# PaddlePaddle/PaddleRec

Hardware: AMD Instinct MI355X
Metric: CTR samples/sec, Criteo DeepFM bs=65536 (train step: fwd+bwd+optimizer) (higher is better)
Workload: dtype f32 (MLP GEMMs: f32 operands as 3 bf16 terms, 6 bf16 MFMAs per product, f32 accumulate); 1 GPU; DeepFM full Criteo: 26 sparse slots x 1000000 rows x dim 16, 13 dense, MLP 400,400,400, batch 65536 per GPU, lazy Adam, uniform ids; global_batch=65536, parallelism=single, table_rows_total=26000000, index_oob_flag=0

## Files before the change

### include/recengine.h

```cpp
#ifndef RECENGINE_H_
#define RECENGINE_H_

#include <stddef.h>
#include <stdint.h>

#ifdef __cplusplus
extern "C" {
#endif

typedef enum {
  REC_OK = 0,
  REC_EINVAL = -1,
  REC_ESHAPE = -2,
  REC_EWORKSPACE = -3,
  REC_EHIP = -4,
  REC_ENCCL = -5
} rec_status;

#define REC_FLAG_INDEX_OOB 1
#define REC_FLAG_EXCHANGE_OVERFLOW 2

const char* rec_last_error(void);
int rec_version(void);

// ... 342 lines not shown

int rec_batchnorm_workspace_bytes(int64_t m, int32_t n, size_t* bytes);
int rec_batchnorm_fwd(int64_t m, int32_t n, const float* X, int64_t ldx, const float* gamma, const float* beta,
                      float* running_mean, float* running_var, float momentum, float eps, int32_t training,
                      float* Y, int64_t ldy, float* save_mean, float* save_invstd, void* workspace,
                      size_t workspace_bytes, void* stream);
int rec_batchnorm_bwd(int64_t m, int32_t n, const float* X, int64_t ldx, const float* dY, int64_t lddy,
                      const float* gamma, const float* save_mean, const float* save_invstd, int32_t relu_mask,
                      float* dX, int64_t lddx, float* dgamma, float* dbeta, void* workspace,
                      size_t workspace_bytes, void* stream);
int rec_dot_interact_fwd(int64_t batch, int32_t F, int32_t D, const float* T, int64_t ldt, float* R, int64_t ldr,
                         void* stream);
int rec_dot_interact_bwd(int64_t batch, int32_t F, int32_t D, const float* T, int64_t ldt, const float* dR,
                         int64_t ldr, float* dT, int64_t lddt, void* stream);
int rec_accuracy_count(int64_t n, const float* pred, const int64_t* label, int64_t* counts, void* stream);

typedef enum {
  REC_EPI_NONE = 0,
  REC_EPI_BIAS = 1,
  REC_EPI_BIAS_RELU = 2,
  REC_EPI_RELU_MASK = 3,
  REC_EPI_CROSS = 4,
  REC_EPI_BIAS_SIGMOID = 5,
  REC_EPI_BIAS_TANH = 6,
  REC_EPI_ADD = 7,
  REC_EPI_DTANH = 10,
  REC_EPI_DSIGMOID = 9,
  REC_EPI_MOE = 8
} rec_epilogue;

typedef struct {
  int64_t m;
  int32_t n, k;
  int32_t lda, ldb, ldc;
  int32_t trans_a, trans_b;
  int32_t epilogue;
  int32_t split_k;
  int32_t num_cus;
} rec_gemm_desc;

typedef struct {
  const float* bias;
  const float* aux0;
  int32_t ld_aux0;
  const float* aux1;
  int32_t ld_aux1;
  const float* row_scale;
  int32_t row_scale_stride;
  float* out2;
  int32_t ld_out2;
  float* b_colsum;
  const void* b_image;
  void* relu_bits;
} rec_gemm_epilogue_args;

int rec_gemm_f32_workspace_bytes(const rec_gemm_desc* desc, size_t* bytes);
int rec_gemm_relu_bits_bytes(const rec_gemm_desc* desc, int32_t* eligible, size_t* bytes);
int rec_gemm_plan_splits(const rec_gemm_desc* desc, int32_t num_cus, int32_t* splits);
int rec_gemm_f32(const rec_gemm_desc* desc, const float* A, const float* B, float* C,
                 const rec_gemm_epilogue_args* args , void* workspace,
                 size_t workspace_bytes, void* stream);
int rec_gemm_f32_pair(const rec_gemm_desc* desc0, const float* A0, const float* B0, float* C0,
                      const rec_gemm_epilogue_args* args0 , const rec_gemm_desc* desc1, const float* A1,
                      const float* B1, float* C1, const rec_gemm_epilogue_args* args1 , void* workspace,
                      size_t workspace_bytes, void* stream);
typedef enum {
  REC_GEMM_ROUTE_SKINNY_ROWS = 0,
  REC_GEMM_ROUTE_SKINNY_DW = 1,
  REC_GEMM_ROUTE_X3_DW = 2,
  REC_GEMM_ROUTE_X3 = 3,
  REC_GEMM_ROUTE_PANEL = 4,
  REC_GEMM_ROUTE_GLDS = 5,
  REC_GEMM_ROUTE_DIRECT = 6,
  REC_GEMM_ROUTE_TILED = 7
} rec_gemm_route_family;
enum {
  REC_GEMM_ROUTE_FAST = 1,
  REC_GEMM_ROUTE_PIPE = 2,
  REC_GEMM_ROUTE_VEC = 4,
  REC_GEMM_ROUTE_KS4 = 8,
  REC_GEMM_ROUTE_FOLD = 16,
  REC_GEMM_ROUTE_VEC_A = 32,
  REC_GEMM_ROUTE_PAIR = 64
};
typedef struct {
  int32_t family;
  int32_t cfg;
  int32_t splits;
  int32_t flags;
} rec_gemm_route;
int rec_gemm_last_route(rec_gemm_route* out);
typedef struct {
  const float* B;
  int32_t ldb, k, n, trans_b;
  void* image;
} rec_gemm_b_image;
int rec_gemm_b_image_bytes(int32_t k, int32_t n, int32_t* eligible, size_t* bytes);
int rec_gemm_b_images(int32_t count, const rec_gemm_b_image* items, void* stream);

int rec_colsum_workspace_bytes(int64_t m, int32_t n, size_t* bytes);
int rec_colsum(int64_t m, int32_t n, int32_t ld, const float* G, float* out, void* workspace,
               size_t workspace_bytes, void* stream);

typedef struct {
  int64_t batch;
  int32_t d;
  int32_t ld_x0, ld_xl, ld_out, ld_u;
} rec_crossnet_v2_desc;
int rec_crossnet_v2_layer_workspace_bytes(const rec_crossnet_v2_desc* desc, size_t* fwd_bytes, size_t* bwd_bytes);
int rec_crossnet_v2_layer_fwd(const rec_crossnet_v2_desc* desc, const float* X0, const float* Xl, const float* W,
                              const float* bias, float* Xnext, float* U_saved, void* workspace,
                              size_t workspace_bytes, void* stream);
int rec_crossnet_v2_layer_bwd(const rec_crossnet_v2_desc* desc, const float* X0, const float* Xl, const float* W,
                              const float* U_saved, const float* dXnext, int32_t ld_dxnext, float* dX0_acc,
                              int32_t ld_acc, int32_t accumulate_dx0, int32_t fold_dx0, float* dXl,
                              int32_t ld_dxl, float* dW, float* db, void* workspace, size_t workspace_bytes,
                              void* stream);

typedef struct {
  int64_t batch;
  int32_t d, rank, experts;
  int32_t ld_x0, ld_xl, ld_out;
} rec_crossnet_mix_desc;
int rec_crossnet_mix_layer_workspace_bytes(const rec_crossnet_mix_desc* desc, size_t* fwd_bytes, size_t* bwd_bytes);
int rec_crossnet_mix_layer_fwd(const rec_crossnet_mix_desc* desc, const float* X0, const float* Xl, const float* U,
                               const float* V, const float* C, const float* bias, const float* gate_w,
                               const float* gate_b, float* Xnext, float* t1, float* t2, float* prob,
                               void* workspace, size_t workspace_bytes, void* stream);
int rec_crossnet_mix_layer_bwd(const rec_crossnet_mix_desc* desc, const float* X0, const float* Xl, const float* U,
                               const float* V, const float* C, const float* bias, const float* gate_w,
                               const float* t1, const float* t2, const float* prob, const float* dXnext,
                               int32_t ld_dxnext, float* dX0_acc, int32_t ld_acc, int32_t accumulate_dx0,
                               int32_t fold_dx0, float* dXl, int32_t ld_dxl, float* gU, float* gV, float* gC,
                               float* gbias, float* g_gate_w, float* g_gate_b, int32_t accumulate_gate,
                               void* workspace, size_t workspace_bytes, void* stream);

// ... 497 lines not shown
```

### paddlerec_amd/_lib.py

```python
import ctypes as C
import os
import re

_HERE = os.path.dirname(os.path.abspath(__file__))
LIB_PATH = os.path.join(_HERE, "librecengine.so")
HEADER_PATH = os.path.join(os.path.dirname(_HERE), "include", "recengine.h")


class RecError(RuntimeError):
    pass


_SCALARS = {"int64_t": C.c_int64, "int32_t": C.c_int32, "uint64_t": C.c_uint64, "uint32_t": C.c_uint32,
            "float": C.c_float, "size_t": C.c_size_t, "int": C.c_int}
_POINTEES = ("void", "char", "uint8_t")
_DIRECTIVE = re.compile(r"#\s*(?:ifn?def\s+\w+|endif|include\s*<\w+\.h>|define\s+RECENGINE_H_)")
_DEFINE = re.compile(r"#\s*define\s+(REC_\w+)\s+(\S.*)")
_DECL = re.compile(r"\s*(?:(typedef\s+)?(enum|struct)\s*\{([^{}]*)\}\s*(\w*)\s*;|([^;{}]+);)")
_PROTO = re.compile(r"(const\s+)?(\w+)\s*(\*?)\s*(rec_\w+)\s*\((.*)\)", re.S)
_PARAM = re.compile(r"(?:const\s+)?(\w+)\s*((?:\*\s*(?:const\s*)?)*)(\w+)")
_FIELD = re.compile(r"(?:const\s+)?(\w+)\b(.*)", re.S)
_DECLARATOR = re.compile(r"(\*?)\s*(\w+)\s*(?:\[\s*(\w+)\s*\])?")


# ... 67 lines not shown
                argtypes.append(pointee(base, decl) if stars else by_value(base, decl))
        sigs[name] = (C.c_char_p if star else by_value(ret, decl), argtypes)

    pos = 0
    while body[pos:].strip():
        m = _DECL.match(body, pos)
        if not m:
            raise RecError("recengine.h: cannot place declaration %r" % body[pos:].strip()[:80])
        pos = m.end()
        typedef, kind, members, name, other = m.groups()
        if kind == "enum":
            for item in filter(None, (s.strip() for s in members.split(","))):
                e = re.fullmatch(r"(REC_\w+)\s*=\s*(.+)", item, re.S)
                if not e:
                    raise RecError("recengine.h: enumerator %r has no explicit value" % item)
                consts[e.group(1)] = _int(e.group(2), consts, item)
        elif kind == "struct":
            if not typedef or not name or name in structs:
                raise RecError("recengine.h: cannot place declaration 'struct { ... } %s'" % name)
            structs[name] = type(struct_names.get(name, name), (C.Structure,),
                                 {"_fields_": fields_of(members, name), "__doc__": name + " (include/recengine.h)."})
        else:
            prototype(" ".join(other.split()))
    return consts, structs, sigs


def _read_header():
    try:
        with open(HEADER_PATH) as f:
            return f.read()
    except OSError as e:
        raise RecError("cannot read the engine's header %s: %s" % (HEADER_PATH, e)) from None


_STRUCT_NAMES = dict(
    rec_deepfm_desc="DeepFMDesc", rec_ffm_desc="FFMDesc", rec_fatffm_desc="FatFFMDesc", rec_fefm_desc="FEFMDesc",
    rec_dcn_cross_desc="DcnCrossDesc", rec_deepfm_net="DeepFMNet", rec_din_net="DinNet", rec_dcn_v2_net="DcnV2Net",
    rec_adam_hyper="AdamHyper", rec_adagrad_hyper="AdagradHyper", rec_grad_layout="GradLayout",
    rec_small_sgd_job="SmallSgdJob", rec_cin_view="CinView", rec_ps_accessor="PsAccessor", rec_lazy_init="LazyInit",
    rec_ps_layout="PsLayout", rec_grad_src="GradSrc", rec_multislot_desc="MultislotDesc", rec_din_desc="DinDesc",
    rec_crossnet_v2_desc="CrossV2Desc", rec_crossnet_mix_desc="CrossMixDesc", rec_gemm_desc="GemmDesc",
    rec_gemm_epilogue_args="GemmEpilogueArgs", rec_gemm_route="GemmRoute", rec_mtl_mix_desc="MtlMixDesc",
    rec_esm_head_desc="EsmHeadDesc", rec_aitm_head_desc="AitmHeadDesc", rec_ids_group_plan_t="IdsGroupPlan",
    rec_gemm_b_image="GemmBImage")

CONSTANTS, STRUCTS, SIGNATURES = parse_header(_read_header(), _STRUCT_NAMES)
globals().update(CONSTANTS)
globals().update((_STRUCT_NAMES[c_name], cls) for c_name, cls in STRUCTS.items() if c_name in _STRUCT_NAMES)

STRUCTS["rec_deepfm_net"].MAX_LINEAR = CONSTANTS["REC_DEEPFM_MAX_LINEAR"]
DCN_MAX_LAYERS = CONSTANTS["REC_DCN_MAX_LAYERS"]
EPI = {name[len("REC_EPI_"):].lower(): value for name, value in CONSTANTS.items() if name.startswith("REC_EPI_")}
GEMM_ROUTE_FAMILIES = ("skinny_rows", "skinny_dw", "x3_dw", "x3", "panel", "glds", "direct", "tiled")
GEMM_ROUTE_FLAGS = dict(fast=1, pipe=2, vec=4, ks4=8, fold=16, vec_a=32, pair=64)
GEMM_CFGS = ("128x80", "256x80", "256x128", "128x128", "80x80", "64x80", "128x80_o4", "144x80")

_lib = None


def lib():
    global _lib
    if _lib is None:
        if not os.path.exists(LIB_PATH):
            raise RecError(
                "librecengine.so not found at %s — run `python -m paddlerec_amd.build` "
                "(there is no CPU fallback)" % LIB_PATH)
        import torch
        h = C.CDLL(LIB_PATH)
        for name, (res, args) in SIGNATURES.items():
            fn = getattr(h, name)
            fn.restype, fn.argtypes = res, args
        _lib = h
    return _lib


def check(rc, what=""):
    if rc != 0:
        msg = lib().rec_last_error().decode("utf-8", "replace")
        raise RecError("%s failed (rc=%d): %s" % (what or "recengine call", rc, msg))
```

### paddlerec_amd/csrc/deepfm_step.hip

```cpp
#include <stdlib.h>

#include <map>
#include <mutex>
#include <tuple>

#include "rec_common.h"
#include "tail_roles.h"

using namespace rec;

namespace {

struct Carve {
  char* base;
  size_t off = 0;
  explicit Carve(void* p) : base((char*)p) {}
  template <class T>
  T* take(size_t count) {
    T* p = base ? (T*)(base + off) : nullptr;
    off += align_up(count * sizeof(T), 256);
    return p;
  }
  void* bytes(size_t n) { return take<char>(n); }
};
// ... 155 lines not shown
        size_t ib = 0;
        if (rec_gemm_b_image_bytes(in, w, &ok, &ib) == REC_OK && ok) bf->img_f[i] = c.bytes(ib);
        if (rec_gemm_b_image_bytes(w, in, &ok, &ib) == REC_OK && ok) bf->img_t[i] = c.bytes(ib);
      }
      in = w;
    }
  }
  static const bool bits_env = [] { const char* v = getenv("REC_RELU_BITS"); return !(v && *v == '0'); }();
  for (int i = 0; i < s.n; ++i) {
    bf->relu_bits[i] = nullptr;
    if (i == 0 || !bits_env) continue;
    const int wi = net->widths[i - 1], kin = i == 1 ? s.in0 : net->widths[i - 2];
    rec_gemm_desc df{B, wi, kin, kin, wi, wi, 0, 0, REC_EPI_BIAS_RELU, 0, 0};
    rec_gemm_desc db{B, wi, net->widths[i], net->widths[i], net->widths[i], wi, 0, 1, REC_EPI_RELU_MASK, 0, 0};
    int32_t okf = 0, okb = 0;
    size_t nf = 0, nb = 0;
    if (rec_gemm_relu_bits_bytes(&df, &okf, &nf) == REC_OK && rec_gemm_relu_bits_bytes(&db, &okb, &nb) == REC_OK && okf && okb &&
        nf == nb)
      bf->relu_bits[i] = c.bytes(nf);
  }
  size_t cw = 0;
  if (int rc = call_workspace(net, s, B, &cw)) return rc;
  bf->ws = c.bytes(cw);
  bf->ws_bytes = cw;
  bf->ws_head = nullptr;
  bf->ws_head_bytes = 0;
  if (s.small && s.ctr_head) {
    size_t hb = 0;
    if (int rc = rec_ctr_head_workspace_bytes(B, net->widths[s.n - 2], &hb)) return rc;
    bf->ws_head = c.bytes(hb);
    bf->ws_head_bytes = hb;
  }
  *total = c.off;
  return REC_OK;
}

int gemm(int64_t m, int n, int k, bool ta, bool tb, int epi, const float* A, const float* Bm, float* C,
         const float* bias, const float* aux0, int ld0, float* b_colsum, int split_k, const Buffers& bf, void* st,
         const void* b_image = nullptr, int num_cus = 0, void* relu_bits = nullptr) {
  rec_gemm_desc d{};
  d.num_cus = num_cus;
  d.m = m; d.n = n; d.k = k;
  d.lda = ta ? (int)m : k;
  d.ldb = tb ? k : n;
  d.ldc = n;
  d.trans_a = ta; d.trans_b = tb; d.epilogue = epi; d.split_k = split_k;
  rec_gemm_epilogue_args x{};
  x.bias = bias; x.aux0 = aux0; x.ld_aux0 = ld0; x.b_colsum = b_colsum; x.b_image = b_image; x.relu_bits = relu_bits;
  return rec_gemm_f32(&d, A, Bm, C, &x, bf.ws, bf.ws_bytes, st);
}

int linear_backward(int64_t B, int in, int w, const float* X, const float* G, const float* W, float* dW, float* db,
                    float* dX, const float* mask, const Buffers& bf, void* st, const void* b_image_t,
                    void* mask_bits = nullptr) {
  rec_gemm_desc d0{}, d1{};
  d0.m = in; d0.n = w; d0.k = (int)B; d0.lda = in; d0.ldb = w; d0.ldc = w; d0.trans_a = 1; d0.epilogue = REC_EPI_NONE;
  d1.m = B; d1.n = in; d1.k = w; d1.lda = w; d1.ldb = w; d1.ldc = in; d1.trans_b = 1;
  d1.epilogue = mask ? REC_EPI_RELU_MASK : REC_EPI_NONE;
  rec_gemm_epilogue_args x0{}, x1{};
  x0.b_colsum = db;
  x1.aux0 = mask; x1.ld_aux0 = mask ? in : 0; x1.b_image = b_image_t; x1.relu_bits = mask ? mask_bits : nullptr;
  return rec_gemm_f32_pair(&d0, X, G, dW, &x0, &d1, G, W, dX, &x1, bf.ws, bf.ws_bytes, st);
}

}

extern "C" int rec_deepfm_train_step_workspace_bytes(const rec_deepfm_net* net, int64_t batch, size_t* bytes) {
  REC_REQUIRE(bytes, REC_EINVAL, "bytes is NULL");
  Shape s;
  if (int rc = shape_of(net, batch, &s)) return rc;
  Buffers bf;
  return carve(net, s, batch, nullptr, &bf, bytes);
}

#define REC_TRY(call)            \
  do {                           \
    if (int rc_ = (call)) return rc_; \
  } while (0)

int rec::step_events(void* stream, void* side_stream, hipEvent_t** out) {
  struct Set { hipEvent_t ev[kStepEvents]; };
  static std::mutex mu;
  static std::map<std::tuple<int, void*, void*>, Set> cache;
  int dev = 0;
  REC_REQUIRE(hipGetDevice(&dev) == hipSuccess, REC_EHIP, "hipGetDevice failed");
  std::lock_guard<std::mutex> lock(mu);
  auto key = std::make_tuple(dev, stream, side_stream);
  auto it = cache.find(key);
  if (it == cache.end()) {
    Set st{};
    for (auto& e : st.ev)
      REC_REQUIRE(hipEventCreateWithFlags(&e, hipEventDisableTiming) == hipSuccess, REC_EHIP, "hipEventCreate failed");
    it = cache.emplace(key, st).first;
  }
  *out = it->second.ev;
  return REC_OK;
}

extern "C" int rec_deepfm_train_step(const rec_deepfm_net* net, int64_t batch, const int64_t* ids, const float* dense,
                                     const int64_t* label, const rec_adam_hyper* hyper, int64_t* auc_pos,
                                     int64_t* auc_neg, int32_t num_thresholds, float* loss_out, float* pred_out,
                                     int32_t* status, void* workspace, size_t workspace_bytes, void* stream,
                                     void* side_stream) {
  Shape s;
  if (int rc = shape_of(net, batch, &s)) return rc;
  REC_REQUIRE(ids && label && hyper && loss_out && pred_out && (dense || s.Dn == 0), REC_EINVAL,
              "null pointer argument");
  REC_REQUIRE(net->rec && net->mv && net->flat_param && net->flat_grad && net->flat_m && net->flat_v, REC_EINVAL,
              "net: null parameter pointer");
  REC_REQUIRE(!(s.compact || s.pad) || net->w0_folded, REC_EINVAL,
              "net: w0_folded is needed with 0 < dense_dim <= dim and with a padded layer0_width");
  REC_REQUIRE((auc_pos == nullptr) == (auc_neg == nullptr), REC_EINVAL, "auc_pos / auc_neg: both or neither");
  Buffers bf;
  size_t need = 0;
// ... 41 lines not shown
  float* gw0 = net->gw[0];
  if (s.compact) {
    if (!fold_rode)
      REC_TRY(rec_dense_fold_fwd_full(S, Dn, D, net->widths[0], net->dense_w, net->w[0], net->w0_folded, stream));
    w0 = net->w0_folded;
    gw0 = bf.dw0p;
  }
  const bool pad_copy = s.pad && net->w0_folded != net->w[0];
  if (pad_copy) {
    REC_TRY(rec_copy_async(net->w0_folded, net->w[0], (size_t)s.in0_real * net->widths[0] * f4, stream));
    w0 = net->w0_folded;
    gw0 = bf.dw0p;
  }
  const int n_fwd = s.ctr_head ? n - 1 : n;
  {
    rec_gemm_b_image items[2 * REC_DEEPFM_MAX_LINEAR];
    int cnt = 0, in = s.in0;
    for (int i = 0; i < n; ++i) {
      const int w = net->widths[i];
      const float* wi = i == 0 ? w0 : net->w[i];
      if (bf.img_f[i]) items[cnt++] = rec_gemm_b_image{wi, w, in, w, 0, bf.img_f[i]};
      if (bf.img_t[i]) items[cnt++] = rec_gemm_b_image{wi, w, w, in, 1, bf.img_t[i]};
      in = w;
    }
    if (cnt) REC_TRY(rec_gemm_b_images(cnt, items, stream));
  }
  {
    int in = s.in0;
    for (int i = 0; i < n_fwd; ++i) {
      const bool last = i == n - 1;
      float* out = last ? bf.y_dnn : bf.act[i + 1];
      REC_TRY(gemm(B, net->widths[i], in, false, false, last ? REC_EPI_BIAS : REC_EPI_BIAS_RELU, bf.act[i],
                   i == 0 ? w0 : net->w[i], out, net->b[i], nullptr, 0, nullptr, 0, bf, stream, bf.img_f[i], 0,
                   last ? nullptr : bf.relu_bits[i + 1]));
      in = net->widths[i];
    }
  }
  const float* g = bf.dz;
  int gi = 0;
  int n_run = n;
  const float* P0 = net->flat_param;
  const float* G0 = net->flat_grad;
  auto flat_pair = [&](const float* pp, const float* gg, int64_t cnt) {
    return pp && gg && pp >= P0 && pp + cnt <= P0 + net->flat_numel && pp - P0 == gg - G0;
  };
  const bool pad_copy_ = s.pad && net->w0_folded != net->w[0];
  bool tail = s.small && s.ctr_head && !pad_copy_ && small_tail_eligible(nlook, D, net->slot_offset, S) &&
              flat_pair(net->w[n - 1], net->gw[n - 1], net->widths[n - 2]) && flat_pair(net->b[n - 1], net->gb[n - 1], 1) &&
              flat_pair(net->w[0], net->gw[0], (int64_t)s.in0_full * net->widths[0]) &&
              (Dn == 0 || (flat_pair(net->dense_w, net->g_dense_w, (int64_t)Dn * D) &&
                           flat_pair(net->dense_w_one, net->g_dense_w_one, Dn)));
  int head_nblk = 0;
  float head_inv = 0.f;
  if (s.ctr_head) {
    const int nh = net->widths[n - 2];
    if (tail)
      REC_TRY(ctr_head_fwd_bwd_partial(B, nh, 0, bf.act[n - 1], nh, net->w[n - 1], net->b[n - 1], bf.y1, bf.y2, label, 1e-4f,
                                       0.f, 0.f, 1, nullptr, pred_out, bf.dz, bf.g[gi], nh, bf.ws_head, bf.ws_head_bytes,
                                       stream, &head_nblk, &head_inv));
    else
    REC_TRY(rec_ctr_head_fwd_bwd(B, nh, 0, bf.act[n - 1], nh, net->w[n - 1], net->b[n - 1], bf.y1, bf.y2, label, 1e-4f,
                                 0.f, 0.f, 1, nullptr, pred_out, bf.dz, loss_out, bf.g[gi], nh, net->gw[n - 1],
                                 net->gb[n - 1], bf.ws, bf.ws_bytes, stream));
    g = bf.g[gi];
    gi ^= 1;
    n_run = n - 1;
  } else {
    REC_TRY(rec_sigmoid_logloss(B, 0, bf.y1, bf.y2, bf.y_dnn, label, 1e-4f, 0.f, 0.f, pred_out, bf.dz, loss_out, bf.ws,
                                bf.ws_bytes, stream));
  }
  if (auc_pos) REC_TRY(rec_auc_histogram(B, pred_out, label, num_thresholds, auc_pos, auc_neg, stream));
  if (!s.ctr_head && s.head) {
    const int nh = net->widths[n - 2];
    REC_TRY(rec_mlp_head_bwd(B, nh, bf.act[n - 1], nh, bf.dz, net->w[n - 1], 1, bf.g[gi], nh, net->gw[n - 1],
                             net->gb[n - 1], bf.ws, bf.ws_bytes, stream));
    g = bf.g[gi];
    gi ^= 1;
    n_run = n - 1;
  }
  const float* g0 = nullptr;
  float* d_flat = nullptr;
  bool dw0_done = false;
  for (int i = n_run - 1; i >= 0; --i) {
    const int in = i == 0 ? s.in0 : net->widths[i - 1], w = net->widths[i];
    if (i == 0) {
      g0 = g;
      d_flat = bf.g[gi];
      if (s.small) {
        dw0_done = true;
        REC_TRY(linear_backward(B, in, w, bf.feat, g, w0, gw0, net->gb[0], d_flat, nullptr, bf, stream, bf.img_t[0]));
        break;
      }
      REC_TRY(gemm(B, in, w, false, true, REC_EPI_NONE, g, w0, d_flat, nullptr, nullptr, 0, nullptr, 0, bf, stream,
                   bf.img_t[0]));
      break;
    }
    REC_TRY(linear_backward(B, in, w, bf.act[i], g, net->w[i], net->gw[i], net->gb[i], bf.g[gi], bf.act[i], bf, stream,
                            bf.img_t[i], bf.relu_bits[i]));
    g = bf.g[gi];
    gi ^= 1;
  }
  rec_deepfm_desc bd{B, S, Dn, D, D, 1, -1, 1, s.compact ? 1 : 0, s.pad ? (int64_t)s.in0 : 0};
  int fm_nblk = 0;
  if (tail)
    REC_TRY(deepfm_fm_bwd_partial(&bd, dense, bf.feat, bf.sum_emb, d_flat, bf.dz, bf.dz, net->dense_w, bf.row_grad, bf.ws,
                                  bf.ws_bytes, stream, &fm_nblk));
  else
  REC_TRY(rec_deepfm_fm_bwd(&bd, dense, bf.feat, bf.sum_emb, d_flat, bf.dz, bf.dz, net->dense_w, bf.row_grad,
                            net->g_dense_w, net->g_dense_w_one, bf.ws, bf.ws_bytes, stream));
  rec_grad_layout gl{1, 0, 0, nullptr, nullptr, 0}, gl1{S, 0, 0, nullptr, nullptr, 0};
  if (tail) {
    TailRoles t{};
    const int nh = net->widths[n - 2], NO = net->widths[0];
    t.head_blocks = (nh + 2 + 15) / 16;
    t.head_nblk = head_nblk; t.head_n2 = nh + 2; t.head_partial = (const float*)bf.ws_head; t.head_invB = head_inv;
    t.head_dw = net->gw[n - 1]; t.head_db = net->gb[n - 1]; t.loss = loss_out;
    t.head_w_off = net->w[n - 1] - P0; t.head_b_off = net->b[n - 1] - P0;
    t.n_skip = 0;
    auto skip = [&](int64_t lo, int64_t cnt) { t.skip_lo[t.n_skip] = lo; t.skip_hi[t.n_skip] = lo + cnt; ++t.n_skip; };
    skip(t.head_w_off, nh);
    skip(t.head_b_off, 1);
    t.fm_blocks = Dn * D + Dn;
    t.fm_nblk = fm_nblk; t.fm_split = Dn * D; t.fm_partial = (const float*)bf.ws;
    t.ddw = net->g_dense_w; t.ddw1 = net->g_dense_w_one;
    if (Dn > 0) {
      t.dw_off = net->dense_w - P0; t.dw1_off = net->dense_w_one - P0;
      skip(t.dw_off, (int64_t)Dn * D);
      skip(t.dw1_off, Dn);
    }
    t.w0_off = net->w[0] - P0;
    t.f = FoldedLayer0{S, Dn, D, NO, nullptr, nullptr, nullptr, nullptr};
    t.w0_blocks = 0;
    if (s.compact) {
      t.f.dW0f = gw0; t.f.dW0 = net->gw[0]; t.f.W0 = net->w[0]; t.f.dense_w = net->dense_w;
      skip(t.w0_off, (int64_t)s.in0_full * NO);
      const int64_t we = (int64_t)S * D * NO;
      t.w0_blocks = (int)((we + 4 * 1024 - 1) / (4 * 1024));
    }
    t.flat_numel = net->flat_numel; t.flat_grad = net->flat_grad;
    t.adam.p = net->flat_param; t.adam.m = net->flat_m; t.adam.v = net->flat_v;
    t.rest_blocks = (int)((net->flat_numel + 4 * 1024 - 1) / (4 * 1024));
    if (t.rest_blocks > 256) t.rest_blocks = 256;
    REC_TRY(sparse_adam_record_small_tail(nlook, S, D, net->rec_stride, net->mv_stride, net->v_offset, net->table_rows,
                                          net->padding_idx, ids, net->slot_offset, bf.row_grad, &gl, bf.dz, &gl1, net->rec,
                                          net->mv, hyper, status, t, stream));
    return REC_OK;
  }
  if (s.small) {
    REC_TRY(rec_sparse_adam_record_small(nlook, S, D, net->rec_stride, net->mv_stride, net->v_offset, net->table_rows,
                                         net->padding_idx, ids, net->slot_offset, bf.row_grad, &gl, bf.dz, &gl1,
                                         nullptr, net->rec, net->mv, hyper, status, bf.small_scratch, stream));
// ... 26 lines not shown
```

### paddlerec_amd/csrc/gemm_bf16x3.h

```cpp
#pragma once

#include <atomic>

#include "gemm_epi.h"
#include "gemm_glds.h"

namespace rec {

typedef __bf16 bf16x8_t __attribute__((ext_vector_type(8)));
typedef unsigned u32x4_t __attribute__((ext_vector_type(4)));

constexpr int kX3NT = 13;
constexpr int kX3NP = 2 * kX3NT * 16;
constexpr int kX3BM = 128;
constexpr int kX3MT = 4;
constexpr int kX3Stage = 3 * kX3NP * 64;
template <int NT>
struct X3Geo {
  static constexpr int NP = NT * 16;
  static constexpr int Plane = NP * 64;
  static constexpr int Stage = 3 * Plane;
  static constexpr int Pieces = Stage / 1024;
};
struct X3Cols { int nt, ncb; };
inline X3Cols x3_cols(int N) {
  const int tiles = (N + 15) / 16;
  X3Cols best{0, 0};
  int best_pad = 1 << 30;
  const int cand[3] = {13, 8, 7};
  for (int c = 0; c < 3; ++c) {
    const int ncb = (tiles + 2 * cand[c] - 1) / (2 * cand[c]);
    const int pad = ncb * 2 * cand[c] - tiles;
    if (pad < best_pad) { best_pad = pad; best = X3Cols{cand[c], ncb}; }
  }
  if (best_pad * 100 > tiles * 15) best.nt = 0;
  return best;
}
inline size_t x3_image_bytes(int K, int N) {
  const X3Cols c = x3_cols(N);
  return (size_t)c.ncb * ((K + 31) / 32) * 3 * (2 * c.nt * 16) * 64;
}

__device__ __forceinline__ int x3_swz(int i) { return (4 - (i >> 2)) & 3; }

typedef __bf16 bf16x2_t __attribute__((ext_vector_type(2)));
typedef float f32x2_t __attribute__((ext_vector_type(2)));
__device__ __forceinline__ unsigned x3_cvt_pk(float lo, float hi) {
  return __builtin_bit_cast(unsigned, __builtin_convertvector(f32x2_t{lo, hi}, bf16x2_t));
}
__device__ __forceinline__ void x3_split_pair(float xe, float xo, unsigned& p0, unsigned& p1, unsigned& p2) {
  p0 = x3_cvt_pk(xe, xo);
  const float re = xe - __uint_as_float(p0 << 16), ro = xo - __uint_as_float(p0 & 0xffff0000u);
  p1 = x3_cvt_pk(re, ro);
  const float se = re - __uint_as_float(p1 << 16), so = ro - __uint_as_float(p1 & 0xffff0000u);
  p2 = x3_cvt_pk(se, so);
}

__device__ __forceinline__ void x3_split_one(const float* __restrict__ W, int64_t ldw, int K, int N, int trans,
                                             char* __restrict__ img, int nkt, int np, int ncb, int64_t tid) {
  if (tid >= (int64_t)ncb * nkt * np * 4) return;
  const int c = (int)(tid & 3), nl = (int)((tid >> 2) % np);
  const int kt = (int)(((tid >> 2) / np) % nkt), cb = (int)((tid >> 2) / np / nkt);
  const int n = cb * np + nl;
  float x[8];
#pragma unroll
  for (int j = 0; j < 8; ++j) {
    const int k = kt * 32 + c * 8 + j;
    x[j] = (n < N && k < K) ? (trans ? W[(int64_t)n * ldw + k] : W[(int64_t)k * ldw + n]) : 0.f;
  }
  u32x4_t p0, p1, p2;
#pragma unroll
  for (int d = 0; d < 4; ++d) {
    unsigned a, b, e;
    x3_split_pair(x[2 * d], x[2 * d + 1], a, b, e);
    p0[d] = a; p1[d] = b; p2[d] = e;
  }
  const size_t plane = (size_t)np * 64;
  char* dst = img + ((size_t)cb * nkt + kt) * 3 * plane + (size_t)nl * 64 + ((c ^ x3_swz(nl & 15)) * 16);
  *reinterpret_cast<u32x4_t*>(dst) = p0;
  *reinterpret_cast<u32x4_t*>(dst + plane) = p1;
  *reinterpret_cast<u32x4_t*>(dst + 2 * plane) = p2;
}
__global__ __launch_bounds__(kBlock) void x3_split_kernel(const float* __restrict__ W, int64_t ldw, int K, int N, int trans,
                                                          char* __restrict__ img, int nkt, int np, int ncb) {
  x3_split_one(W, ldw, K, N, trans, img, nkt, np, ncb, (int64_t)blockIdx.x * kBlock + threadIdx.x);
}
constexpr int kX3BatchMax = 8;
struct X3SplitBatch {
  const float* W[kX3BatchMax];
  char* img[kX3BatchMax];
  int64_t ldw[kX3BatchMax];
  int K[kX3BatchMax], N[kX3BatchMax], trans[kX3BatchMax], nkt[kX3BatchMax], np[kX3BatchMax], ncb[kX3BatchMax];
  unsigned first[kX3BatchMax + 1];
  int count;
};
__global__ __launch_bounds__(kBlock) void x3_split_batch_kernel(const X3SplitBatch b) {
  int i = 0;
#pragma unroll
  for (int j = 1; j < kX3BatchMax; ++j)
    if (j < b.count && blockIdx.x >= b.first[j]) i = j;
  x3_split_one(b.W[i], b.ldw[i], b.K[i], b.N[i], b.trans[i], b.img[i], b.nkt[i], b.np[i], b.ncb[i],
               (int64_t)(blockIdx.x - b.first[i]) * kBlock + threadIdx.x);
}

template <int T, int PLANE>
__device__ __forceinline__ void x3_read_frags(u32x4_t (&bf)[3], unsigned sb, unsigned sb2) {
  asm volatile("ds_read_b128 %0, %1 offset:%2" : "=v"(bf[0]) : "v"(sb), "n"(T * 1024));
  asm volatile("ds_read_b128 %0, %1 offset:%2" : "=v"(bf[1]) : "v"(sb), "n"(T * 1024 + PLANE));
  asm volatile("ds_read_b128 %0, %1 offset:%2" : "=v"(bf[2]) : "v"(sb2), "n"(T * 1024));
}
template <int PLANE>
__device__ __forceinline__ void x3_read_frags_t(u32x4_t (&bf)[3], unsigned sb, unsigned sb2, int t) {
  switch (t) {
    case 0: x3_read_frags<0, PLANE>(bf, sb, sb2); break;
    case 1: x3_read_frags<1, PLANE>(bf, sb, sb2); break;
    case 2: x3_read_frags<2, PLANE>(bf, sb, sb2); break;
    case 3: x3_read_frags<3, PLANE>(bf, sb, sb2); break;
    case 4: x3_read_frags<4, PLANE>(bf, sb, sb2); break;
    case 5: x3_read_frags<5, PLANE>(bf, sb, sb2); break;
    case 6: x3_read_frags<6, PLANE>(bf, sb, sb2); break;
    case 7: x3_read_frags<7, PLANE>(bf, sb, sb2); break;
    case 8: x3_read_frags<8, PLANE>(bf, sb, sb2); break;
    case 9: x3_read_frags<9, PLANE>(bf, sb, sb2); break;
    case 10: x3_read_frags<10, PLANE>(bf, sb, sb2); break;
    case 11: x3_read_frags<11, PLANE>(bf, sb, sb2); break;
    default: x3_read_frags<12, PLANE>(bf, sb, sb2); break;
  }
}

#ifndef REC_X3_LAB
#define REC_X3_LAB 0
#endif
#ifndef REC_X3_TG
#define REC_X3_TG 2
#endif
template <int TG>
__device__ __forceinline__ void x3_wait_group(u32x4_t (&f)[TG][3], int left) {
#define REC_X3_TIE(U) if constexpr (TG > U) asm volatile("" : "+v"(f[U][0]), "+v"(f[U][1]), "+v"(f[U][2]));
  switch (left) {
    case 0: asm volatile("s_waitcnt lgkmcnt(0)" ::: "memory"); break;
    case 3: asm volatile("s_waitcnt lgkmcnt(3)" ::: "memory"); break;
    case 6: asm volatile("s_waitcnt lgkmcnt(6)" ::: "memory"); break;
    case 9: asm volatile("s_waitcnt lgkmcnt(9)" ::: "memory"); break;
    default: asm volatile("s_waitcnt lgkmcnt(0)" ::: "memory"); break;
  }
  REC_X3_TIE(0) REC_X3_TIE(1) REC_X3_TIE(2) REC_X3_TIE(3)
#undef REC_X3_TIE
}

#ifndef REC_X3_DW_PIPE_STORES
#define REC_X3_DW_PIPE_STORES 1
#endif
#ifndef REC_X3_DW_VALU_PER_MFMA
#define REC_X3_DW_VALU_PER_MFMA 2
#endif
#ifndef REC_X3_PRODUCTS
#define REC_X3_PRODUCTS 6
#endif

template <int NT, int EPI, int WM, int WN>
__global__ __launch_bounds__(WM * WN * 64, WN == 1 ? 2 : 1) void gemm_bf16x3_kernel(
    int64_t M, int N, int K, const float* __restrict__ A, int64_t lda, const char* __restrict__ Bimg_all,
    float* __restrict__ C, int64_t ldc, EpiArgs epi, int ncb) {
  using Geo = X3Geo<NT>;
  constexpr int MT = kX3BM / 16 / WM;
  constexpr int NW = WM * WN;
  constexpr int BStage = WN * Geo::Stage;
  extern __shared__ __attribute__((aligned(1024))) char x3_smem[];
  const int lane = threadIdx.x % kWave;
  const int wave = __builtin_amdgcn_readfirstlane(threadIdx.x / kWave);
  const int li = lane & 15, g = lane >> 4;
  const int wm = wave % WM, wn = wave / WM;
  const int nkt = (K + 31) / 32;
  int64_t row_tile;
  int cb0;
  if constexpr (WN == 1) {
    const int xcd = blockIdx.x & 7, j = blockIdx.x >> 3;
    cb0 = j % ncb;
    row_tile = (int64_t)(j / ncb) * 8 + xcd;
    if (row_tile * kX3BM >= M) return;
  } else {
    row_tile = blockIdx.x;
    cb0 = blockIdx.y * WN;
  }
  const int64_t m0 = row_tile * kX3BM + wm * (MT * 16);
  const char* Bimg = Bimg_all + (size_t)cb0 * nkt * Geo::Stage;

  const float* ap[MT];
#pragma unroll
  for (int a = 0; a < MT; ++a) {
    int64_t r = m0 + a * 16 + li;
    r = r < M ? r : M - 1;
    ap[a] = A + r * lda + g * 8;
  }
  float4 araw[MT][2];
  auto load_a = [&](int kt) {
#if REC_X3_LAB == 2
    if (kt > 0) return;
#endif
    const int koff = kt * 32 + g * 8 < K ? kt * 32 : 0;
#pragma unroll
    for (int a = 0; a < MT; ++a) {
      araw[a][0] = *reinterpret_cast<const float4*>(ap[a] + koff);
      araw[a][1] = *reinterpret_cast<const float4*>(ap[a] + koff + 4);
    }
  };
  auto issue_b = [&](int kt, int stage) {
#if REC_X3_LAB == 3
    if (kt > 0) return;
#endif
    const char* src = Bimg + (size_t)kt * Geo::Stage + lane * 16;
    const char* dst = x3_smem + stage * BStage;
#pragma unroll
    for (int j = 0; j < (WN * Geo::Pieces + NW - 1) / NW; ++j) {
      const int piece = wave + NW * j;
      if (piece < WN * Geo::Pieces) {
        const int w = WN == 1 ? 0 : piece / Geo::Pieces, q = piece - w * Geo::Pieces;
        __builtin_amdgcn_global_load_lds((glb_void_t*)(src + (size_t)w * nkt * Geo::Stage + q * 1024),
                                         (lds_void_t*)(dst + w * Geo::Stage + q * 1024), 16, 0, 0);
      }
    }
  };

  f32x4_t acc[MT][NT];
#pragma unroll
  for (int a = 0; a < MT; ++a)
#pragma unroll
    for (int t = 0; t < NT; ++t) acc[a][t] = f32x4_t{0.f, 0.f, 0.f, 0.f};

  const unsigned lds_base = (unsigned)(uintptr_t)x3_smem + wn * Geo::Stage + li * 64 + ((g ^ x3_swz(li)) * 16);

  issue_b(0, 0);
  load_a(0);
  wait_vmcnt<0>();
  __builtin_amdgcn_s_barrier();

  for (int kt = 0; kt < nkt; ++kt) {
    const int stage = kt & 1;
    u32x4_t af[MT][3];
    if (kt == nkt - 1 && (K & 31) != 0 && kt * 32 + g * 8 >= K) {
#pragma unroll
      for (int a = 0; a < MT; ++a) araw[a][0] = araw[a][1] = make_float4(0.f, 0.f, 0.f, 0.f);
    }
#pragma unroll
    for (int a = 0; a < MT; ++a) {
      const float x[8] = {araw[a][0].x, araw[a][0].y, araw[a][0].z, araw[a][0].w,
                          araw[a][1].x, araw[a][1].y, araw[a][1].z, araw[a][1].w};
#pragma unroll
      for (int d = 0; d < 4; ++d) {
#if REC_X3_LAB == 4
        af[a][0][d] = __float_as_uint(x[2 * d]); af[a][1][d] = __float_as_uint(x[2 * d + 1]); af[a][2][d] = __float_as_uint(x[2 * d]) ^ 1u;
#else
        unsigned p0, p1, p2;
        x3_split_pair(x[2 * d], x[2 * d + 1], p0, p1, p2);
        af[a][0][d] = p0; af[a][1][d] = p1; af[a][2][d] = p2;
#endif
      }
    }
    if (kt + 1 < nkt) {
      issue_b(kt + 1, stage ^ 1);
      load_a(kt + 1);
    }
    __builtin_amdgcn_sched_barrier(0);
#if REC_X3_LAB == 3
    const unsigned sb = lds_base;
#else
    const unsigned sb = lds_base + stage * BStage;
#endif
    constexpr int TG = REC_X3_TG, NG = (NT + TG - 1) / TG;
    u32x4_t bf[2][TG][3];
    auto read_group = [&](int gi, int slot) {
#pragma unroll
      for (int u = 0; u < TG; ++u)
        if (gi * TG + u < NT) x3_read_frags_t<Geo::Plane>(bf[slot][u], sb, sb + 2 * Geo::Plane, gi * TG + u);
    };
    read_group(0, 0);
#pragma unroll
    for (int gi = 0; gi < NG; ++gi) {
      const int slot = gi & 1;
      const int n_cur = NT - gi * TG < TG ? NT - gi * TG : TG;
      int left = 0;
      if (gi + 1 < NG) {
        read_group(gi + 1, slot ^ 1);
        left = 3 * (NT - (gi + 1) * TG < TG ? NT - (gi + 1) * TG : TG);
      }
      x3_wait_group<TG>(bf[slot], left);
#define REC_X3_MFMA(PB, PA)                                                                                          \
  _Pragma("unroll") for (int u = 0; u < TG; ++u) if (u < n_cur) {                                                    \
    _Pragma("unroll") for (int a = 0; a < MT; ++a) acc[a][gi * TG + u] = __builtin_amdgcn_mfma_f32_16x16x32_bf16(    \
        __builtin_bit_cast(bf16x8_t, bf[slot][u][PB]), __builtin_bit_cast(bf16x8_t, af[a][PA]), acc[a][gi * TG + u], 0, 0, 0); \
  }
#if REC_X3_PRODUCTS >= 6
      REC_X3_MFMA(2, 0)
      REC_X3_MFMA(1, 1)
      REC_X3_MFMA(0, 2)
#endif
#if REC_X3_PRODUCTS >= 3
      REC_X3_MFMA(1, 0)
      REC_X3_MFMA(0, 1)
#endif
      REC_X3_MFMA(0, 0)
#undef REC_X3_MFMA
      __builtin_amdgcn_sched_barrier(0);
    }
    if (kt + 1 < nkt) {
      wait_vmcnt<0>();
      __builtin_amdgcn_s_barrier();
// ... 10 lines not shown
    unsigned long long* bits_at = epi.relu_bits ? epi.relu_bits + ((ic * ncb + (cb0 + wn)) * 4 + g) : nullptr;
    unsigned long long mbits = 0ull;
    if constexpr (EPI == REC_EPI_RELU_MASK) {
      if (bits_at) mbits = *bits_at;
    }
#pragma unroll
    for (int t = 0; t < NT; ++t) {
      const int j = n_base + t * 16;
      const int jc = j < N ? j : 0;
#pragma unroll
      for (int c = 0; c < 4; ++c) bj[t][c] = load_bias<EPI>(jc + c, epi);
      if constexpr (EPI == REC_EPI_ADD) {
        x0[t] = epi.aux0 ? *reinterpret_cast<const f32x4_t*>(epi.aux0 + ic * epi.ld0 + jc) : f32x4_t{0.f, 0.f, 0.f, 0.f};
      } else if constexpr (EPI == REC_EPI_RELU_MASK) {
        if (bits_at) {
#pragma unroll
          for (int c = 0; c < 4; ++c) x0[t][c] = ((mbits >> (4 * t + c)) & 1ull) ? 1.f : 0.f;
        } else {
          x0[t] = *reinterpret_cast<const f32x4_t*>(epi.aux0 + ic * epi.ld0 + jc);
        }
      } else if constexpr (EpiUses<EPI>::aux0) {
        x0[t] = *reinterpret_cast<const f32x4_t*>(epi.aux0 + ic * epi.ld0 + jc);
      } else {
        x0[t] = f32x4_t{0.f, 0.f, 0.f, 0.f};
      }
      if constexpr (EpiUses<EPI>::aux1) x1[t] = *reinterpret_cast<const f32x4_t*>(epi.aux1 + ic * epi.ld1 + jc);
    }
#pragma unroll
    for (int t = 0; t < NT; ++t) {
      const int j = n_base + t * 16;
      f32x4_t v, u;
#pragma unroll
      for (int c = 0; c < 4; ++c) {
        const float xx1 = EpiUses<EPI>::aux1 ? x1[EpiUses<EPI>::aux1 ? t : 0][c] : 0.f;
        v[c] = apply_epi<EPI>(acc[a][t][c], x0[t][c], xx1, bj[t][c], ic, epi);
        u[c] = acc[a][t][c] + bj[t][c];
        if constexpr (EPI == REC_EPI_BIAS_RELU) mbits |= (unsigned long long)(v[c] > 0.f ? 1 : 0) << (4 * t + c);
      }
#if REC_X3_LAB == 1
      if (row_ok && j < N && v[0] == 1.2345678e33f) {
#else
      if (row_ok && j < N) {
#endif
        *reinterpret_cast<f32x4_t*>(C + i * ldc + j) = v;
        if constexpr (EPI == REC_EPI_CROSS) {
          if (epi.out2) *reinterpret_cast<f32x4_t*>(epi.out2 + i * epi.ld2 + j) = u;
        }
      }
    }
    if constexpr (EPI == REC_EPI_BIAS_RELU) {
      if (bits_at && row_ok) *bits_at = mbits;
    }
  }
}

constexpr int kX3DwCols = 208;
constexpr int kX3DwPlane = kX3DwCols * 64;
constexpr int kX3DwOperand = 3 * kX3DwPlane;
constexpr int kX3DwWT = 7;

__device__ __forceinline__ int x3_dw_q(int i, int a) { return (i >> 2) + 4 * (((i & 3) + a) & 3); }

template <int T>
__device__ __forceinline__ void x3_dw_read(u32x4_t (&f)[3], unsigned base) {
  asm volatile("ds_read_b128 %0, %1 offset:%2" : "=v"(f[0]) : "v"(base), "n"(T * 256));
  asm volatile("ds_read_b128 %0, %1 offset:%2" : "=v"(f[1]) : "v"(base), "n"(T * 256 + kX3DwPlane));
  asm volatile("ds_read_b128 %0, %1 offset:%2" : "=v"(f[2]) : "v"(base), "n"(T * 256 + 2 * kX3DwPlane));
}

__device__ __forceinline__ void x3_dw_read_u(u32x4_t (&f)[3], unsigned base, int u) {
  switch (u) {
    case 0: x3_dw_read<0>(f, base); break;
    case 1: x3_dw_read<1>(f, base); break;
    case 2: x3_dw_read<2>(f, base); break;
    case 3: x3_dw_read<3>(f, base); break;
    case 4: x3_dw_read<4>(f, base); break;
    case 5: x3_dw_read<5>(f, base); break;
    default: x3_dw_read<6>(f, base); break;
  }
}

__device__ __forceinline__ void x3_dw_wait_frags(u32x4_t (&f)[3], int left) {
#define REC_X3_WAIT_CASE(N) case N: asm volatile("s_waitcnt lgkmcnt(" #N ")" : "+v"(f[0]), "+v"(f[1]), "+v"(f[2])); break;
  switch (left) {
    REC_X3_WAIT_CASE(0) REC_X3_WAIT_CASE(1) REC_X3_WAIT_CASE(2) REC_X3_WAIT_CASE(3) REC_X3_WAIT_CASE(4) REC_X3_WAIT_CASE(5)
    REC_X3_WAIT_CASE(6) REC_X3_WAIT_CASE(7) REC_X3_WAIT_CASE(8) REC_X3_WAIT_CASE(9) REC_X3_WAIT_CASE(10) REC_X3_WAIT_CASE(11)
    REC_X3_WAIT_CASE(12) REC_X3_WAIT_CASE(13) REC_X3_WAIT_CASE(14) REC_X3_WAIT_CASE(15)
    default: asm volatile("s_waitcnt lgkmcnt(0)" : "+v"(f[0]), "+v"(f[1]), "+v"(f[2])); break;
  }
#undef REC_X3_WAIT_CASE
}

struct X3DwArgs {
  const float* X; int64_t ldx;
  const float* G; int64_t ldg;
  int64_t rows;
  int kin, nout;
  int kb_tiles, nb_tiles;
  int kblocks, nblocks;
  int slices, steps_per_slice;
  float* P; int64_t ldp;
  float* cpart;
};

template <int PW, bool PIPE>
__global__ __launch_bounds__(256) void gemm_bf16x3_dw_kernel(X3DwArgs w) {
  extern __shared__ __attribute__((aligned(1024))) char x3_smem[];
  const int tid = threadIdx.x;
  const int lane = tid % kWave;
  const int wave = __builtin_amdgcn_readfirstlane(tid / kWave);
  const int li = lane & 15, g = lane >> 4;
  const int wk = wave & 1, wn = wave >> 1;
  const int nob = w.kblocks * w.nblocks;
  const int xcd = blockIdx.x & 7, j = blockIdx.x >> 3;
  const int ob = j % nob, slice = (j / nob) * 8 + xcd;
  const int kb = ob / w.nblocks, nb = ob % w.nblocks;
  const int k_tile0 = kb * w.kb_tiles, n_tile0 = nb * w.nb_tiles;
  const int kt_blk = min(w.kb_tiles, (w.kin + 15) / 16 - k_tile0);
  const int nt_blk = min(w.nb_tiles, (w.nout + 15) / 16 - n_tile0);
  const int k_split = (kt_blk + 1) / 2, n_split = (nt_blk + 1) / 2;
  const int my_k0 = wk ? k_split : 0, my_p = __builtin_amdgcn_readfirstlane(wk ? kt_blk - k_split : k_split);
  const int my_n0 = wn ? n_split : 0, my_q = __builtin_amdgcn_readfirstlane(wn ? nt_blk - n_split : n_split);
  const int64_t row0 = (int64_t)slice * w.steps_per_slice * 32;
  int nsteps = (int)min((int64_t)w.steps_per_slice, (w.rows - row0) / 32);
  if (nsteps < 0) nsteps = 0;

  const bool stager = tid < 4 * (kX3DwCols / 4);
  const int mg = stager ? tid / (kX3DwCols / 4) : 0, cg = tid % (kX3DwCols / 4);
  const int xc = k_tile0 * 16 + cg * 4, gc = n_tile0 * 16 + cg * 4;
  const bool x_ok = stager && cg * 4 < kt_blk * 16 && xc < w.kin;
  const bool g_ok = stager && cg * 4 < nt_blk * 16 && gc < w.nout;
  const float* xp = w.X + (row0 + mg * 8) * w.ldx + (x_ok ? xc : 0);
  const float* gp = w.G + (row0 + mg * 8) * w.ldg + (g_ok ? gc : 0);
  float4 xr[8], gr[8];
  auto load_patches = [&](int kt) {
#ifdef REC_X3_DW_NO_LOADS
    if (kt > 0) return;
#endif
#pragma unroll
    for (int r = 0; r < 8; ++r) {
      xr[r] = *reinterpret_cast<const float4*>(xp + ((int64_t)kt * 32 + r) * w.ldx);
      gr[r] = *reinterpret_cast<const float4*>(gp + ((int64_t)kt * 32 + r) * w.ldg);
    }
  };
  unsigned wr_off[4];
#pragma unroll
  for (int e = 0; e < 4; ++e) {
    const int a = cg >> 2, i = 4 * (cg & 3) + e;
    wr_off[e] = (unsigned)((mg * kX3DwCols + 16 * a + x3_dw_q(i, a)) * 16);
  }
  float4 csum = make_float4(0.f, 0.f, 0.f, 0.f);
  const unsigned w_stage = stager ? (unsigned)kX3Stage : 0u, w_oper = stager ? (unsigned)kX3DwOperand : 0u,
                 w_plane = stager ? (unsigned)kX3DwPlane : 0u;
  char* const w_base = stager ? x3_smem : x3_smem + 2 * kX3Stage + tid * 16;
  if (!stager) { wr_off[0] = wr_off[1] = wr_off[2] = wr_off[3] = 0u; }
  auto convert_compute = [&](int e, u32x4_t (&ch)[6]) {
    float xv[8], gv[8];
#pragma unroll
    for (int r = 0; r < 8; ++r) {
      xv[r] = e == 0 ? xr[r].x : e == 1 ? xr[r].y : e == 2 ? xr[r].z : xr[r].w;
      gv[r] = e == 0 ? gr[r].x : e == 1 ? gr[r].y : e == 2 ? gr[r].z : gr[r].w;
    }
    asm volatile("" : "+v"(xv[0]), "+v"(xv[1]), "+v"(xv[2]), "+v"(xv[3]), "+v"(xv[4]), "+v"(xv[5]), "+v"(xv[6]), "+v"(xv[7]),
                      "+v"(gv[0]), "+v"(gv[1]), "+v"(gv[2]), "+v"(gv[3]), "+v"(gv[4]), "+v"(gv[5]), "+v"(gv[6]), "+v"(gv[7]));
#pragma unroll
    for (int d = 0; d < 4; ++d) {
      unsigned a, b, c;
#ifdef REC_X3_DW_NOCVT
      a = __float_as_uint(xv[2 * d]); b = __float_as_uint(xv[2 * d + 1]); c = a ^ b;
#else
      x3_split_pair(x_ok ? xv[2 * d] : 0.f, x_ok ? xv[2 * d + 1] : 0.f, a, b, c);
#endif
      ch[0][d] = a; ch[1][d] = b; ch[2][d] = c;
    }
    float cs = 0.f;
#pragma unroll
    for (int d = 0; d < 4; ++d) {
      const float u0 = g_ok ? gv[2 * d] : 0.f, u1 = g_ok ? gv[2 * d + 1] : 0.f;
      cs += u0 + u1;
      unsigned a, b, c;
#ifdef REC_X3_DW_NOCVT
      a = __float_as_uint(u0); b = __float_as_uint(u1); c = a ^ b;
#else
      x3_split_pair(u0, u1, a, b, c);
#endif
      ch[3][d] = a; ch[4][d] = b; ch[5][d] = c;
    }
    if (e == 0) csum.x += cs; else if (e == 1) csum.y += cs; else if (e == 2) csum.z += cs; else csum.w += cs;
  };
  auto convert_write = [&](int stage, int e, const u32x4_t (&ch)[6]) {
    char* sx = w_base + stage * w_stage + wr_off[e];
    char* sg = sx + w_oper;
#ifdef REC_X3_DW_NOWRITE
    *reinterpret_cast<u32x4_t*>(sx) = ch[0] ^ ch[1] ^ ch[2];
    *reinterpret_cast<u32x4_t*>(sg) = ch[3] ^ ch[4] ^ ch[5];
#else
    *reinterpret_cast<u32x4_t*>(sx) = ch[0];
    *reinterpret_cast<u32x4_t*>(sx + w_plane) = ch[1];
    *reinterpret_cast<u32x4_t*>(sx + 2 * w_plane) = ch[2];
    *reinterpret_cast<u32x4_t*>(sg) = ch[3];
    *reinterpret_cast<u32x4_t*>(sg + w_plane) = ch[4];
    *reinterpret_cast<u32x4_t*>(sg + 2 * w_plane) = ch[5];
#endif
  };
  auto convert_part = [&](int stage, int e) {
    u32x4_t ch[6];
    convert_compute(e, ch);
    convert_write(stage, e, ch);
  };
  auto convert_store = [&](int stage) {
#pragma unroll
    for (int e = 0; e < 4; ++e) convert_part(stage, e);
  };

  f32x4_t acc[PW][kX3DwWT];
#pragma unroll
  for (int a = 0; a < PW; ++a)
// ... 28 lines not shown
#pragma unroll
    for (int u = 0; u < PW; ++u) x3_dw_read_u(af[u], xb[u & 3] + so, u);
    x3_dw_read_u(bf[1], gb[1] + so, 1);
#pragma unroll
    for (int a = 0; a < PW; ++a) {
      x3_dw_wait_frags(af[a], 3 * (PW - 1 - a) + 3);
      const u32x4_t* b0 = bf[0];
#define REC_X3_DW_MFMA0(PB, PA)                                                                                \
  acc[a][0] = __builtin_amdgcn_mfma_f32_16x16x32_bf16(__builtin_bit_cast(bf16x8_t, b0[PB]),                      \
                                                      __builtin_bit_cast(bf16x8_t, af[a][PA]), acc[a][0], 0, 0, 0);
#if REC_X3_PRODUCTS >= 6
      REC_X3_DW_MFMA0(2, 0) REC_X3_DW_MFMA0(1, 1) REC_X3_DW_MFMA0(0, 2)
#endif
#if REC_X3_PRODUCTS >= 3
      REC_X3_DW_MFMA0(1, 0) REC_X3_DW_MFMA0(0, 1)
#endif
      REC_X3_DW_MFMA0(0, 0)
#undef REC_X3_DW_MFMA0
      __builtin_amdgcn_sched_barrier(0);
    }
    __builtin_amdgcn_sched_barrier(0);
#pragma unroll
    for (int t = 1; t < kX3DwWT; ++t) {
      if (t + 1 < kX3DwWT) {
        x3_dw_read_u(bf[(t + 1) & 1], gb[(t + 1) & 3] + so, t + 1);
        asm volatile("s_waitcnt lgkmcnt(3)" : "+v"(bf[t & 1][0]), "+v"(bf[t & 1][1]), "+v"(bf[t & 1][2]));
      } else {
        asm volatile("s_waitcnt lgkmcnt(0)" : "+v"(bf[t & 1][0]), "+v"(bf[t & 1][1]), "+v"(bf[t & 1][2]));
      }
      const u32x4_t* b = bf[t & 1];
#define REC_X3_DW_MFMA(PB, PA)                                                                                 \
  _Pragma("unroll") for (int a = 0; a < PW; ++a) acc[a][t] = __builtin_amdgcn_mfma_f32_16x16x32_bf16(            \
      __builtin_bit_cast(bf16x8_t, b[PB]), __builtin_bit_cast(bf16x8_t, af[a][PA]), acc[a][t], 0, 0, 0);
#if REC_X3_PRODUCTS >= 6
      REC_X3_DW_MFMA(2, 0) REC_X3_DW_MFMA(1, 1) REC_X3_DW_MFMA(0, 2)
#endif
#if REC_X3_PRODUCTS >= 3
      REC_X3_DW_MFMA(1, 0) REC_X3_DW_MFMA(0, 1)
#endif
      REC_X3_DW_MFMA(0, 0)
#undef REC_X3_DW_MFMA
#ifndef REC_X3_DW_SERIAL_CONVERT
      if constexpr (PIPE) {
      if (MORE && t >= kX3DwWT - 5) {
        const bool wr = t >= kX3DwWT - 4, cv = t <= kX3DwWT - 2;
        if (wr) convert_write(stage ^ 1, t - (kX3DwWT - 4), pend);
        if (cv) convert_compute(t - (kX3DwWT - 5), pend);
#pragma unroll
        for (int i = 0; i < 6 * PW; ++i) {
          __builtin_amdgcn_sched_group_barrier(0x008, 1, 0);
          if (cv) __builtin_amdgcn_sched_group_barrier(0x002, REC_X3_DW_VALU_PER_MFMA, 0);
          if (wr && i % PW == PW / 2) __builtin_amdgcn_sched_group_barrier(0x200, 1, 0);
        }
        if (cv) __builtin_amdgcn_sched_group_barrier(0x002, 32, 0);
      }
      } else if (MORE && t >= kX3DwWT - 4) {
        convert_part(stage ^ 1, t - (kX3DwWT - 4));
#pragma unroll
        for (int i = 0; i < 6 * PW; ++i) {
          __builtin_amdgcn_sched_group_barrier(0x008, 1, 0);
          __builtin_amdgcn_sched_group_barrier(0x002, REC_X3_DW_VALU_PER_MFMA, 0);
        }
        __builtin_amdgcn_sched_group_barrier(0x002, 32, 0);
        __builtin_amdgcn_sched_group_barrier(0x200, 6, 0);
      }
#endif
      __builtin_amdgcn_sched_barrier(0);
    }
#ifdef REC_X3_DW_SERIAL_CONVERT
    if (MORE) convert_store(stage ^ 1);
#endif
    __syncthreads();
  };
  for (int kt = 0; kt + 1 < nsteps; ++kt) step(kt, std::true_type{});
  if (nsteps > 0) step(nsteps - 1, std::false_type{});

  float* P = w.P + (int64_t)slice * w.kin * w.ldp;
#pragma unroll
  for (int a = 0; a < PW; ++a) {
    if (a >= my_p) continue;
    const int ki = (k_tile0 + my_k0 + a) * 16 + li;
#pragma unroll
    for (int t = 0; t < kX3DwWT; ++t) {
      if (t >= my_q) continue;
      const int nj = (n_tile0 + my_n0 + t) * 16 + g * 4;
      if (ki < w.kin && nj < w.nout) *reinterpret_cast<f32x4_t*>(P + (int64_t)ki * w.ldp + nj) = acc[a][t];
    }
  }
  if (w.cpart && kb == 0) {
    float4* red = reinterpret_cast<float4*>(x3_smem);
    if (stager) red[(tid / (kX3DwCols / 4)) * (kX3DwCols / 4) + cg] = csum;
    __syncthreads();
    if (tid < kX3DwCols / 4 && tid * 4 < nt_blk * 16 && n_tile0 * 16 + tid * 4 < w.nout) {
      const float4 s0 = red[tid], s1 = red[kX3DwCols / 4 + tid], s2 = red[2 * (kX3DwCols / 4) + tid],
                   s3 = red[3 * (kX3DwCols / 4) + tid];
      float4 o;
      o.x = (s0.x + s1.x) + (s2.x + s3.x); o.y = (s0.y + s1.y) + (s2.y + s3.y);
      o.z = (s0.z + s1.z) + (s2.z + s3.z); o.w = (s0.w + s1.w) + (s2.w + s3.w);
      *reinterpret_cast<float4*>(w.cpart + (int64_t)slice * w.nout + n_tile0 * 16 + tid * 4) = o;
    }
  }
}

template <int PW>
struct X3Dw8Acc { f32x4_t v[PW][kX3DwWT]; };

struct X3Dw8Ctx {
  const float* src; int64_t ld; bool ok;
  char* base; unsigned wr_off[4];
  unsigned xb[4], gb[4];
  float4 raw[8];
  float4 csum;
  float* P; int64_t ldp; int kin, nout, k_tile0, n_tile0, my_k0, my_n0, my_p, my_q, li, g;
  __device__ __forceinline__ void load_patch(int kt) {
#pragma unroll
    for (int r = 0; r < 8; ++r) raw[r] = *reinterpret_cast<const float4*>(src + ((int64_t)kt * 32 + r) * ld);
  }
  __device__ __forceinline__ void convert(int e, u32x4_t (&ch)[3]) {
    float v[8];
#pragma unroll
    for (int r = 0; r < 8; ++r) v[r] = e == 0 ? raw[r].x : e == 1 ? raw[r].y : e == 2 ? raw[r].z : raw[r].w;
    asm volatile("" : "+v"(v[0]), "+v"(v[1]), "+v"(v[2]), "+v"(v[3]), "+v"(v[4]), "+v"(v[5]), "+v"(v[6]), "+v"(v[7]));
    float cs = 0.f;
#pragma unroll
    for (int d = 0; d < 4; ++d) {
      const float u0 = ok ? v[2 * d] : 0.f, u1 = ok ? v[2 * d + 1] : 0.f;
      cs += u0 + u1;
      unsigned a, b, cc;
      x3_split_pair(u0, u1, a, b, cc);
      ch[0][d] = a; ch[1][d] = b; ch[2][d] = cc;
    }
    if (e == 0) csum.x += cs; else if (e == 1) csum.y += cs; else if (e == 2) csum.z += cs; else csum.w += cs;
  }
  __device__ __forceinline__ void write(int stage, int e, const u32x4_t (&ch)[3]) {
    char* p = base + stage * kX3Stage + wr_off[e];
    *reinterpret_cast<u32x4_t*>(p) = ch[0];
    *reinterpret_cast<u32x4_t*>(p + kX3DwPlane) = ch[1];
    *reinterpret_cast<u32x4_t*>(p + 2 * kX3DwPlane) = ch[2];
  }
  template <int NP>
  __device__ __forceinline__ void store(const f32x4_t (&acc)[NP][kX3DwWT]) {
#pragma unroll
    for (int a = 0; a < NP; ++a) {
      if (a >= my_p) continue;
      const int ki = (k_tile0 + my_k0 + a) * 16 + li;
#pragma unroll
      for (int t = 0; t < kX3DwWT; ++t) {
        if (t >= my_q) continue;
        const int nj = (n_tile0 + my_n0 + t) * 16 + g * 4;
        if (ki < kin && nj < nout) *reinterpret_cast<f32x4_t*>(P + (int64_t)ki * ldp + nj) = acc[a][t];
      }
    }
  }
};

template <int PW>
__device__ __forceinline__ void x3_dw8_run(X3Dw8Ctx& c, int nsteps) {
  X3Dw8Acc<PW> acc;
#pragma unroll
  for (int a = 0; a < PW; ++a)
#pragma unroll
    for (int t = 0; t < kX3DwWT; ++t) acc.v[a][t] = f32x4_t{0.f, 0.f, 0.f, 0.f};
  auto step = [&](int kt, auto more_c) {
    constexpr bool MORE = decltype(more_c)::value;
    const int stage = kt & 1;
    if (MORE) c.load_patch(kt + 1);
    __builtin_amdgcn_sched_barrier(0);
    const unsigned so = stage * kX3Stage;
    u32x4_t af[PW][3];
    u32x4_t bf[2][3];
    u32x4_t pend[3];
    x3_dw_read_u(bf[0], c.gb[0] + so, 0);
#pragma unroll
    for (int u = 0; u < PW; ++u) x3_dw_read_u(af[u], c.xb[u & 3] + so, u);
    x3_dw_read_u(bf[1], c.gb[1] + so, 1);
#pragma unroll
    for (int a = 0; a < PW; ++a) {
      x3_dw_wait_frags(af[a], 3 * (PW - 1 - a) + 3);
      const u32x4_t* b0 = bf[0];
#define REC_X3_DW8_MFMA0(PB, PA)                                                                               \
  acc.v[a][0] = __builtin_amdgcn_mfma_f32_16x16x32_bf16(__builtin_bit_cast(bf16x8_t, b0[PB]),                  \
                                                        __builtin_bit_cast(bf16x8_t, af[a][PA]), acc.v[a][0], 0, 0, 0);
#if REC_X3_PRODUCTS >= 6
      REC_X3_DW8_MFMA0(2, 0) REC_X3_DW8_MFMA0(1, 1) REC_X3_DW8_MFMA0(0, 2)
#endif
#if REC_X3_PRODUCTS >= 3
      REC_X3_DW8_MFMA0(1, 0) REC_X3_DW8_MFMA0(0, 1)
#endif
      REC_X3_DW8_MFMA0(0, 0)
#undef REC_X3_DW8_MFMA0
      __builtin_amdgcn_sched_barrier(0);
    }
    __builtin_amdgcn_sched_barrier(0);
#pragma unroll
    for (int t = 1; t < kX3DwWT; ++t) {
      if (t + 1 < kX3DwWT) {
        x3_dw_read_u(bf[(t + 1) & 1], c.gb[(t + 1) & 3] + so, t + 1);
        asm volatile("s_waitcnt lgkmcnt(3)" : "+v"(bf[t & 1][0]), "+v"(bf[t & 1][1]), "+v"(bf[t & 1][2]));
      } else {
        asm volatile("s_waitcnt lgkmcnt(0)" : "+v"(bf[t & 1][0]), "+v"(bf[t & 1][1]), "+v"(bf[t & 1][2]));
      }
      const u32x4_t* b = bf[t & 1];
#define REC_X3_DW8_MFMA(PB, PA)                                                                                \
  _Pragma("unroll") for (int a = 0; a < PW; ++a) acc.v[a][t] = __builtin_amdgcn_mfma_f32_16x16x32_bf16(        \
      __builtin_bit_cast(bf16x8_t, b[PB]), __builtin_bit_cast(bf16x8_t, af[a][PA]), acc.v[a][t], 0, 0, 0);
#if REC_X3_PRODUCTS >= 6
      REC_X3_DW8_MFMA(2, 0) REC_X3_DW8_MFMA(1, 1) REC_X3_DW8_MFMA(0, 2)
#endif
#if REC_X3_PRODUCTS >= 3
      REC_X3_DW8_MFMA(1, 0) REC_X3_DW8_MFMA(0, 1)
#endif
      REC_X3_DW8_MFMA(0, 0)
#undef REC_X3_DW8_MFMA
      if (MORE && t >= kX3DwWT - 5) {
        const bool wr = t >= kX3DwWT - 4, cv = t <= kX3DwWT - 2;
        if (wr) c.write(stage ^ 1, t - (kX3DwWT - 4), pend);
        if (cv) c.convert(t - (kX3DwWT - 5), pend);
#pragma unroll
        for (int i = 0; i < 6 * PW; ++i) {
          __builtin_amdgcn_sched_group_barrier(0x008, 1, 0);
          if (cv) __builtin_amdgcn_sched_group_barrier(0x002, REC_X3_DW_VALU_PER_MFMA, 0);
          if (wr && i % (2 * PW) == PW) __builtin_amdgcn_sched_group_barrier(0x200, 1, 0);
        }
        if (cv) __builtin_amdgcn_sched_group_barrier(0x002, 32, 0);
      }
      __builtin_amdgcn_sched_barrier(0);
    }
    __syncthreads();
  };
  for (int kt = 0; kt + 1 < nsteps; ++kt) step(kt, std::true_type{});
  if (nsteps > 0) step(nsteps - 1, std::false_type{});
  c.store(acc.v);
}

template <int PW>
__global__ __launch_bounds__(512) void gemm_bf16x3_dw_kernel_w8(X3DwArgs w) {
  static_assert(PW >= 2 && PW <= 4, "four X tiles at most fit the 256-register budget");
  extern __shared__ __attribute__((aligned(1024))) char x3_smem[];
  const int tid = threadIdx.x;
  const int lane = tid % kWave;
  const int wave = __builtin_amdgcn_readfirstlane(tid / kWave);
  const int li = lane & 15, g = lane >> 4;
  const int wk = wave < 4 ? wave : 7 - wave, wn = wave >> 2;
  const int nob = w.kblocks * w.nblocks;
  const int xcd = blockIdx.x & 7, j = blockIdx.x >> 3;
  const int ob = j % nob, slice = (j / nob) * 8 + xcd;
  const int kb = ob / w.nblocks, nb = ob % w.nblocks;
  const int k_tile0 = kb * w.kb_tiles, n_tile0 = nb * w.nb_tiles;
  const int kt_blk = min(w.kb_tiles, (w.kin + 15) / 16 - k_tile0);
  const int nt_blk = min(w.nb_tiles, (w.nout + 15) / 16 - n_tile0);
  const int n_split = (nt_blk + 1) / 2;
  const int kq = kt_blk >> 2, kr = kt_blk & 3;
  const int my_k0 = wk * kq + min(wk, kr), my_p = __builtin_amdgcn_readfirstlane(kq + (wk < kr ? 1 : 0));
  const int my_n0 = wn ? n_split : 0, my_q = __builtin_amdgcn_readfirstlane(wn ? nt_blk - n_split : n_split);
  const int64_t row0 = (int64_t)slice * w.steps_per_slice * 32;
  int nsteps = (int)min((int64_t)w.steps_per_slice, (w.rows - row0) / 32);
  if (nsteps < 0) nsteps = 0;

  const int op = wave >> 2, s = tid & 255;
  const bool stager = s < 4 * (kX3DwCols / 4);
  const int sp = stager ? s : s - 4 * (kX3DwCols / 4);
  const int mg = sp / (kX3DwCols / 4), cg = sp % (kX3DwCols / 4);
  const int col = (op ? n_tile0 : k_tile0) * 16 + cg * 4;
  const bool ok = cg * 4 < (op ? nt_blk : kt_blk) * 16 && col < (op ? w.nout : w.kin);
  const int64_t ld = op ? w.ldg : w.ldx;
  const float* src = (op ? w.G : w.X) + (row0 + mg * 8) * ld + (ok ? col : 0);

  X3Dw8Ctx c;
  c.src = src; c.ld = ld; c.ok = ok;
  c.base = x3_smem + op * kX3DwOperand;
#pragma unroll
  for (int e = 0; e < 4; ++e) {
    const int a = cg >> 2, i = 4 * (cg & 3) + e;
    c.wr_off[e] = (unsigned)((mg * kX3DwCols + 16 * a + x3_dw_q(i, a)) * 16);
  }
  c.csum = make_float4(0.f, 0.f, 0.f, 0.f);
  const unsigned lds0 = (unsigned)(uintptr_t)x3_smem;
#pragma unroll
  for (int u = 0; u < 4; ++u) {
    const int ax = my_k0 + u, an = my_n0 + u;
    c.xb[u] = lds0 + (unsigned)((g * kX3DwCols + 16 * my_k0 + x3_dw_q(li, ax)) * 16);
    c.gb[u] = lds0 + kX3DwOperand + (unsigned)((g * kX3DwCols + 16 * my_n0 + x3_dw_q(li, an)) * 16);
  }
  c.P = w.P + (int64_t)slice * w.kin * w.ldp; c.ldp = w.ldp; c.kin = w.kin; c.nout = w.nout; c.k_tile0 = k_tile0; c.n_tile0 = n_tile0; c.my_k0 = my_k0; c.my_n0 = my_n0;
  c.my_p = my_p; c.my_q = my_q; c.li = li; c.g = g;

  if (nsteps > 0) {
    c.load_patch(0);
#pragma unroll
    for (int e = 0; e < 4; ++e) {
      u32x4_t ch[3];
      c.convert(e, ch);
      c.write(0, e, ch);
    }
  }
  __syncthreads();
  if (my_p == PW) x3_dw8_run<PW>(c, nsteps);
  else x3_dw8_run<PW - 1>(c, nsteps);

  if (w.cpart && kb == 0) {
    float4* red = reinterpret_cast<float4*>(x3_smem);
    if (op == 1 && stager) red[mg * (kX3DwCols / 4) + cg] = c.csum;
    __syncthreads();
    if (tid < kX3DwCols / 4 && tid * 4 < nt_blk * 16 && n_tile0 * 16 + tid * 4 < w.nout) {
      const float4 s0 = red[tid], s1 = red[kX3DwCols / 4 + tid], s2 = red[2 * (kX3DwCols / 4) + tid],
                   s3 = red[3 * (kX3DwCols / 4) + tid];
      float4 o;
      o.x = (s0.x + s1.x) + (s2.x + s3.x); o.y = (s0.y + s1.y) + (s2.y + s3.y);
      o.z = (s0.z + s1.z) + (s2.z + s3.z); o.w = (s0.w + s1.w) + (s2.w + s3.w);
      *reinterpret_cast<float4*>(w.cpart + (int64_t)slice * w.nout + n_tile0 * 16 + tid * 4) = o;
    }
  }
}

inline int x3_launch_split(const float* W, int64_t ldw, int K, int N, int trans, char* img, hipStream_t st) {
  const X3Cols c = x3_cols(N);
  const int nkt = (K + 31) / 32, np = c.nt * 16, ncb = 2 * c.ncb;
  const int64_t thr = (int64_t)ncb * nkt * np * 4;
  hipLaunchKernelGGL(x3_split_kernel, dim3((unsigned)((thr + kBlock - 1) / kBlock)), dim3(kBlock), 0, st, W, ldw, K, N,
                     trans, img, nkt, np, ncb);
  return check_launch("x3_split_kernel");
}

inline size_t x3_relu_bits_bytes(int64_t M, int N) { return (size_t)M * (2 * x3_cols(N).ncb) * 4 * sizeof(unsigned long long); }

inline bool x3_shape_ok(int64_t M, int N, int K, int64_t lda, int64_t ldc, const void* A, const void* C) {
  return M > 0 && N > 0 && x3_cols(N).nt > 0 && N % 4 == 0 && K > 0 && K % 8 == 0 && lda % 4 == 0 && ldc % 4 == 0 &&
         ((uintptr_t)A % 16) == 0 && ((uintptr_t)C % 16) == 0;
}

template <int NT, int EPI, int WM, int WN>
inline int x3_launch_gemm_wm(int64_t M, int N, int K, const float* A, int64_t lda, const char* img, float* C, int64_t ldc,
                             const EpiArgs& e, int ncb, hipStream_t st) {
  static std::atomic<bool> attr_set{false};
  constexpr int lds = 2 * WN * X3Geo<NT>::Stage;
  if (!attr_set.load(std::memory_order_acquire)) {
    if (hipFuncSetAttribute(reinterpret_cast<const void*>(&gemm_bf16x3_kernel<NT, EPI, WM, WN>),
                            hipFuncAttributeMaxDynamicSharedMemorySize, lds) != hipSuccess) {
      (void)hipGetLastError();
      set_error("gemm_bf16x3: %d B of dynamic LDS refused", lds);
      return REC_EHIP;
    }
    attr_set.store(true, std::memory_order_release);
  }
  const int64_t row_tiles = (M + kX3BM - 1) / kX3BM;
  if constexpr (WN == 1) {
    const int64_t grid = (row_tiles + 7) / 8 * 8 * ncb;
    if (grid >= (1ll << 31)) { set_error("gemm_bf16x3: too many workgroups"); return REC_ESHAPE; }
    hipLaunchKernelGGL((gemm_bf16x3_kernel<NT, EPI, WM, WN>), dim3((unsigned)grid), dim3(WM * WN * 64), lds, st, M, N, K, A,
                       lda, img, C, ldc, e, ncb);
  } else {
    hipLaunchKernelGGL((gemm_bf16x3_kernel<NT, EPI, WM, WN>), dim3((unsigned)row_tiles, (unsigned)(ncb / WN)),
                       dim3(WM * WN * 64), lds, st, M, N, K, A, lda, img, C, ldc, e, ncb);
  }
  return check_launch("gemm_bf16x3_kernel");
}

#ifndef REC_X3_WM
#define REC_X3_WM 4
#endif
inline int x3_wn_default() {
  static const int v = [] { const char* e = getenv("REC_X3_WN"); return e && *e == '2' ? 2 : 1; }();
  return v;
}
template <int NT, int EPI>
inline int x3_launch_gemm_cfg(int64_t M, int N, int K, const float* A, int64_t lda, const char* img, float* C, int64_t ldc,
                              const EpiArgs& e, int ncb, hipStream_t st) {
  if constexpr (EpiUses<EPI>::aux1) {
    return x3_launch_gemm_wm<NT, EPI, 2, 2>(M, N, K, A, lda, img, C, ldc, e, ncb, st);
  } else {
    if (REC_X3_WM == 4 && x3_wn_default() == 1)
      return x3_launch_gemm_wm<NT, EPI, 4, 1>(M, N, K, A, lda, img, C, ldc, e, ncb, st);
    return x3_launch_gemm_wm<NT, EPI, REC_X3_WM, 2>(M, N, K, A, lda, img, C, ldc, e, ncb, st);
  }
}

template <int EPI>
inline int x3_launch_gemm_epi(int64_t M, int N, int K, const float* A, int64_t lda, const char* img, float* C, int64_t ldc,
                              const EpiArgs& e, hipStream_t st) {
  const X3Cols c = x3_cols(N);
  switch (c.nt) {
    case 13: return x3_launch_gemm_cfg<13, EPI>(M, N, K, A, lda, img, C, ldc, e, 2 * c.ncb, st);
    case 8: return x3_launch_gemm_cfg<8, EPI>(M, N, K, A, lda, img, C, ldc, e, 2 * c.ncb, st);
    case 7: return x3_launch_gemm_cfg<7, EPI>(M, N, K, A, lda, img, C, ldc, e, 2 * c.ncb, st);
    default: set_error("gemm_bf16x3: no column blocking for N = %d", N); return REC_ESHAPE;
  }
}

inline bool x3_epilogue_ok(int epi) { return epi >= REC_EPI_NONE && epi <= REC_EPI_DTANH; }

inline int x3_launch_gemm(int epi, int64_t M, int N, int K, const float* A, int64_t lda, const char* img, float* C,
                          int64_t ldc, const EpiArgs& e, hipStream_t st) {
  switch (epi) {
    case REC_EPI_NONE: return x3_launch_gemm_epi<REC_EPI_NONE>(M, N, K, A, lda, img, C, ldc, e, st);
    case REC_EPI_BIAS: return x3_launch_gemm_epi<REC_EPI_BIAS>(M, N, K, A, lda, img, C, ldc, e, st);
    case REC_EPI_BIAS_RELU: return x3_launch_gemm_epi<REC_EPI_BIAS_RELU>(M, N, K, A, lda, img, C, ldc, e, st);
    case REC_EPI_RELU_MASK: return x3_launch_gemm_epi<REC_EPI_RELU_MASK>(M, N, K, A, lda, img, C, ldc, e, st);
    case REC_EPI_CROSS: return x3_launch_gemm_epi<REC_EPI_CROSS>(M, N, K, A, lda, img, C, ldc, e, st);
    case REC_EPI_BIAS_SIGMOID: return x3_launch_gemm_epi<REC_EPI_BIAS_SIGMOID>(M, N, K, A, lda, img, C, ldc, e, st);
    case REC_EPI_BIAS_TANH: return x3_launch_gemm_epi<REC_EPI_BIAS_TANH>(M, N, K, A, lda, img, C, ldc, e, st);
    case REC_EPI_ADD: return x3_launch_gemm_epi<REC_EPI_ADD>(M, N, K, A, lda, img, C, ldc, e, st);
    case REC_EPI_MOE: return x3_launch_gemm_epi<REC_EPI_MOE>(M, N, K, A, lda, img, C, ldc, e, st);
    case REC_EPI_DSIGMOID: return x3_launch_gemm_epi<REC_EPI_DSIGMOID>(M, N, K, A, lda, img, C, ldc, e, st);
    case REC_EPI_DTANH: return x3_launch_gemm_epi<REC_EPI_DTANH>(M, N, K, A, lda, img, C, ldc, e, st);
    default: set_error("gemm_bf16x3: epilogue %d not built", epi); return REC_EINVAL;
  }
}

struct X3DwPlan { int kb_tiles, nb_tiles, kblocks, nblocks, slices, steps_per_slice; };
inline bool x3_dw_plan(int kin, int nout, int64_t rows, int cus, X3DwPlan* p) {
  if (kin % 4 || nout % 4 || rows % 32 || kin < 16 || nout < 16) return false;
  const int kt = (kin + 15) / 16, nt = (nout + 15) / 16;
  p->kblocks = (kt + 12) / 13; p->nblocks = (nt + 12) / 13;
  p->kb_tiles = (kt + p->kblocks - 1) / p->kblocks; p->nb_tiles = (nt + p->nblocks - 1) / p->nblocks;
  const int nob = p->kblocks * p->nblocks;
  int slices = cus / nob;
  slices -= slices % 8;
  if (slices < 8) return false;
  const int64_t steps = rows / 32;
  p->steps_per_slice = (int)((steps + slices - 1) / slices);
  if (p->steps_per_slice < 4) return false;
  p->slices = (int)((steps + p->steps_per_slice - 1) / p->steps_per_slice);
  p->slices = (p->slices + 7) / 8 * 8;
  return true;
}
#ifndef REC_X3_DW_FORM_DEFAULT
#define REC_X3_DW_FORM_DEFAULT 1
#endif
template <typename K>
inline bool x3_dw_lds_attr(K kernel, int lds) {
  return hipFuncSetAttribute(reinterpret_cast<const void*>(kernel), hipFuncAttributeMaxDynamicSharedMemorySize, lds) == hipSuccess;
}
inline int x3_launch_dw(const X3DwPlan& pl, int kin, int nout, int64_t rows, const float* X, int64_t ldx, const float* G,
                        int64_t ldg, float* P, int64_t ldp, float* cpart, hipStream_t st, int form = -1) {
  static std::atomic<bool> attr_set{false};
  constexpr int lds = 2 * kX3Stage + 4096;
  if (!attr_set.load(std::memory_order_acquire)) {
    if (!x3_dw_lds_attr(&gemm_bf16x3_dw_kernel<7, true>, lds) || !x3_dw_lds_attr(&gemm_bf16x3_dw_kernel<5, true>, lds) ||
        !x3_dw_lds_attr(&gemm_bf16x3_dw_kernel<7, false>, lds) || !x3_dw_lds_attr(&gemm_bf16x3_dw_kernel<5, false>, lds) ||
        !x3_dw_lds_attr(&gemm_bf16x3_dw_kernel_w8<4>, lds) || !x3_dw_lds_attr(&gemm_bf16x3_dw_kernel_w8<3>, lds)) {
      (void)hipGetLastError();
      set_error("gemm_bf16x3_dw: %d B of dynamic LDS refused", lds);
      return REC_EHIP;
    }
    attr_set.store(true, std::memory_order_release);
  }
  X3DwArgs w{X, ldx, G, ldg, rows, kin, nout, pl.kb_tiles, pl.nb_tiles, pl.kblocks, pl.nblocks, pl.slices,
             pl.steps_per_slice, P, ldp, cpart};
  const unsigned grid = (unsigned)(pl.slices * pl.kblocks * pl.nblocks);
  static const int env_form = [] {
    const char* v = getenv("REC_X3_DW_FORM");
    return v && *v ? (*v != '0' ? 1 : 0) : REC_X3_DW_FORM_DEFAULT;
  }();
  if ((form < 0 ? env_form : form) != 0) {
    if ((pl.kb_tiles + 3) / 4 >= 4) hipLaunchKernelGGL((gemm_bf16x3_dw_kernel_w8<4>), dim3(grid), dim3(512), lds, st, w);
    else hipLaunchKernelGGL((gemm_bf16x3_dw_kernel_w8<3>), dim3(grid), dim3(512), lds, st, w);
    return check_launch("gemm_bf16x3_dw_kernel_w8");
  }
  static const bool pipe = [] { const char* v = getenv("REC_X3_DW_PIPE"); return v && *v ? *v != '0' : REC_X3_DW_PIPE_STORES != 0; }();
  const bool p5 = (pl.kb_tiles + 1) / 2 <= 5;
  if (p5 && pipe) hipLaunchKernelGGL((gemm_bf16x3_dw_kernel<5, true>), dim3(grid), dim3(256), lds, st, w);
  else if (p5) hipLaunchKernelGGL((gemm_bf16x3_dw_kernel<5, false>), dim3(grid), dim3(256), lds, st, w);
  else if (pipe) hipLaunchKernelGGL((gemm_bf16x3_dw_kernel<7, true>), dim3(grid), dim3(256), lds, st, w);
  else hipLaunchKernelGGL((gemm_bf16x3_dw_kernel<7, false>), dim3(grid), dim3(256), lds, st, w);
  return check_launch("gemm_bf16x3_dw_kernel");
}

}
```

### paddlerec_amd/csrc/gemm_epi.h

```cpp
#pragma once

#include "rec_common.h"

namespace rec {

typedef float f32x4_t __attribute__((ext_vector_type(4)));

constexpr int kBK = 16;

inline thread_local rec_gemm_route g_gemm_route = {-1, -1, 0, 0};
inline void set_route(int family, int cfg = -1, int splits = 1, int flags = 0) {
  g_gemm_route = rec_gemm_route{family, cfg, splits, flags};
}

template <int R, int C, bool MEMT, int NTHR>
struct TileLoader {
  static constexpr int INNER = MEMT ? R : C, OUTER = MEMT ? C : R;
  static constexpr int kVecs = R * C / 4;
  static constexpr int kPerThread = (kVecs + NTHR - 1) / NTHR;
  float4 stage[kPerThread];

  template <int MODE>
  __device__ __forceinline__ void load(const float* __restrict__ p, int64_t ld, int64_t r0, int64_t c0,
                                       int64_t rmax, int64_t cmax, bool vec_ok, int tid) {
// ... 9 lines not shown
        if (MODE == 0) {
          x = *reinterpret_cast<const float4*>(p + go * ld + gi);
        } else if (MODE == 1) {
          const bool ok = go < omax && gi + 3 < imax;
          const int64_t go_c = go < omax ? go : omax - 1;
          const int64_t gi_c = gi + 3 < imax ? gi : 0;
          const float4 t = *reinterpret_cast<const float4*>(p + go_c * ld + gi_c);
          x.x = ok ? t.x : 0.f; x.y = ok ? t.y : 0.f; x.z = ok ? t.z : 0.f; x.w = ok ? t.w : 0.f;
        } else if (go < omax) {
          const float* q = p + go * ld + gi;
          if (vec_ok && gi + 3 < imax) {
            x = *reinterpret_cast<const float4*>(q);
          } else {
            if (gi + 0 < imax) x.x = q[0];
            if (gi + 1 < imax) x.y = q[1];
            if (gi + 2 < imax) x.z = q[2];
            if (gi + 3 < imax) x.w = q[3];
          }
        }
      }
      stage[it] = x;
    }
  }

  template <bool TRANSPOSE>
  __device__ __forceinline__ void store(float* __restrict__ lds, int tid) const {
#pragma unroll
    for (int it = 0; it < kPerThread; ++it) {
      const int v = tid + it * NTHR;
      if (kVecs % NTHR == 0 || v < kVecs) {
        const int o = v / (INNER / 4), i4 = (v % (INNER / 4)) * 4;
        if (!TRANSPOSE) {
          *reinterpret_cast<float4*>(lds + o * (INNER + 4) + i4) = stage[it];
        } else {
          lds[(i4 + 0) * (OUTER + 4) + o] = stage[it].x;
          lds[(i4 + 1) * (OUTER + 4) + o] = stage[it].y;
          lds[(i4 + 2) * (OUTER + 4) + o] = stage[it].z;
          lds[(i4 + 3) * (OUTER + 4) + o] = stage[it].w;
        }
      }
    }
  }
};

struct EpiArgs {
  const float* bias;
  const float* aux0;
  const float* aux1;
  const float* row_scale;
  float* out2;
  int ld0, ld1, rs_stride, ld2;
  int nt_store;
  unsigned long long* relu_bits;
};

template <int EPI>
struct EpiUses {
  static constexpr bool aux0 = EPI == REC_EPI_RELU_MASK || EPI == REC_EPI_CROSS || EPI == REC_EPI_DTANH ||
                               EPI == REC_EPI_DSIGMOID || EPI == REC_EPI_MOE || EPI == REC_EPI_ADD;
  static constexpr bool aux1 = EPI == REC_EPI_CROSS || EPI == REC_EPI_MOE || EPI == REC_EPI_ADD;
};
template <int EPI>
__device__ __forceinline__ float load_aux0(int64_t i, int j, const EpiArgs& e) {
  if (EPI == REC_EPI_ADD) return e.aux0 ? e.aux0[i * e.ld0 + j] : 0.f;
  return EpiUses<EPI>::aux0 ? e.aux0[i * e.ld0 + j] : 0.f;
}
template <int EPI>
__device__ __forceinline__ float load_aux1(int64_t i, int j, const EpiArgs& e) {
  return EpiUses<EPI>::aux1 ? e.aux1[i * e.ld1 + j] : 0.f;
}

template <int EPI>
__device__ __forceinline__ float load_bias(int j, const EpiArgs& e) {
  if (EPI == REC_EPI_BIAS || EPI == REC_EPI_BIAS_RELU || EPI == REC_EPI_CROSS || EPI == REC_EPI_MOE ||
      EPI == REC_EPI_BIAS_SIGMOID)
    return e.bias[j];
  if (EPI == REC_EPI_BIAS_TANH || EPI == REC_EPI_ADD) return e.bias ? e.bias[j] : 0.f;
  return 0.f;
}
template <int EPI>
__device__ __forceinline__ float apply_epi(float acc, float x0, float x1, float bj, int64_t i, const EpiArgs& e) {
  if (EPI == REC_EPI_NONE) return acc;
  if (EPI == REC_EPI_BIAS) return acc + bj;
  if (EPI == REC_EPI_BIAS_RELU) return fmaxf(acc + bj, 0.f);
  if (EPI == REC_EPI_RELU_MASK) return x0 > 0.f ? acc : 0.f;
  if (EPI == REC_EPI_CROSS) return x1 + x0 * (acc + bj);
  if (EPI == REC_EPI_DTANH) return acc * (1.f - x0 * x0);
  if (EPI == REC_EPI_DSIGMOID) return acc * x0 * (1.f - x0);
  if (EPI == REC_EPI_MOE) return x1 + x0 * (e.row_scale[i * e.rs_stride] * (acc + bj));
  if (EPI == REC_EPI_BIAS_SIGMOID) return 1.f / (1.f + expf(-(acc + bj)));
  if (EPI == REC_EPI_BIAS_TANH) return tanhf(acc + bj);
  if (EPI == REC_EPI_ADD) return acc + bj + x1 + x0;
  return acc;
}
template <int EPI>
__device__ __forceinline__ float apply_epi(float acc, int64_t i, int j, const EpiArgs& e) {
  return apply_epi<EPI>(acc, load_aux0<EPI>(i, j, e), load_aux1<EPI>(i, j, e), load_bias<EPI>(j, e), i, e);
}

}
```

### paddlerec_amd/csrc/gemm_f32.hip

```cpp
#include <stdlib.h>

#include "rec_common.h"

#include "gemm_epi.h"
#include "gemm_direct.h"
#include "gemm_glds.h"
#include "gemm_panel.h"
#include "gemm_pipe.h"
#include "gemm_bf16x3.h"
namespace rec {

template <int BM, int BN, int WAVES_M, int WAVES_N, int OCC, bool TA, bool TB, int EPI>
__global__ __launch_bounds__(WAVES_M* WAVES_N* kWave, (OCC * WAVES_M * WAVES_N + 3) / 4) void gemm_f32_kernel(
    int64_t M, int N, int K, const float* __restrict__ A, int64_t lda, const float* __restrict__ B,
    int64_t ldb, float* __restrict__ C, int64_t ldc, EpiArgs epi, int tiles_n, int64_t tiles_total,
    int k_chunk, bool vec_a, bool vec_b, bool fast, float* __restrict__ partial,
    float* __restrict__ colsum_partial, int splits_in_x) {
  constexpr int NTHR = WAVES_M * WAVES_N * kWave;
  constexpr int WTM = BM / WAVES_M, WTN = BN / WAVES_N;
  constexpr int MT = WTM / 16, NT = WTN / 16;
  static_assert(WTM % 16 == 0 && WTN % 16 == 0, "wave tile must be a multiple of the 16x16 MFMA tile");
  constexpr int LDA_S = TA ? BM + 4 : kBK + 4, LDB_S = BN + 4;
  constexpr int A_ELEMS = TA ? kBK * LDA_S : BM * LDA_S, B_ELEMS = kBK * LDB_S;
  extern __shared__ __attribute__((aligned(16))) float gemm_smem[];
// ... 700 lines not shown
static bool x3_call_ok(const rec_gemm_desc* d, const float* A, const float* C, const EpiArgs& e) {
  if (!x3_eligible(d)) return false;
  if (!x3_shape_ok(d->m, d->n, d->k, d->lda, d->ldc, A, C)) return false;
  if (e.aux0 && (e.ld0 % 4 || ((uintptr_t)e.aux0) % 16)) return false;
  if (e.aux1 && (e.ld1 % 4 || ((uintptr_t)e.aux1) % 16)) return false;
  if (e.out2 && (e.ld2 % 4 || ((uintptr_t)e.out2) % 16)) return false;
  return true;
}
static bool launch_x3(const rec_gemm_desc* d, const float* A, const float* B, float* C, const EpiArgs& e,
                      const void* b_image, void* workspace, size_t workspace_bytes, hipStream_t st) {
  if (!x3_call_ok(d, A, C, e)) return false;
  if (b_image && ((uintptr_t)b_image) % 16 == 0)
    return x3_launch_gemm(d->epilogue, d->m, d->n, d->k, A, d->lda, (const char*)b_image, C, d->ldc, e, st) == REC_OK;
  if (!workspace || ((uintptr_t)workspace) % 16 || workspace_bytes < x3_image_bytes(d->k, d->n)) return false;
  char* img = (char*)workspace;
  if (x3_launch_split(B, d->ldb, d->k, d->n, d->trans_b ? 1 : 0, img, st) != REC_OK) return false;
  return x3_launch_gemm(d->epilogue, d->m, d->n, d->k, A, d->lda, img, C, d->ldc, e, st) == REC_OK;
}

template <int EPI>
static void launch_reduce(const rec_gemm_desc* d, const GemmPlan& p, const float* partial, float* C,
                          const EpiArgs& e, hipStream_t st, const float* cpart = nullptr, float* colsum_out = nullptr) {
  int64_t grid = (d->m * d->n + kBlock - 1) / kBlock;
  if (grid > kNumCU * 8) grid = kNumCU * 8;
  const int cblocks = cpart && colsum_out ? (d->n + kBlock - 1) / kBlock : 0;
  hipLaunchKernelGGL(splitk_reduce_kernel<EPI>, dim3((unsigned)(grid + cblocks)), dim3(kBlock), 0, st, d->m,
                     d->n, (int64_t)d->ldc, p.splits, partial, C, e, cpart, colsum_out, cblocks);
}

static bool x3_dw_eligible(const rec_gemm_desc* d, X3DwPlan* pl) {
  const char* v = getenv("REC_GEMM_BF16X3");
  const bool forced = !(v && *v == '1');
  const char* vd = getenv("REC_GEMM_BF16X3_DW");
  if (vd && *vd == '0') return false;
  if (!x3_enabled() || !d->trans_a || d->trans_b || (d->split_k != 0 && !forced && d->num_cus <= 0) ||
      d->epilogue != REC_EPI_NONE)
    return false;
  if (d->k < 8192 || d->m < 336 || d->m > 448 || d->n < 336 || d->n > 416) return false;
  if (d->lda % 4 || d->ldb % 4 || d->ldc % 4) return false;
  const int cus = d->num_cus > 0 && d->num_cus < device_cus() ? d->num_cus : device_cus();
  return x3_dw_plan((int)d->m, d->n, d->k, cus, pl);
}
static size_t x3_dw_bytes(const rec_gemm_desc* d, const X3DwPlan& pl) {
  return align_up((size_t)pl.slices * d->m * d->ldc * sizeof(float), 256) + align_up((size_t)pl.slices * d->n * sizeof(float), 256);
}
static bool launch_x3_dw(const rec_gemm_desc* d, const float* A, const float* B, float* C, const EpiArgs& e, float* b_colsum,
                         void* workspace, size_t workspace_bytes, hipStream_t st) {
  X3DwPlan pl;
  if (!x3_dw_eligible(d, &pl)) return false;
  if (((uintptr_t)A) % 16 || ((uintptr_t)B) % 16 || ((uintptr_t)C) % 16) return false;
  if (!workspace || ((uintptr_t)workspace) % 16 || workspace_bytes < x3_dw_bytes(d, pl)) return false;
  float* partial = (float*)workspace;
  float* cpart = (float*)((char*)workspace + align_up((size_t)pl.slices * d->m * d->ldc * sizeof(float), 256));
  if (x3_launch_dw(pl, (int)d->m, d->n, d->k, A, d->lda, B, d->ldb, partial, d->ldc, b_colsum ? cpart : nullptr, st) != REC_OK)
    return false;
  GemmPlan sp{};
  sp.splits = pl.slices;
  launch_reduce<REC_EPI_NONE>(d, sp, partial, C, e, st, b_colsum ? cpart : nullptr, b_colsum);
  set_route(REC_GEMM_ROUTE_X3_DW, -1, pl.slices);
  return true;
}

}

using namespace rec;

static size_t plain_workspace_bytes(const rec_gemm_desc* desc) {
  if (skinny_dw(desc)) {
    const size_t z = (size_t)((desc->k + kSkinnyKC - 1) / kSkinnyKC);
    return align_up(z * desc->m * desc->ldc * sizeof(float), 256) + align_up(z * desc->n * sizeof(float), 256);
  }
  const GemmPlan p = plan_gemm(desc);
  return (p.splits > 1 ? align_up((size_t)p.splits * desc->m * desc->ldc * sizeof(float), 256) : 0) +
         align_up((size_t)p.splits * desc->n * sizeof(float), 256);
}

static bool relu_bits_ok(const rec_gemm_desc* d) {
  return (d->epilogue == REC_EPI_BIAS_RELU || d->epilogue == REC_EPI_RELU_MASK) && x3_eligible(d) && d->lda % 4 == 0 &&
         d->ldc % 4 == 0;
}
extern "C" int rec_gemm_relu_bits_bytes(const rec_gemm_desc* desc, int32_t* eligible, size_t* bytes) {
  if (int rc = check_gemm(desc)) return rc;
  REC_REQUIRE(bytes, REC_EINVAL, "bytes is NULL");
  const bool ok = relu_bits_ok(desc);
  if (eligible) *eligible = ok ? 1 : 0;
  *bytes = ok ? align_up(x3_relu_bits_bytes(desc->m, desc->n), 256) : 0;
  return REC_OK;
}

extern "C" int rec_gemm_f32_workspace_bytes(const rec_gemm_desc* desc, size_t* bytes) {
  if (int rc = check_gemm(desc)) return rc;
  REC_REQUIRE(bytes, REC_EINVAL, "bytes is NULL");
  if (skinny_dw(desc)) {
    const size_t z = (size_t)((desc->k + kSkinnyKC - 1) / kSkinnyKC);
    *bytes = align_up(z * desc->m * desc->ldc * sizeof(float), 256) + align_up(z * desc->n * sizeof(float), 256);
    return REC_OK;
  }
  const GemmPlan p = plan_gemm(desc);
  *bytes = (p.splits > 1 ? align_up((size_t)p.splits * desc->m * desc->ldc * sizeof(float), 256) : 0) +
           align_up((size_t)p.splits * desc->n * sizeof(float), 256);
  if (x3_eligible(desc) && *bytes < x3_image_bytes(desc->k, desc->n)) *bytes = align_up(x3_image_bytes(desc->k, desc->n), 256);
  X3DwPlan dwp;
  if (x3_dw_eligible(desc, &dwp) && *bytes < x3_dw_bytes(desc, dwp)) *bytes = x3_dw_bytes(desc, dwp);
  return REC_OK;
}

extern "C" int rec_gemm_b_image_bytes(int32_t k, int32_t n, int32_t* eligible, size_t* bytes) {
  REC_REQUIRE(k > 0 && n > 0 && bytes, REC_EINVAL, "bad arguments");
  const bool ok = n % 4 == 0 && k % 8 == 0 && k >= 64 && x3_cols(n).nt > 0;
  if (eligible) *eligible = ok ? 1 : 0;
  *bytes = ok ? align_up(x3_image_bytes(k, n), 256) : 0;
  return REC_OK;
}

extern "C" int rec_gemm_b_images(int32_t count, const rec_gemm_b_image* items, void* stream) {
  REC_REQUIRE(count >= 0 && (count == 0 || items), REC_EINVAL, "bad arguments");
  for (int32_t at = 0; at < count; at += kX3BatchMax) {
    X3SplitBatch b{};
    b.count = count - at < kX3BatchMax ? count - at : kX3BatchMax;
    int64_t blocks = 0;
    for (int i = 0; i < b.count; ++i) {
      const rec_gemm_b_image& it = items[at + i];
      REC_REQUIRE(it.B && it.image && ((uintptr_t)it.image) % 16 == 0, REC_EINVAL, "item %d: null / unaligned pointer", at + i);
      REC_REQUIRE(it.k > 0 && it.n > 0 && it.n % 4 == 0 && it.k % 8 == 0 && it.k >= 64 && x3_cols(it.n).nt > 0, REC_ESHAPE,
                  "item %d: k %d x n %d has no image form (rec_gemm_b_image_bytes)", at + i, it.k, it.n);
      REC_REQUIRE(it.ldb >= (it.trans_b ? it.k : it.n), REC_EINVAL, "item %d: ldb too small", at + i);
      const X3Cols c = x3_cols(it.n);
      b.W[i] = it.B; b.img[i] = (char*)it.image; b.ldw[i] = it.ldb; b.K[i] = it.k; b.N[i] = it.n;
      b.trans[i] = it.trans_b ? 1 : 0;
      b.nkt[i] = (it.k + 31) / 32; b.np[i] = c.nt * 16; b.ncb[i] = 2 * c.ncb;
      b.first[i] = (unsigned)blocks;
      blocks += ((int64_t)b.ncb[i] * b.nkt[i] * b.np[i] * 4 + kBlock - 1) / kBlock;
    }
    b.first[b.count] = (unsigned)blocks;
    REC_REQUIRE(blocks < (1ll << 31), REC_ESHAPE, "too many blocks");
    hipLaunchKernelGGL(x3_split_batch_kernel, dim3((unsigned)blocks), dim3(kBlock), 0, (hipStream_t)stream, b);
    if (int rc = check_launch("rec_gemm_b_images")) return rc;
  }
  return REC_OK;
}

extern "C" int rec_gemm_last_route(rec_gemm_route* out) {
  REC_REQUIRE(out, REC_EINVAL, "out is NULL");
  *out = g_gemm_route;
  return REC_OK;
}

extern "C" int rec_gemm_plan_splits(const rec_gemm_desc* desc, int32_t num_cus, int32_t* splits) {
  if (int rc = check_gemm(desc)) return rc;
  REC_REQUIRE(splits && num_cus <= kNumCU, REC_EINVAL, "bad arguments");
  rec_gemm_desc d = *desc;
  d.split_k = 0;
  *splits = plan_gemm(&d, num_cus > 0 ? num_cus : kNumCU).splits;
  return REC_OK;
}

extern "C" int rec_gemm_f32_pair(const rec_gemm_desc* desc0, const float* A0, const float* B0, float* C0,
                                 const rec_gemm_epilogue_args* x0, const rec_gemm_desc* desc1, const float* A1,
                                 const float* B1, float* C1, const rec_gemm_epilogue_args* x1, void* workspace,
                                 size_t workspace_bytes, void* stream) {
  if (int rc = check_gemm(desc0)) return rc;
  if (int rc = check_gemm(desc1)) return rc;
  {
    size_t q0 = 0, q1 = 0;
    rec_gemm_f32_workspace_bytes(desc0, &q0);
    rec_gemm_f32_workspace_bytes(desc1, &q1);
    const size_t owed = q0 > q1 ? q0 : q1;
    REC_REQUIRE(owed == 0 || (workspace && workspace_bytes >= owed), REC_EWORKSPACE, "workspace %zu < %zu", workspace_bytes,
                owed);
  }
  static const rec_gemm_epilogue_args kNoArgs = {};
  const rec_gemm_epilogue_args* y0 = x0 ? x0 : &kNoArgs;
  const rec_gemm_epilogue_args* y1 = x1 ? x1 : &kNoArgs;
  const bool shape = desc0->m > 0 && desc1->m > 0 && A0 && B0 && C0 && A1 && B1 && C1 && desc0->trans_a &&
                     desc0->epilogue == REC_EPI_NONE && !desc1->trans_a &&
                     (desc1->epilogue == REC_EPI_NONE ||
                      ((desc1->epilogue == REC_EPI_RELU_MASK || desc1->epilogue == REC_EPI_DSIGMOID) && y1->aux0 &&
                       y1->ld_aux0 >= desc1->n)) &&
                     !y1->b_colsum;
  if (shape) {
    EpiArgs e0{}, e1{};
    e1.aux0 = y1->aux0;
    e1.ld0 = y1->ld_aux0;
    if (launch_direct_pair(desc0, A0, B0, C0, e0, y0->b_colsum, desc1, A1, B1, C1, e1, (hipStream_t)stream))
      return check_launch("rec_gemm_f32_pair");
  }
  if (int rc = rec_gemm_f32(desc0, A0, B0, C0, x0, workspace, workspace_bytes, stream)) return rc;
  return rec_gemm_f32(desc1, A1, B1, C1, x1, workspace, workspace_bytes, stream);
}

extern "C" int rec_gemm_f32(const rec_gemm_desc* desc, const float* A, const float* B, float* C,
                            const rec_gemm_epilogue_args* x, void* workspace,
                            size_t workspace_bytes, void* stream) {
  if (int rc = check_gemm(desc)) return rc;
  if (desc->m == 0) return REC_OK;
  REC_REQUIRE(A && B && C, REC_EINVAL, "null pointer argument");
  static const rec_gemm_epilogue_args kNoArgs = {};
  if (!x) x = &kNoArgs;
  const int epi = desc->epilogue;
  const float* bias = x->bias;
  const float *aux0 = x->aux0, *aux1 = x->aux1;
  const int ld_aux0 = x->ld_aux0, ld_aux1 = x->ld_aux1;
  float* b_colsum = x->b_colsum;
  REC_REQUIRE(!b_colsum || desc->trans_a, REC_EINVAL,
              "b_colsum (the bias gradient) is produced by the trans_a form dW = X^T dY only");
  REC_REQUIRE(!(epi == REC_EPI_BIAS || epi == REC_EPI_BIAS_RELU || epi == REC_EPI_CROSS ||
                epi == REC_EPI_BIAS_SIGMOID || epi == REC_EPI_MOE) || bias, REC_EINVAL,
              "epilogue needs bias");
  unsigned long long* relu_bits = (unsigned long long*)x->relu_bits;
  REC_REQUIRE(!relu_bits || ((epi == REC_EPI_BIAS_RELU || epi == REC_EPI_RELU_MASK) && relu_bits_ok(desc) &&
                             ((uintptr_t)relu_bits) % 8 == 0), REC_EINVAL,
              "relu_bits: only a BIAS_RELU / RELU_MASK call that takes the bf16 x 3 forward / dX kernel "
              "(rec_gemm_relu_bits_bytes says which)");
  REC_REQUIRE(!(epi == REC_EPI_RELU_MASK || epi == REC_EPI_CROSS || epi == REC_EPI_MOE ||
                epi == REC_EPI_DSIGMOID || epi == REC_EPI_DTANH) || (epi == REC_EPI_RELU_MASK && relu_bits) ||
                  (aux0 && ld_aux0 >= desc->n), REC_EINVAL, "epilogue needs aux0");
  REC_REQUIRE(!(epi == REC_EPI_CROSS || epi == REC_EPI_ADD || epi == REC_EPI_MOE) ||
                  (aux1 && ld_aux1 >= desc->n), REC_EINVAL, "epilogue needs aux1");
  REC_REQUIRE(epi != REC_EPI_ADD || !aux0 || ld_aux0 >= desc->n, REC_EINVAL, "bad ld_aux0");
  REC_REQUIRE(epi != REC_EPI_MOE || (x->row_scale && x->row_scale_stride >= 1), REC_EINVAL,
              "epilogue needs row_scale");
  hipStream_t st = (hipStream_t)stream;
  static const int nt_env = [] { const char* v = getenv("REC_GEMM_NT_STORE"); return v && *v ? atoi(v) : 0; }();
  const int nt_store = nt_env == 2 || (nt_env == 1 && epi == REC_EPI_RELU_MASK) ? 1 : 0;
  EpiArgs e{bias, aux0, aux1, x->row_scale, x->out2, ld_aux0, ld_aux1, x->row_scale_stride, x->ld_out2, nt_store, relu_bits};
  REC_REQUIRE(!x->out2 || x->ld_out2 >= desc->n, REC_EINVAL, "bad ld_out2");
  if (skinny_rows(desc) && !b_colsum) {
    const bool vec_a = desc->lda % 4 == 0 && ((uintptr_t)A) % 16 == 0 && desc->k % 4 == 0;
    int64_t grid = (desc->m + kBlock / kWave - 1) / (kBlock / kWave);
    if (grid > kNumCU * 8) grid = kNumCU * 8;
    const size_t shmem = (size_t)desc->n * desc->k * sizeof(float);
#define REC_GEMV_CASE(E)                                                                                   \
  case E:                                                                                                  \
    hipLaunchKernelGGL(gemv_rows_kernel<E>, dim3((unsigned)grid), dim3(kBlock), shmem, st, desc->m, desc->n, \
                       desc->k, A, (int64_t)desc->lda, B, (int64_t)desc->ldb, desc->trans_b != 0, C,       \
                       (int64_t)desc->ldc, e, vec_a);                                                      \
    break;
    switch (epi) {
      REC_GEMV_CASE(REC_EPI_NONE) REC_GEMV_CASE(REC_EPI_BIAS) REC_GEMV_CASE(REC_EPI_BIAS_RELU)
      REC_GEMV_CASE(REC_EPI_RELU_MASK) REC_GEMV_CASE(REC_EPI_CROSS) REC_GEMV_CASE(REC_EPI_BIAS_SIGMOID)
      REC_GEMV_CASE(REC_EPI_BIAS_TANH) REC_GEMV_CASE(REC_EPI_ADD) REC_GEMV_CASE(REC_EPI_MOE)
      REC_GEMV_CASE(REC_EPI_DSIGMOID) REC_GEMV_CASE(REC_EPI_DTANH)
    }
#undef REC_GEMV_CASE
    set_route(REC_GEMM_ROUTE_SKINNY_ROWS, -1, 1, vec_a ? REC_GEMM_ROUTE_VEC_A : 0);
    return check_launch("rec_gemm_f32 (skinny rows)");
  }
  if (skinny_dw(desc) && epi == REC_EPI_NONE) {
    const size_t need = plain_workspace_bytes(desc);
    REC_REQUIRE(workspace && workspace_bytes >= need, REC_EWORKSPACE, "workspace %zu < %zu", workspace_bytes, need);
    const int z = (int)((desc->k + kSkinnyKC - 1) / kSkinnyKC);
    float* part = (float*)workspace;
    float* cpart2 = (float*)((char*)workspace + align_up((size_t)z * desc->m * desc->ldc * sizeof(float), 256));
    hipLaunchKernelGGL(desc->m <= kBlock / 2 ? skinny_dw_narrow_kernel : skinny_dw_kernel, dim3(z), dim3(kBlock), 0, st,
                       (int)desc->m, desc->n, (int64_t)desc->k, A, (int64_t)desc->lda, B, (int64_t)desc->ldb,
                       (int64_t)desc->ldc, part, b_colsum ? cpart2 : nullptr);
    GemmPlan sp;
    sp.splits = z;
    launch_reduce<REC_EPI_NONE>(desc, sp, part, C, e, st);
    if (b_colsum)
      hipLaunchKernelGGL(colsum_reduce_kernel, dim3((desc->n + kBlock - 1) / kBlock), dim3(kBlock), 0, st,
                         desc->n, z, (const float*)cpart2, b_colsum);
    set_route(REC_GEMM_ROUTE_SKINNY_DW, -1, z);
    return check_launch("rec_gemm_f32 (skinny dW)");
  }
  {
    X3DwPlan pl;
    size_t owed = 0;
    if ((x3_dw_eligible(desc, &pl) && ((uintptr_t)A) % 16 == 0 && ((uintptr_t)B) % 16 == 0 && ((uintptr_t)C) % 16 == 0) ||
        (!b_colsum && x3_call_ok(desc, A, C, e) && !(x->b_image && ((uintptr_t)x->b_image) % 16 == 0)))
      rec_gemm_f32_workspace_bytes(desc, &owed);
    REC_REQUIRE(owed == 0 || (workspace && workspace_bytes >= owed), REC_EWORKSPACE, "workspace %zu < %zu", workspace_bytes,
                owed);
  }
  if (launch_x3_dw(desc, A, B, C, e, b_colsum, workspace, workspace_bytes, st)) return check_launch("rec_gemm_f32 (bf16x3 dW)");
  if (!b_colsum && launch_x3(desc, A, B, C, e, x->b_image, workspace, workspace_bytes, st)) {
    set_route(REC_GEMM_ROUTE_X3);
    return check_launch("rec_gemm_f32 (bf16x3)");
  }
  REC_REQUIRE(!relu_bits, REC_EINVAL, "relu_bits: the call did not take the bf16 x 3 kernel (alignment / workspace)");
  if (!b_colsum && launch_panel(desc, A, B, C, e, st, device_cus())) {
    set_route(REC_GEMM_ROUTE_PANEL);
    return check_launch("rec_gemm_f32 (panel)");
  }
  if (!b_colsum && launch_glds(desc, A, B, C, e, st)) {
    set_route(REC_GEMM_ROUTE_GLDS);
    return check_launch("rec_gemm_f32 (glds)");
  }
  if (launch_direct(desc, A, B, C, e, b_colsum, st)) return check_launch("rec_gemm_f32 (direct)");
  const GemmPlan p = plan_gemm(desc);
  REC_REQUIRE(p.tiles_total < (1ll << 31), REC_ESHAPE, "too many tiles");
  float* partial = nullptr;
  float* cpart = nullptr;
  if (p.splits > 1 || b_colsum) {
    const size_t need = plain_workspace_bytes(desc);
    REC_REQUIRE(workspace && workspace_bytes >= need, REC_EWORKSPACE, "workspace %zu < %zu",
                workspace_bytes, need);
    size_t off = 0;
    if (p.splits > 1) {
      partial = (float*)workspace;
      off = align_up((size_t)p.splits * desc->m * desc->ldc * sizeof(float), 256);
    }
    if (b_colsum) cpart = p.splits == 1 ? b_colsum : (float*)((char*)workspace + off);
  }
  static const bool skip_reduce = [] { const char* v = getenv("REC_GEMM_SKIP_REDUCE"); return v && *v == '1'; }();
#define REC_EPI_CASE(E)                                                   \
  case E:                                                                 \
    if (partial) {                                                        \
      launch_epi<REC_EPI_NONE>(desc, p, A, B, C, e, partial, cpart, st);  \
      if (!skip_reduce) launch_reduce<E>(desc, p, partial, C, e, st, cpart, b_colsum); \
    } else {                                                              \
      launch_epi<E>(desc, p, A, B, C, e, nullptr, cpart, st);             \
    }                                                                     \
    break;
  switch (epi) {
    REC_EPI_CASE(REC_EPI_NONE)
    REC_EPI_CASE(REC_EPI_BIAS)
    REC_EPI_CASE(REC_EPI_BIAS_RELU)
    REC_EPI_CASE(REC_EPI_RELU_MASK)
    REC_EPI_CASE(REC_EPI_CROSS)
    REC_EPI_CASE(REC_EPI_BIAS_SIGMOID)
    REC_EPI_CASE(REC_EPI_BIAS_TANH)
    REC_EPI_CASE(REC_EPI_ADD)
    REC_EPI_CASE(REC_EPI_MOE)
    REC_EPI_CASE(REC_EPI_DSIGMOID)
    REC_EPI_CASE(REC_EPI_DTANH)
  }
#undef REC_EPI_CASE
  if (b_colsum && !partial && cpart != b_colsum && !skip_reduce)
    hipLaunchKernelGGL(colsum_reduce_kernel, dim3((desc->n + kBlock - 1) / kBlock), dim3(kBlock), 0,
                       st, desc->n, p.splits, (const float*)cpart, b_colsum);
  return check_launch("rec_gemm_f32");
}
// ... 59 lines not shown
```

### paddlerec_amd/csrc/head_ops.hip

```cpp
#include <stdarg.h>
#include <string.h>

#include <string>

#include "rec_common.h"
#include "tail_roles.h"

namespace rec {

static thread_local char g_err[512] = "";

void set_error(const char* fmt, ...) {
  va_list ap;
  va_start(ap, fmt);
  vsnprintf(g_err, sizeof(g_err), fmt, ap);
  va_end(ap);
}

constexpr int kLossBlocks = 1024;

__global__ __launch_bounds__(kBlock) void sigmoid_logloss_kernel(
    int64_t B, float invB, const float* __restrict__ y1, const float* __restrict__ y2,
    const float* __restrict__ y3, const int64_t* __restrict__ label, float eps, float clip_lo,
    float clip_hi, float* __restrict__ pred, float* __restrict__ dz, float* __restrict__ partial) {
// ... 36 lines not shown
    if ((int)threadIdx.x < o) red[threadIdx.x] += red[threadIdx.x + o];
    __syncthreads();
  }
  if (threadIdx.x == 0) out[0] = red[0] * invB;
}

__global__ __launch_bounds__(kBlock) void bce_logits_kernel(int64_t B, float invB,
                                                            const float* __restrict__ z,
                                                            const float* __restrict__ label,
                                                            float* __restrict__ pred, float* __restrict__ dz,
                                                            float* __restrict__ partial, float* __restrict__ loss_one) {
  __shared__ float red[kBlock / kWave];
  float local = 0.f;
  for (int64_t i = (int64_t)blockIdx.x * kBlock + threadIdx.x; i < B; i += (int64_t)gridDim.x * kBlock) {
    const float zi = z[i], t = label[i];
    local += fmaxf(zi, 0.f) - zi * t + log1pf(expf(-fabsf(zi)));
    const float p = 1.f / (1.f + expf(-zi));
    if (pred) pred[i] = p;
    if (dz) dz[i] = (p - t) * invB;
  }
#pragma unroll
  for (int o = kWave / 2; o > 0; o >>= 1) local += __shfl_xor(local, o, kWave);
  if (threadIdx.x % kWave == 0) red[threadIdx.x / kWave] = local;
  __syncthreads();
  if (threadIdx.x == 0) {
    float t = 0.f;
    for (int w = 0; w < kBlock / kWave; ++w) t += red[w];
    partial[blockIdx.x] = t;
    if (loss_one) loss_one[0] = (0.f + t) * invB;
  }
}

__global__ __launch_bounds__(kBlock) void auc_hist_kernel(
    int64_t B, const float* __restrict__ pred, const int64_t* __restrict__ label, int T,
    unsigned long long* __restrict__ pos, unsigned long long* __restrict__ neg) {
  extern __shared__ int sh[];
  const int nb = T + 1;
  for (int i = threadIdx.x; i < 2 * nb; i += kBlock) sh[i] = 0;
  __syncthreads();
  for (int64_t i = (int64_t)blockIdx.x * kBlock + threadIdx.x; i < B;
       i += (int64_t)gridDim.x * kBlock) {
    int bucket = (int)(pred[i] * (float)T);
    bucket = bucket < 0 ? 0 : (bucket > T ? T : bucket);
    atomicAdd(&sh[(label[i] != 0 ? 0 : nb) + bucket], 1);
  }
  __syncthreads();
  for (int i = threadIdx.x; i < nb; i += kBlock) {
    if (sh[i]) atomicAdd(&pos[i], (unsigned long long)sh[i]);
    if (sh[nb + i]) atomicAdd(&neg[i], (unsigned long long)sh[nb + i]);
  }
}

constexpr int kCtrHeadMaxBlocks = kNumCU * 4;
__global__ __launch_bounds__(kBlock) void ctr_head_kernel(
    int64_t B, int N, float invB, const float* __restrict__ act, int64_t ld_act, const float* __restrict__ w,
    const float* __restrict__ bias, const float* __restrict__ y1, const float* __restrict__ y2,
    const int64_t* __restrict__ label, float eps, float clip_lo, float clip_hi, int relu, float* __restrict__ y_out,
    float* __restrict__ pred, float* __restrict__ dz_out, float* __restrict__ dx, int64_t ld_dx,
    float* __restrict__ partial) {
  extern __shared__ float ctr_red[];
  constexpr int W = kBlock / kWave;
  const int lane = threadIdx.x % kWave, wave = threadIdx.x / kWave;
  const int c0 = lane * 4, c1 = 256 + lane * 4;
  const bool ok0 = c0 < N, ok1 = c1 < N;
  float w0[4] = {0.f, 0.f, 0.f, 0.f}, w1[4] = {0.f, 0.f, 0.f, 0.f};
  if (ok0) vload<4>(w0, w + c0);
  if (ok1) vload<4>(w1, w + c1);
  const float b0 = bias ? bias[0] : 0.f;
  const bool clipped = clip_lo < clip_hi;
  float g0[4] = {0.f, 0.f, 0.f, 0.f}, g1[4] = {0.f, 0.f, 0.f, 0.f}, gb = 0.f, cost_sum = 0.f;
  const int64_t nw = (int64_t)gridDim.x * W;
  for (int64_t r = (int64_t)blockIdx.x * W + wave; r < B; r += 2 * nw) {
    const int64_t rr[2] = {r, r + nw};
    float a0[2][4], a1[2][4];
#pragma unroll
    for (int u = 0; u < 2; ++u) {
#pragma unroll
      for (int v = 0; v < 4; ++v) a0[u][v] = a1[u][v] = 0.f;
      if (rr[u] < B) {
        if (ok0) vload_nt<4>(a0[u], act + rr[u] * ld_act + c0);
        if (ok1) vload_nt<4>(a1[u], act + rr[u] * ld_act + c1);
      }
    }
#pragma unroll
    for (int u = 0; u < 2; ++u) {
      if (rr[u] >= B) continue;
      const int64_t i = rr[u];
      float acc = 0.f;
      acc += a0[u][0] * w0[0] + a0[u][1] * w0[1] + a0[u][2] * w0[2] + a0[u][3] * w0[3];
      acc += a1[u][0] * w1[0] + a1[u][1] * w1[1] + a1[u][2] * w1[2] + a1[u][3] * w1[3];
#pragma unroll
      for (int o = kWave / 2; o > 0; o >>= 1) acc += __shfl_xor(acc, o, kWave);
      const float y = acc + b0;
      float z = y1 ? y1[i] : 0.f;
      if (y2) z += y2[i];
      z = y1 ? z + y : y;
      const float open = (!clipped || (z > clip_lo && z < clip_hi)) ? 1.f : 0.f;
      if (clipped) z = fminf(fmaxf(z, clip_lo), clip_hi);
      const float p = 1.f / (1.f + expf(-z));
      const float t = (float)label[i];
      cost_sum += -t * logf(p + eps) - (1.f - t) * logf(1.f - p + eps);
      const float dz = (-t / (p + eps) + (1.f - t) / (1.f - p + eps)) * invB * (p * (1.f - p)) * open;
      gb += dz;
      if (lane == 0) {
        if (y_out) y_out[i] = y;
        pred[i] = p;
        dz_out[i] = dz;
      }
      float o0[4], o1[4];
#pragma unroll
      for (int v = 0; v < 4; ++v) {
        g0[v] += a0[u][v] * dz;
        g1[v] += a1[u][v] * dz;
        o0[v] = (!relu || a0[u][v] > 0.f) ? dz * w0[v] : 0.f;
        o1[v] = (!relu || a1[u][v] > 0.f) ? dz * w1[v] : 0.f;
      }
      if (ok0) vstore<4>(dx + i * ld_dx + c0, o0);
      if (ok1) vstore<4>(dx + i * ld_dx + c1, o1);
    }
  }
  float* mine = ctr_red + wave * (N + 2);
  if (ok0) { mine[c0] = g0[0]; mine[c0 + 1] = g0[1]; mine[c0 + 2] = g0[2]; mine[c0 + 3] = g0[3]; }
  if (ok1) { mine[c1] = g1[0]; mine[c1 + 1] = g1[1]; mine[c1 + 2] = g1[2]; mine[c1 + 3] = g1[3]; }
  if (lane == 0) { mine[N] = gb; mine[N + 1] = cost_sum; }
  __syncthreads();
  float* prow = partial + (int64_t)blockIdx.x * (N + 2);
  for (int j = threadIdx.x; j < N + 2; j += kBlock) {
    float s = ctr_red[j];
#pragma unroll
    for (int q = 1; q < W; ++q) s += ctr_red[q * (N + 2) + j];
    prow[j] = s;
  }
}

__global__ __launch_bounds__(kBlock) void ctr_head_fold_kernel(int nblk, int n2, const float* __restrict__ partial,
                                                               float invB, float* __restrict__ dw,
                                                               float* __restrict__ db, float* __restrict__ loss) {
  ctr_head_fold_role<false>(blockIdx.x, threadIdx.x, nblk, n2, partial, invB, dw, db, loss, DenseAdam{}, 0, 0);
}

__device__ __forceinline__ uint64_t splitmix64(uint64_t x) {
  x += 0x9E3779B97F4A7C15ull;
  x = (x ^ (x >> 30)) * 0xBF58476D1CE4E5B9ull;
  x = (x ^ (x >> 27)) * 0x94D049BB133111EBull;
  return x ^ (x >> 31);
}

__global__ void fill_uniform_kernel(int64_t n, float* __restrict__ buf, float lo, float hi,
                                    uint64_t seed) {
  for (int64_t i = (int64_t)blockIdx.x * blockDim.x + threadIdx.x; i < n;
       i += (int64_t)gridDim.x * blockDim.x) {
    const uint64_t r = splitmix64(seed ^ splitmix64((uint64_t)i));
    const float u = (float)(r >> 40) * (1.0f / 16777216.0f);
    buf[i] = lo + (hi - lo) * u;
  }
}

}

using namespace rec;

extern "C" const char* rec_last_error(void) { return rec::g_err; }
extern "C" int rec_version(void) { return 100; }

extern "C" int rec_logloss_workspace_bytes(int64_t batch, size_t* bytes) {
  REC_REQUIRE(bytes && batch >= 0, REC_EINVAL, "bad arguments");
  *bytes = kLossBlocks * sizeof(float);
  return REC_OK;
}

extern "C" int rec_sigmoid_logloss(int64_t batch, int64_t mean_over, const float* y1,
                                   const float* y2, const float* y_dnn, const int64_t* label,
                                   float eps, float clip_lo, float clip_hi,
                                   float* pred, float* dz, float* loss_out, void* workspace,
                                   size_t workspace_bytes, void* stream) {
  REC_REQUIRE(batch > 0 && mean_over >= 0 && y1 && label && loss_out, REC_EINVAL,
              "bad arguments");
  const float inv = 1.f / (float)(mean_over > 0 ? mean_over : batch);
  REC_REQUIRE(workspace && workspace_bytes >= kLossBlocks * sizeof(float), REC_EWORKSPACE,
              "workspace too small");
  int64_t grid = (batch + kBlock - 1) / kBlock;
  if (grid > kLossBlocks) grid = kLossBlocks;
  hipStream_t st = (hipStream_t)stream;
  hipLaunchKernelGGL(sigmoid_logloss_kernel, dim3((unsigned)grid), dim3(kBlock), 0, st, batch, inv,
                     y1, y2, y_dnn, label, eps, clip_lo, clip_hi, pred, dz, (float*)workspace);
  hipLaunchKernelGGL(fold_loss_kernel, dim3(1), dim3(kBlock), 0, st, (const float*)workspace,
                     (int)grid, inv, loss_out);
  return check_launch("rec_sigmoid_logloss");
}

static int64_t ctr_head_grid(int64_t batch) {
  const int per = (kBlock / kWave) * (batch <= 4096 ? 2 : 4);
  int64_t grid = (batch + per - 1) / per;
  if (grid > kCtrHeadMaxBlocks) grid = kCtrHeadMaxBlocks;
  return grid < 1 ? 1 : grid;
}

extern "C" int rec_ctr_head_workspace_bytes(int64_t batch, int32_t n, size_t* bytes) {
  REC_REQUIRE(bytes && batch >= 0 && n > 0, REC_EINVAL, "bad arguments");
  *bytes = align_up((size_t)ctr_head_grid(batch) * (n + 2) * sizeof(float), 256);
  return REC_OK;
}

static int ctr_head_impl(int64_t batch, int32_t n, int64_t mean_over, const float* act, int64_t ld_act, const float* w,
                         const float* bias, const float* y1, const float* y2, const int64_t* label, float eps,
                         float clip_lo, float clip_hi, int32_t relu, float* y_dnn, float* pred, float* dz,
                         float* loss_out, float* dx, int64_t ld_dx, float* dw, float* db, void* workspace,
                         size_t workspace_bytes, void* stream, bool fold, int* nblk, float* invB) {
  REC_REQUIRE(batch > 0 && mean_over >= 0, REC_EINVAL, "bad batch");
  REC_REQUIRE(n > 0 && n % 4 == 0 && n <= 512, REC_ESHAPE, "rec_ctr_head_fwd_bwd: n must be a multiple of 4 and <= 512");
  REC_REQUIRE(act && w && label && pred && dz && dx && (!fold || (loss_out && dw && db)), REC_EINVAL,
              "null pointer argument");
  REC_REQUIRE(!y2 || y1, REC_EINVAL, "y2 without y1");
  REC_REQUIRE(ld_act >= n && ld_dx >= n && ld_act % 4 == 0 && ld_dx % 4 == 0 && ((uintptr_t)act) % 16 == 0 &&
                  ((uintptr_t)dx) % 16 == 0 && ((uintptr_t)w) % 16 == 0, REC_ESHAPE,
              "rec_ctr_head_fwd_bwd: act / dx / w must be 16-byte aligned with row strides that are multiples of 4");
  size_t need = 0;
  rec_ctr_head_workspace_bytes(batch, n, &need);
  REC_REQUIRE(workspace && workspace_bytes >= need, REC_EWORKSPACE, "workspace %zu < %zu", workspace_bytes, need);
  const float inv = 1.f / (float)(mean_over > 0 ? mean_over : batch);
  const int64_t grid = ctr_head_grid(batch);
  hipStream_t st = (hipStream_t)stream;
  const size_t shmem = (size_t)(kBlock / kWave) * (n + 2) * sizeof(float);
  hipLaunchKernelGGL(ctr_head_kernel, dim3((unsigned)grid), dim3(kBlock), shmem, st, batch, n, inv, act, ld_act, w, bias, y1,
                     y2, label, eps, clip_lo, clip_hi, relu, y_dnn, pred, dz, dx, ld_dx, (float*)workspace);
  if (fold)
    hipLaunchKernelGGL(ctr_head_fold_kernel, dim3((unsigned)((n + 2 + 15) / 16)), dim3(kBlock), 0, st, (int)grid,
                       n + 2, (const float*)workspace, inv, dw, db, loss_out);
  if (nblk) *nblk = (int)grid;
  if (invB) *invB = inv;
  return check_launch("rec_ctr_head_fwd_bwd");
}

extern "C" int rec_ctr_head_fwd_bwd(int64_t batch, int32_t n, int64_t mean_over, const float* act, int64_t ld_act,
                                    const float* w, const float* bias, const float* y1, const float* y2,
                                    const int64_t* label, float eps, float clip_lo, float clip_hi, int32_t relu,
                                    float* y_dnn, float* pred, float* dz, float* loss_out, float* dx, int64_t ld_dx,
                                    float* dw, float* db, void* workspace, size_t workspace_bytes, void* stream) {
  return ctr_head_impl(batch, n, mean_over, act, ld_act, w, bias, y1, y2, label, eps, clip_lo, clip_hi, relu, y_dnn, pred,
                       dz, loss_out, dx, ld_dx, dw, db, workspace, workspace_bytes, stream, true, nullptr, nullptr);
}

int rec::ctr_head_fwd_bwd_partial(int64_t batch, int32_t n, int64_t mean_over, const float* act, int64_t ld_act,
                                  const float* w, const float* bias, const float* y1, const float* y2,
                                  const int64_t* label, float eps, float clip_lo, float clip_hi, int32_t relu,
                                  float* y_dnn, float* pred, float* dz, float* dx, int64_t ld_dx, void* workspace,
                                  size_t workspace_bytes, void* stream, int* nblk, float* invB) {
  return ctr_head_impl(batch, n, mean_over, act, ld_act, w, bias, y1, y2, label, eps, clip_lo, clip_hi, relu, y_dnn, pred,
                       dz, nullptr, dx, ld_dx, nullptr, nullptr, workspace, workspace_bytes, stream, false, nblk, invB);
}

extern "C" int rec_bce_with_logits(int64_t batch, int64_t mean_over, const float* logit,
                                   const float* label, float* pred, float* dz, float* loss_out,
                                   void* workspace, size_t workspace_bytes, void* stream) {
  REC_REQUIRE(batch > 0 && mean_over >= 0 && logit && label && loss_out, REC_EINVAL, "bad arguments");
  REC_REQUIRE(workspace && workspace_bytes >= kLossBlocks * sizeof(float), REC_EWORKSPACE,
              "workspace too small");
  const float inv = 1.f / (float)(mean_over > 0 ? mean_over : batch);
  int64_t grid = (batch + kBlock - 1) / kBlock;
  if (grid > kLossBlocks) grid = kLossBlocks;
  hipStream_t st = (hipStream_t)stream;
  hipLaunchKernelGGL(bce_logits_kernel, dim3((unsigned)grid), dim3(kBlock), 0, st, batch, inv, logit, label,
                     pred, dz, (float*)workspace, grid == 1 ? loss_out : (float*)nullptr);
  if (grid > 1)
    hipLaunchKernelGGL(fold_loss_kernel, dim3(1), dim3(kBlock), 0, st, (const float*)workspace, (int)grid, inv,
                       loss_out);
  return check_launch("rec_bce_with_logits");
}

extern "C" int rec_auc_histogram(int64_t batch, const float* pred, const int64_t* label,
                                 int32_t num_thresholds, int64_t* stat_pos, int64_t* stat_neg,
                                 void* stream) {
  REC_REQUIRE(batch >= 0 && num_thresholds > 0 && num_thresholds < 16000, REC_EINVAL,
              "bad arguments");
  if (batch == 0) return REC_OK;
  REC_REQUIRE(pred && label && stat_pos && stat_neg, REC_EINVAL, "null pointer argument");
  int64_t grid = (batch + kBlock * 16 - 1) / (kBlock * 16);
  if (grid > kNumCU * 2) grid = kNumCU * 2;
// ... 180 lines not shown
```

### paddlerec_amd/deepfm.py

```python
import math
import os
import time

import torch

from . import ops
from .slot_net import (NUM_THRESHOLDS, SlotDygraphModel, SlotLayerBase, _OnSide, _round_up,
                       auc_metrics, slot_feeds)


class _FlatParams:
    ALIGN = 64

    def __init__(self, shapes, device, reserve=None):
        self.names = [n for n, _ in shapes]
        self.shapes = dict(shapes)
        self.offsets, o = {}, 0
        for n, s in shapes:
            self.offsets[n] = o
            o += -(-max(math.prod(s), (reserve or {}).get(n, 0)) // self.ALIGN) * self.ALIGN
        self.data = torch.zeros(max(o, 1), dtype=torch.float32, device=device)
        self.grad = torch.zeros_like(self.data)
        self.m = torch.zeros_like(self.data)
        self.v = torch.zeros_like(self.data)
# ... 382 lines not shown
        sorted_rg = slot_sort and self.lazy_mode and os.environ.get("REC_DEEPFM_SORTED_GRAD", "0") == "1"
        gspec = os.environ.get("REC_DEEPFM_GROUP_CUS", "")
        gside = side
        pipe = (self.pipelined and side is not None and self.lazy_mode and not small and allreduce is None
                and B >= 16384 and os.environ.get("REC_DEEPFM_DEFER_ALL", "0") != "1")
        if pipe:
            if self._gside is None:
                self._gside = self.k.concurrent_stream(self.device, index=1)
            gside = self._gside
        elif self._side_pending:
            self.sync()
        if gspec and side is not None and hasattr(self.k, "cu_stride_stream"):
            if "," in gspec:
                gside = self.k.cu_range_stream(self.device, 0, int(gspec.split(",")[1]))
            else:
                gside = self.k.cu_stride_stream(self.device, 0, int(gspec))

        def issue_group():
            if small:
                return
            if self.step_count > 3 and os.environ.get("REC_DEEPFM_SKIP_GROUP", "0") == "1":
                return
            with _OnSide(gside, cur):
                if slot_sort:
                    self.k.ids_group_slots(ids, self.slot_rows, self.fm.padding_idx, self.ws_group, self.status, groups,
                                           want_rank=sorted_rg)
                else:
                    self.k.ids_group(ids, self.sparse_feature_number, self.fm.padding_idx, self.ws_group,
                                     self.fm.slot_offset, self.status, groups)
        if group_at == "pre":
            issue_group()
        if self._adam_done is not None and "adam" in os.environ.get("REC_PIPE_SKIP", ""):
            self._adam_done = None
        if self._adam_done is not None:
            cur.wait_event(self._adam_done)
            self._adam_done = None
        if os.environ.get("REC_PIPE_JOIN", "early") == "early":
            self.sync()
        with self._timed("fm_fwd"):
            y1, y2, feat, sum_emb, _ = self._fm_fwd(ids, dense_inputs)
        self.sync()
        if group_at == "fwd":
            issue_group()
        mlp_w, mlp_dw = self._mlp_weights(use_images)
        img_f, img_t = self._image_lists() if use_images else (None, None)
        nl = self.n_linear
        ikw_f = lambda n_: dict(images=img_f[:n_]) if img_f is not None else {}
        ikw_t = lambda n_: dict(images_t=img_t[:n_]) if img_t is not None else {}
        fused_head = self.n_linear > 1 and hasattr(self.k, "ctr_head") and self.k.ctr_head_ok(mlp_w[-1], mlp_dw[-1])
        with self._timed("mlp_fwd"):
            if fused_head:
                h, acts = self.k.mlp_forward(feat.view(B, -1), mlp_w[:-1], self.mlp_b[:-1], self.ws_mlp, relu_last=True,
                                             **ikw_f(nl - 1))
                pred, dz, loss, g_head = self.k.ctr_head(h, mlp_w[-1], self.mlp_b[-1], y1, y2, label, self.ws,
                                                         mlp_dw[-1], self.mlp_db[-1])
            else:
                y_dnn, acts = self.k.mlp_forward(feat.view(B, -1), mlp_w, self.mlp_b, self.ws_mlp, **ikw_f(nl))
        if not fused_head:
            pred, dz, loss = self.k.sigmoid_logloss(y1, y2, y_dnn, label, self.ws)
        if group_at == "bwd":
            issue_group()
        if auc_stats is not None:
            self.k.auc_histogram(pred, label, auc_stats[0], auc_stats[1], NUM_THRESHOLDS)
        defer_all = os.environ.get("REC_DEEPFM_DEFER_ALL", "0") == "1"
        kw = dict(defer_all=True) if defer_all else dict(defer_first=True) if not small else {}
        if overlap and not defer_all and not small and B >= 16384:
            kw.update(defer_split=int(os.environ.get("REC_DW0_SPLIT", "16")))
            kw.update(defer_cus=int(os.environ.get("REC_DW0_CUS", "192")))
        if on_gpu and not defer_all and not self._recording and os.environ.get("REC_MLP_DW_STREAM", "0") == "1":
            if getattr(self, "_dw_stream", None) is None:
                self._dw_stream, self._ws_dw = self.k.concurrent_stream(self.device), self.k.Workspace(self.device)
            kw.update(dw_stream=self._dw_stream, dw_ws=self._ws_dw)
        with self._timed("mlp_bwd"):
            if fused_head:
                res = self.k.mlp_backward(g_head, acts, mlp_w[:-1], mlp_dw[:-1], self.mlp_db[:-1], self.ws_mlp, **kw,
                                          **ikw_t(nl - 1))
            else:
                res = self.k.mlp_backward(dz, acts, mlp_w, mlp_dw, self.mlp_db, self.ws_mlp, **kw, **ikw_t(nl))
            d_flat, finish_dw0 = res if kw else (res, (lambda: None))
        if group_at == "tail":
            issue_group()
        if sorted_rg and side is not None:
            cur.wait_stream(gside)
        with self._timed("fm_bwd"):
            row_grad, _, _ = self.k.deepfm_fm_bwd(
                dense_inputs, feat, sum_emb, d_flat if self.padded else d_flat.view(B, self.fp, -1), dz, dz, S, self.ws,
                out=(self._buf("_rg", (B * S, self.sparse_feature_dim)),
                     self.dense.g["fm.dense_w"].view(self.dense_feature_dim, -1),
                     self.dense.g["fm.dense_w_one"]),
                dense_w=self.dense.p["fm.dense_w"], compact=self.compact,
                **(dict(row_rank=groups.rank) if sorted_rg else {}),
                **(dict(feat_ld=self.ld0) if self.padded else {}))
        t = self.step_count
        st = self.sparse_state
        skw = dict(grad_sorted=True) if sorted_rg else {}
        swap = (side is not None and allreduce is None and not small
                and os.environ.get("REC_DEEPFM_TAIL_SWAP", "0") == "1")
        if not sorted_rg and side is not None and (gside is not side or swap):
            cur.wait_stream(gside)

        def tail_sparse():
            with self._timed("sparse_adam"):
                upd = self.k.sparse_adam_rows if self.lazy_mode else self.k.adam_rows_all
                if small:
                    D = self.sparse_feature_dim
                    self.k.sparse_adam_record_small(ids, self.fm.slot_offset, self.fm.padding_idx, row_grad, dz, S,
                                                    self.fm.rec, st["mv"], D, t, lr, v_offset=_round_up(D, 4),
                                                    status=self.status)
                    return
                pp = self._pp = self.k.segment_partials(groups, row_grad, row_grad.shape[1],
                                                        out=getattr(self, "_pp", None), **skw)
                pp1 = self._pp1 = self.k.segment_partials(groups, dz, 1, grad_div=S, out=getattr(self, "_pp1", None))
                if self.lazy_mode:
                    D = self.sparse_feature_dim
                    self.k.sparse_adam_record(groups, row_grad, dz, S, self.fm.rec, st["mv"], D, t, lr,
                                              v_offset=_round_up(D, 4), partials=pp, partials1=pp1, **skw)
                elif hasattr(self.k, "adam_record_all") and os.environ.get("REC_NONLAZY_RECORD", "1") != "0":
                    D = self.sparse_feature_dim
                    self.k.adam_record_all(groups, row_grad, dz, S, self.fm.rec, st["mv"], D, t, lr,
                                           v_offset=_round_up(D, 4), partials=pp, partials1=pp1)
                else:
                    upd(groups, row_grad, 1, self.fm.embedding, st["m"], st["v"], t, lr, partials=pp)
                    upd(groups, dz, S, self.fm.embedding_one, st["m1"], st["v1"], t, lr, partials=pp1)

        def tail_dense():
            with self._timed("mlp_bwd_dw0"):
                finish_dw0()
                self._fold_backward()
            if allreduce is not None:
# ... 113 lines not shown
```

### paddlerec_amd/ops.py

```python
import collections
import ctypes as C
import os

import torch

from . import _lib
from ._lib import (EPI, AdagradHyper, AdamHyper, AitmHeadDesc, CinView, DcnCrossDesc, DeepFMDesc, DinDesc, EsmHeadDesc, FatFFMDesc, FEFMDesc, FFMDesc, GemmBImage, GemmDesc, GemmEpilogueArgs, GradLayout,
                   GradSrc, LazyInit, MtlMixDesc, MultislotDesc, PsAccessor, PsLayout, RecError, check)

_recorder = None


def lib():
    h = _lib.lib()
    return h if _recorder is None else _recorder.proxy(h)


_raw_stream = getattr(torch._C, "_cuda_getCurrentRawStream", None)
_raw_device = getattr(torch._C, "_cuda_getDevice", None)


def _stream():
    if _raw_stream is not None and _raw_device is not None:
        return C.c_void_p(_raw_stream(_raw_device()))
# ... 2958 lines not shown
    if route is None:
        route = ShardRoute(n, num_shards, dev)
    if status is None:
        status = new_status(dev)
    nbytes = C.c_size_t(0)
    check(lib().rec_shard_route_workspace_bytes(n, num_shards, C.byref(nbytes)))
    w = ws.get(nbytes.value)
    check(lib().rec_shard_route(n, S, num_rows, -1 if padding_idx is None else padding_idx,
                                num_shards, _p(ids), _p(slot_offset), _p(route.send_local_row),
                                _p(route.send_pos), _p(route.send_sample), _p(route.slot_of_pos),
                                _p(route.send_counts), _p(status), _p(w), C.c_size_t(w.numel()),
                                _stream()), "rec_shard_route")
    return route, status


def _chk_mat(t, name):
    if not t.is_cuda:
        raise RecError("%s must be a device tensor (no CPU fallback)" % name)
    if t.dtype != torch.float32 or t.dim() != 2:
        raise RecError("%s must be a 2-D float32 tensor" % name)
    if t.shape[1] > 1 and t.stride(1) != 1:
        raise RecError("%s must have unit column stride" % name)
    return t.stride(0) if t.shape[0] > 1 else max(t.shape[1], 1)


_gemm_ws_cache = {}


class GemmImages:

    def __init__(self, specs, device):
        self.specs, self.images = list(specs), []
        for B, trans_b in self.specs:
            n, k = (B.shape if trans_b else B.shape[::-1])
            ok, nb = C.c_int32(0), C.c_size_t(0)
            check(lib().rec_gemm_b_image_bytes(int(k), int(n), C.byref(ok), C.byref(nb)), "rec_gemm_b_image_bytes")
            self.images.append(torch.empty(nb.value, dtype=torch.uint8, device=device) if ok.value else None)
        live = [(B, t, img) for (B, t), img in zip(self.specs, self.images) if img is not None]
        self._items = (GemmBImage * max(1, len(live)))()
        self._n = len(live)
        for it, (B, t, img) in zip(self._items, live):
            n, k = (B.shape if t else B.shape[::-1])
            it.B, it.ldb, it.k, it.n, it.trans_b, it.image = B.data_ptr(), _chk_mat(B, "B"), int(k), int(n), int(t), img.data_ptr()

    def refresh(self):
        if self._n:
            check(lib().rec_gemm_b_images(self._n, self._items, _stream()), "rec_gemm_b_images")

    def get(self, i):
        return self.images[i]


def gemm(A, B, ws, trans_a=False, trans_b=False, epilogue="none", bias=None, aux0=None, aux1=None,
         out=None, split_k=0, b_colsum=None, row_scale=None, out2=None, num_cus=0, b_image=None, relu_bits=None):
    d, x, out, need = _gemm_prepare(A, B, trans_a, trans_b, epilogue, bias, aux0, aux1, out, split_k, b_colsum, row_scale,
                                    out2, num_cus, b_image)
    if relu_bits is not None:
        nb = _relu_bits_bytes(d)
        if epilogue == "bias_relu":
            t = torch.empty(nb // 8, dtype=torch.int64, device=A.device) if nb else None
            relu_bits.append(t)
            relu_bits = t
        elif nb == 0 or relu_bits.numel() * 8 < nb:
            relu_bits = None
        if relu_bits is not None:
            x.relu_bits = relu_bits.data_ptr()
            if _recorder is not None:
                _recorder.keep.append(relu_bits)
    w = ws.get(need)
    check(lib().rec_gemm_f32(C.byref(d), _p(A), _p(B), _p(out), C.byref(x), _p(w),
                             C.c_size_t(w.numel()), _stream()), "rec_gemm_f32")
    return out


def linear_backward(X, G, W, ws, dW, db, relu_src=None, b_image=None, epilogue=None, aux0=None, relu_bits=None, out=None):
    if epilogue is None:
        epilogue, aux0 = ("relu_mask", relu_src) if relu_src is not None else ("none", None)
    d0, x0, _, need0 = _gemm_prepare(X, G, True, False, "none", None, None, None, dW, 0, db, None, None, 0, None)
    d1, x1, dX, need1 = _gemm_prepare(G, W, False, True, epilogue, None, aux0, None, out, 0, None, None, None, 0, b_image)
    if relu_bits is not None and epilogue == "relu_mask":
        nb = _relu_bits_bytes(d1)
        if nb and relu_bits.numel() * 8 >= nb:
            x1.relu_bits = relu_bits.data_ptr()
            if _recorder is not None:
                _recorder.keep.append(relu_bits)
    w = ws.get(max(need0, need1))
    check(lib().rec_gemm_f32_pair(C.byref(d0), _p(X), _p(G), _p(dW), C.byref(x0), C.byref(d1), _p(G), _p(W), _p(dX),
                                  C.byref(x1), _p(w), C.c_size_t(w.numel()), _stream()), "rec_gemm_f32_pair")
    return dX


GemmRouteInfo = collections.namedtuple("GemmRouteInfo", "family cfg splits flags")


def gemm_last_route():
    r = _lib.GemmRoute()
    check(lib().rec_gemm_last_route(C.byref(r)), "rec_gemm_last_route")
    return GemmRouteInfo(_lib.GEMM_ROUTE_FAMILIES[r.family] if r.family >= 0 else None,
                         _lib.GEMM_CFGS[r.cfg] if r.cfg >= 0 else None, r.splits,
                         frozenset(n for n, b in _lib.GEMM_ROUTE_FLAGS.items() if r.flags & b))


_relu_bits_cache = {}


def _relu_bits_bytes(d):
    if os.environ.get("REC_RELU_BITS") == "0":
        return 0
    key = (d.m, d.n, d.k, d.lda, d.ldb, d.ldc, d.trans_a, d.trans_b, d.epilogue, d.split_k, os.environ.get("REC_GEMM_BF16X3"))
    nb = _relu_bits_cache.get(key)
    if nb is None:
        ok, nbytes = C.c_int32(0), C.c_size_t(0)
        check(lib().rec_gemm_relu_bits_bytes(C.byref(d), C.byref(ok), C.byref(nbytes)), "rec_gemm_relu_bits_bytes")
        nb = _relu_bits_cache[key] = nbytes.value if ok.value else 0
    return nb


def _gemm_prepare(A, B, trans_a, trans_b, epilogue, bias, aux0, aux1, out, split_k, b_colsum, row_scale, out2, num_cus,
                  b_image):
    lda, ldb = _chk_mat(A, "A"), _chk_mat(B, "B")
    K, M = (A.shape if trans_a else A.shape[::-1])
    N, K2 = (B.shape if trans_b else B.shape[::-1])
    if K != K2:
        raise RecError("inner dimensions differ: %d vs %d" % (K, K2))
    if out is None:
        out = torch.empty(M, N, dtype=torch.float32, device=A.device)
    ldc = _chk_mat(out, "out")
    if tuple(out.shape) != (M, N):
        raise RecError("out has shape %s, expected %s" % (tuple(out.shape), (M, N)))
    ld0 = ld1 = 0
    if aux0 is not None:
        ld0 = _chk_mat(aux0, "aux0")
    if aux1 is not None:
        ld1 = _chk_mat(aux1, "aux1")
    if bias is not None:
        _chk(bias, torch.float32, "bias")
        if bias.numel() != N:
            raise RecError("bias must have N elements")
# ... 34 lines not shown
def colsum(G, ws, out=None):
    ld = _chk_mat(G, "G")
    M, N = G.shape
    if out is None:
        out = torch.empty(N, dtype=torch.float32, device=G.device)
    nbytes = C.c_size_t(0)
    check(lib().rec_colsum_workspace_bytes(M, N, C.byref(nbytes)))
    w = ws.get(nbytes.value)
    check(lib().rec_colsum(M, N, ld, _p(G), _p(out), _p(w), C.c_size_t(w.numel()), _stream()),
          "rec_colsum")
    return out


class _Acts(list):
    relu_bits = None


def mlp_forward(x, weights, biases, ws, relu_last=False, out_last=None, images=None):
    acts = _Acts()
    bits = [None]
    n = len(weights)
    for i in range(n):
        acts.append(x)
        last = i == n - 1
        relu = not last or relu_last
        x = gemm(x, weights[i], ws, epilogue="bias_relu" if relu else "bias",
                 bias=biases[i], out=out_last if last else None, b_image=images[i] if images is not None else None,
                 relu_bits=bits if relu else None)
        if not relu:
            bits.append(None)
    acts.append(x)
    acts.relu_bits = bits
    return x, acts


def mlp_head_bwd(act, dz, w, ws, dw, db, relu=True, out=None):
    B, n = act.shape
    if out is None:
        out = torch.empty(B, n, dtype=torch.float32, device=act.device)
    nbytes = C.c_size_t(0)
    check(lib().rec_mlp_head_bwd_workspace_bytes(B, n, C.byref(nbytes)))
    wk = ws.get(nbytes.value)
    check(lib().rec_mlp_head_bwd(B, n, _p(act), act.stride(0), _p(dz), _p(w), 1 if relu else 0, _p(out), out.stride(0),
                                 _p(dw), _p(db), _p(wk), C.c_size_t(wk.numel()), _stream()), "rec_mlp_head_bwd")
    return out


def ctr_head_ok(w, dw):
    return (os.environ.get("REC_CTR_HEAD_FUSED", "1") != "0" and w.dim() == 2 and w.shape[1] == 1 and
            w.shape[0] % 4 == 0 and w.shape[0] <= 512 and w.is_contiguous() and w.data_ptr() % 16 == 0 and
            dw.is_contiguous())


def ctr_head(act, w, bias, y1, y2, label, ws, dw, db, eps=1e-4, clip=None, mean_over=0, relu=True, out=None):
    B, n = act.shape
    dev = act.device
    _chk(label, torch.int64, "label")
    for t, nm in ((y1, "y1"), (y2, "y2"), (bias, "bias")):
        _chk(t, torch.float32, nm)
    if label.numel() != B or (y1 is not None and y1.numel() != B) or (y2 is not None and y2.numel() != B):
        raise RecError("ctr_head: y1 / y2 / label must have one entry per row of act")
    if clip is not None and not clip[0] < clip[1]:
        raise RecError("clip must be (lo, hi) with lo < hi")
    if out is None:
        pred = torch.empty(B, 1, dtype=torch.float32, device=dev)
        dz = torch.empty(B, 1, dtype=torch.float32, device=dev)
        loss = torch.empty(1, dtype=torch.float32, device=dev)
        dx = torch.empty(B, n, dtype=torch.float32, device=dev)
    else:
        pred, dz, loss, dx = out
    nbytes = C.c_size_t(0)
    check(lib().rec_ctr_head_workspace_bytes(B, n, C.byref(nbytes)))
    wk = ws.get(nbytes.value)
    lo, hi = (float(clip[0]), float(clip[1])) if clip is not None else (0.0, 0.0)
    check(lib().rec_ctr_head_fwd_bwd(B, n, int(mean_over), _p(act), act.stride(0), _p(w), _p(bias), _p(y1), _p(y2),
                                     _p(label), float(eps), lo, hi, 1 if relu else 0, None, _p(pred), _p(dz), _p(loss),
                                     _p(dx), dx.stride(0), _p(dw), _p(db), _p(wk), C.c_size_t(wk.numel()), _stream()),
          "rec_ctr_head_fwd_bwd")
    return pred, dz, loss, dx


def _head_ok(act, w, dw, db, dy):
    return (os.environ.get("REC_MLP_HEAD_FUSED", "1") != "0" and w.dim() == 2 and w.shape[1] == 1 and
            w.shape[0] % 4 == 0 and w.shape[0] <= 512 and act.dim() == 2 and act.stride(1) == 1 and
            act.stride(0) % 4 == 0 and act.data_ptr() % 16 == 0 and w.is_contiguous() and w.data_ptr() % 16 == 0 and
            dw.is_contiguous() and dy.is_contiguous() and dy.shape[-1] == 1 and act.shape[0] >= 64)


def mlp_backward(dy, acts, weights, dws, dbs, ws, defer_first=False, defer_all=False, dw_stream=None, dw_ws=None,
                 defer_split=0, images_t=None, defer_cus=0):
    n = len(weights)
    g = dy
    imt = (lambda i: images_t[i]) if images_t is not None else (lambda i: None)
    rbl = getattr(acts, "relu_bits", None)
    rb = (lambda i: rbl[i]) if rbl is not None else (lambda i: None)
    head = n > 1 and _head_ok(acts[n - 1], weights[n - 1], dws[n - 1], dbs[n - 1], dy)
    if head:
        g = mlp_head_bwd(acts[n - 1], dy, weights[n - 1], ws, dws[n - 1], dbs[n - 1], relu=True)
        n_run = n - 1
    else:
        n_run = n
    if defer_all:
        gs = [None] * n_run
        for i in reversed(range(n_run)):
            gs[i] = g
            g = gemm(g, weights[i], ws, trans_b=True, b_image=imt(i),
                     **(dict(epilogue="relu_mask", aux0=acts[i], relu_bits=rb(i)) if i > 0 else {}))

        def finish(num_cus=0):
            for i in reversed(range(n_run)):
                gemm(acts[i], gs[i], ws, trans_a=True, out=dws[i], b_colsum=dbs[i], num_cus=num_cus)
        return g, finish
    cur = torch.cuda.current_stream() if dw_stream is not None else None
    keep = []

    def join():
        if dw_stream is not None:
            cur.wait_stream(dw_stream)
            keep.clear()
    for i in reversed(range(n_run)):
        if i == 0 and defer_first:
            g0 = g
            d_in = gemm(g0, weights[0], ws, trans_b=True, b_image=imt(0))
            join()
            return d_in, (lambda: gemm(acts[0], g0, ws, trans_a=True, out=dws[0], b_colsum=dbs[0], split_k=defer_split,
                                    num_cus=defer_cus))
        if dw_stream is not None:
            dw_stream.wait_stream(cur)
            keep.append(g)
            with torch.cuda.stream(dw_stream):
                gemm(acts[i], g, dw_ws if dw_ws is not None else ws, trans_a=True, out=dws[i], b_colsum=dbs[i])
        else:
            g = linear_backward(acts[i], g, weights[i], ws, dws[i], dbs[i], relu_src=acts[i] if i > 0 else None,
                                b_image=imt(i), relu_bits=rb(i) if i > 0 else None)
            continue
        if i > 0:
            g = gemm(g, weights[i], ws, trans_b=True, epilogue="relu_mask", aux0=acts[i], b_image=imt(i), relu_bits=rb(i))
        else:
            g = gemm(g, weights[i], ws, trans_b=True, b_image=imt(i))
    join()
    return g


def sigmoid_logloss(y1, y2, y_dnn, label, ws, eps=1e-4, want_dz=True, out=None, mean_over=0, clip=None):
    B = y1.numel()
    dev = y1.device
    _chk(y1, torch.float32, "y1")
    _chk(y2, torch.float32, "y2")
    _chk(y_dnn, torch.float32, "y_dnn")
    _chk(label, torch.int64, "label")
    if clip is not None and not clip[0] < clip[1]:
        raise RecError("clip must be (lo, hi) with lo < hi")
    if out is None:
        pred = torch.empty(B, 1, dtype=torch.float32, device=dev)
        dz = torch.empty(B, 1, dtype=torch.float32, device=dev) if want_dz else None
        loss = torch.empty(1, dtype=torch.float32, device=dev)
    else:
        pred, dz, loss = out
    nbytes = C.c_size_t(0)
    check(lib().rec_logloss_workspace_bytes(B, C.byref(nbytes)))
    w = ws.get(nbytes.value)
    lo, hi = (float(clip[0]), float(clip[1])) if clip is not None else (0.0, 0.0)
    check(lib().rec_sigmoid_logloss(B, int(mean_over), _p(y1), _p(y2), _p(y_dnn), _p(label), float(eps), lo, hi,
                                    _p(pred), _p(dz), _p(loss), _p(w), C.c_size_t(w.numel()), _stream()),
          "rec_sigmoid_logloss")
    return pred, dz, loss


def auc_histogram(pred, label, stat_pos, stat_neg, num_thresholds=4095):
    _chk(pred, torch.float32, "pred")
    _chk(label, torch.int64, "label")
    _chk(stat_pos, torch.int64, "stat_pos", (num_thresholds + 1,))
    _chk(stat_neg, torch.int64, "stat_neg", (num_thresholds + 1,))
    check(lib().rec_auc_histogram(pred.numel(), _p(pred), _p(label), num_thresholds, _p(stat_pos),
                                  _p(stat_neg), _stream()), "rec_auc_histogram")


def fill_uniform(buf, lo, hi, seed):
    _chk(buf, torch.float32, "buf")
    check(lib().rec_fill_uniform(buf.numel(), _p(buf), float(lo), float(hi), int(seed), _stream()),
          "rec_fill_uniform")
    return buf


_SIDE_STREAMS = {}


# ... 71 lines not shown
```

Measured before the change: 45.04 million samples/s.

## Generate CTR head input gradient inside the next layer's backward GEMMs

The CTR head no longer materializes its B x 400 input gradient dx. The following layer's dW and dX GEMM kernels rebuild it on the fly from the activation, dz and the head weight (relu(act) ? dz*w : 0) while loading operands. This removes one large f32 write and read of the gradient, in exchange for extra VALU work in the split and convert stages plus new GEN kernel variants. An eligibility query falls back to the old path when the operands don't fit.

```diff
diff --git a/include/recengine.h b/include/recengine.h
--- a/include/recengine.h
+++ b/include/recengine.h
@@ -418,10 +418,15 @@
   float* b_colsum;
   const void* b_image;
   void* relu_bits;
+  const float* gen_dz;
+  const float* gen_w;
 } rec_gemm_epilogue_args;
 
 int rec_gemm_f32_workspace_bytes(const rec_gemm_desc* desc, size_t* bytes);
 int rec_gemm_relu_bits_bytes(const rec_gemm_desc* desc, int32_t* eligible, size_t* bytes);
+int rec_gemm_gen_operand_ok(const rec_gemm_desc* desc, const float* A, const float* B, const float* C,
+                            const rec_gemm_epilogue_args* args, const void* workspace, size_t workspace_size,
+                            int32_t* eligible);
 int rec_gemm_plan_splits(const rec_gemm_desc* desc, int32_t num_cus, int32_t* splits);
 int rec_gemm_f32(const rec_gemm_desc* desc, const float* A, const float* B, float* C,
                  const rec_gemm_epilogue_args* args , void* workspace,
@@ -447,7 +452,8 @@
   REC_GEMM_ROUTE_KS4 = 8,
   REC_GEMM_ROUTE_FOLD = 16,
   REC_GEMM_ROUTE_VEC_A = 32,
-  REC_GEMM_ROUTE_PAIR = 64
+  REC_GEMM_ROUTE_PAIR = 64,
+  REC_GEMM_ROUTE_GEN = 128
 };
 typedef struct {
   int32_t family;
diff --git a/paddlerec_amd/_lib.py b/paddlerec_amd/_lib.py
--- a/paddlerec_amd/_lib.py
+++ b/paddlerec_amd/_lib.py
@@ -143,7 +143,7 @@
 DCN_MAX_LAYERS = CONSTANTS["REC_DCN_MAX_LAYERS"]
 EPI = {name[len("REC_EPI_"):].lower(): value for name, value in CONSTANTS.items() if name.startswith("REC_EPI_")}
 GEMM_ROUTE_FAMILIES = ("skinny_rows", "skinny_dw", "x3_dw", "x3", "panel", "glds", "direct", "tiled")
-GEMM_ROUTE_FLAGS = dict(fast=1, pipe=2, vec=4, ks4=8, fold=16, vec_a=32, pair=64)
+GEMM_ROUTE_FLAGS = dict(fast=1, pipe=2, vec=4, ks4=8, fold=16, vec_a=32, pair=64, gen=128)
 GEMM_CFGS = ("128x80", "256x80", "256x128", "128x128", "80x80", "64x80", "128x80_o4", "144x80")
 
 _lib = None
diff --git a/paddlerec_amd/csrc/deepfm_step.hip b/paddlerec_amd/csrc/deepfm_step.hip
--- a/paddlerec_amd/csrc/deepfm_step.hip
+++ b/paddlerec_amd/csrc/deepfm_step.hip
@@ -231,7 +231,8 @@
 
 int linear_backward(int64_t B, int in, int w, const float* X, const float* G, const float* W, float* dW, float* db,
                     float* dX, const float* mask, const Buffers& bf, void* st, const void* b_image_t,
-                    void* mask_bits = nullptr) {
+                    void* mask_bits = nullptr, const float* gen_dz = nullptr, const float* gen_w = nullptr,
+                    bool* gen_ok = nullptr) {
   rec_gemm_desc d0{}, d1{};
   d0.m = in; d0.n = w; d0.k = (int)B; d0.lda = in; d0.ldb = w; d0.ldc = w; d0.trans_a = 1; d0.epilogue = REC_EPI_NONE;
   d1.m = B; d1.n = in; d1.k = w; d1.lda = w; d1.ldb = w; d1.ldc = in; d1.trans_b = 1;
@@ -239,6 +240,15 @@
   rec_gemm_epilogue_args x0{}, x1{};
   x0.b_colsum = db;
   x1.aux0 = mask; x1.ld_aux0 = mask ? in : 0; x1.b_image = b_image_t; x1.relu_bits = mask ? mask_bits : nullptr;
+  x0.gen_dz = x1.gen_dz = gen_dz;
+  x0.gen_w = x1.gen_w = gen_w;
+  if (gen_ok) {
+    int32_t ok0 = 0, ok1 = 0;
+    if (int rc = rec_gemm_gen_operand_ok(&d0, X, G, dW, &x0, bf.ws, bf.ws_bytes, &ok0)) return rc;
+    if (int rc = rec_gemm_gen_operand_ok(&d1, G, W, dX, &x1, bf.ws, bf.ws_bytes, &ok1)) return rc;
+    *gen_ok = ok0 && ok1;
+    return REC_OK;
+  }
   return rec_gemm_f32_pair(&d0, X, G, dW, &x0, &d1, G, W, dX, &x1, bf.ws, bf.ws_bytes, st);
 }
 
@@ -386,6 +396,13 @@
                            flat_pair(net->dense_w_one, net->g_dense_w_one, Dn)));
   int head_nblk = 0;
   float head_inv = 0.f;
+  static const bool gen_env = [] { const char* v = getenv("REC_CTR_HEAD_IN_GEMM"); return !(v && *v == '0'); }();
+  bool head_gen = false;
+  if (s.ctr_head && !tail && gen_env && n >= 3) {
+    const int i = n - 2, in = net->widths[i - 1], w = net->widths[i];
+    REC_TRY(linear_backward(B, in, w, bf.act[i], bf.act[n - 1], net->w[i], net->gw[i], net->gb[i], bf.g[1], bf.act[i], bf,
+                            stream, bf.img_t[i], bf.relu_bits[i], bf.dz, net->w[n - 1], &head_gen));
+  }
   if (s.ctr_head) {
     const int nh = net->widths[n - 2];
     if (tail)
@@ -394,9 +411,9 @@
                                        stream, &head_nblk, &head_inv));
     else
     REC_TRY(rec_ctr_head_fwd_bwd(B, nh, 0, bf.act[n - 1], nh, net->w[n - 1], net->b[n - 1], bf.y1, bf.y2, label, 1e-4f,
-                                 0.f, 0.f, 1, nullptr, pred_out, bf.dz, loss_out, bf.g[gi], nh, net->gw[n - 1],
-                                 net->gb[n - 1], bf.ws, bf.ws_bytes, stream));
-    g = bf.g[gi];
+                                 0.f, 0.f, 1, nullptr, pred_out, bf.dz, loss_out, head_gen ? nullptr : bf.g[gi], nh,
+                                 net->gw[n - 1], net->gb[n - 1], bf.ws, bf.ws_bytes, stream));
+    g = head_gen ? bf.act[n - 1] : bf.g[gi];
     gi ^= 1;
     n_run = n - 1;
   } else {
@@ -429,8 +446,9 @@
                    bf.img_t[0]));
       break;
     }
+    const bool gen = head_gen && i == n_run - 1;
     REC_TRY(linear_backward(B, in, w, bf.act[i], g, net->w[i], net->gw[i], net->gb[i], bf.g[gi], bf.act[i], bf, stream,
-                            bf.img_t[i], bf.relu_bits[i]));
+                            bf.img_t[i], bf.relu_bits[i], gen ? bf.dz : nullptr, gen ? net->w[n - 1] : nullptr));
     g = bf.g[gi];
     gi ^= 1;
   }
diff --git a/paddlerec_amd/csrc/gemm_bf16x3.h b/paddlerec_amd/csrc/gemm_bf16x3.h
--- a/paddlerec_amd/csrc/gemm_bf16x3.h
+++ b/paddlerec_amd/csrc/gemm_bf16x3.h
@@ -56,6 +56,29 @@
   p2 = x3_cvt_pk(se, so);
 }
 
+__device__ __forceinline__ float x3_sub1(float a, float b) {
+  float r;
+  asm("v_sub_f32 %0, %1, %2" : "=v"(r) : "v"(a), "v"(b));
+  return r;
+}
+__device__ __forceinline__ float x3_mul1(float a, float b) {
+  float r;
+  asm("v_mul_f32 %0, %1, %2" : "=v"(r) : "v"(a), "v"(b));
+  return r;
+}
+__device__ __forceinline__ void x3_split_pair1(float xe, float xo, unsigned& p0, unsigned& p1, unsigned& p2) {
+  p0 = x3_cvt_pk(xe, xo);
+  const float re = x3_sub1(xe, __uint_as_float(p0 << 16)), ro = x3_sub1(xo, __uint_as_float(p0 & 0xffff0000u));
+  p1 = x3_cvt_pk(re, ro);
+  const float se = x3_sub1(re, __uint_as_float(p1 << 16)), so = x3_sub1(ro, __uint_as_float(p1 & 0xffff0000u));
+  p2 = x3_cvt_pk(se, so);
+}
+#ifndef REC_X3_SPLIT_SINGLE
+#define REC_X3_SPLIT_SINGLE 1
+#endif
+
+__device__ __forceinline__ float x3_gen(float act, float dz, float w) { return act > 0.f ? __fmul_rn(dz, w) : 0.f; }
+
 __device__ __forceinline__ void x3_split_one(const float* __restrict__ W, int64_t ldw, int K, int N, int trans,
                                              char* __restrict__ img, int nkt, int np, int ncb, int64_t tid) {
   if (tid >= (int64_t)ncb * nkt * np * 4) return;
@@ -158,10 +181,10 @@
 #define REC_X3_PRODUCTS 6
 #endif
 
-template <int NT, int EPI, int WM, int WN>
-__global__ __launch_bounds__(WM * WN * 64, WN == 1 ? 2 : 1) void gemm_bf16x3_kernel(
+template <int NT, int EPI, int WM, int WN, bool GEN>
+__device__ __forceinline__ void x3_gemm_body(
     int64_t M, int N, int K, const float* __restrict__ A, int64_t lda, const char* __restrict__ Bimg_all,
-    float* __restrict__ C, int64_t ldc, EpiArgs epi, int ncb) {
+    float* __restrict__ C, int64_t ldc, const EpiArgs& epi, int ncb) {
   using Geo = X3Geo<NT>;
   constexpr int MT = kX3BM / 16 / WM;
   constexpr int NW = WM * WN;
@@ -187,11 +210,14 @@
   const char* Bimg = Bimg_all + (size_t)cb0 * nkt * Geo::Stage;
 
   const float* ap[MT];
+  float gen_dzr[GEN ? MT : 1];
+  float4 gen_wraw[2];
 #pragma unroll
   for (int a = 0; a < MT; ++a) {
     int64_t r = m0 + a * 16 + li;
     r = r < M ? r : M - 1;
     ap[a] = A + r * lda + g * 8;
+    if constexpr (GEN) gen_dzr[a] = epi.gen_dz[r];
   }
   float4 araw[MT][2];
   auto load_a = [&](int kt) {
@@ -203,6 +229,10 @@
     for (int a = 0; a < MT; ++a) {
       araw[a][0] = *reinterpret_cast<const float4*>(ap[a] + koff);
       araw[a][1] = *reinterpret_cast<const float4*>(ap[a] + koff + 4);
+    }
+    if constexpr (GEN) {
+      gen_wraw[0] = *reinterpret_cast<const float4*>(epi.gen_w + koff + g * 8);
+      gen_wraw[1] = *reinterpret_cast<const float4*>(epi.gen_w + koff + g * 8 + 4);
     }
   };
   auto issue_b = [&](int kt, int stage) {
@@ -244,15 +274,23 @@
     }
 #pragma unroll
     for (int a = 0; a < MT; ++a) {
-      const float x[8] = {araw[a][0].x, araw[a][0].y, araw[a][0].z, araw[a][0].w,
-                          araw[a][1].x, araw[a][1].y, araw[a][1].z, araw[a][1].w};
+      float x[8] = {araw[a][0].x, araw[a][0].y, araw[a][0].z, araw[a][0].w,
+                    araw[a][1].x, araw[a][1].y, araw[a][1].z, araw[a][1].w};
+      if constexpr (GEN) {
+        const float wv[8] = {gen_wraw[0].x, gen_wraw[0].y, gen_wraw[0].z, gen_wraw[0].w,
+                             gen_wraw[1].x, gen_wraw[1].y, gen_wraw[1].z, gen_wraw[1].w};
+#pragma unroll
+        for (int j = 0; j < 8; ++j)
+          x[j] = REC_X3_SPLIT_SINGLE ? (x[j] > 0.f ? x3_mul1(gen_dzr[a], wv[j]) : 0.f) : x3_gen(x[j], gen_dzr[a], wv[j]);
+      }
 #pragma unroll
       for (int d = 0; d < 4; ++d) {
 #if REC_X3_LAB == 4
         af[a][0][d] = __float_as_uint(x[2 * d]); af[a][1][d] = __float_as_uint(x[2 * d + 1]); af[a][2][d] = __float_as_uint(x[2 * d]) ^ 1u;
 #else
         unsigned p0, p1, p2;
-        x3_split_pair(x[2 * d], x[2 * d + 1], p0, p1, p2);
+        if (REC_X3_SPLIT_SINGLE) x3_split_pair1(x[2 * d], x[2 * d + 1], p0, p1, p2);
+        else x3_split_pair(x[2 * d], x[2 * d + 1], p0, p1, p2);
         af[a][0][d] = p0; af[a][1][d] = p1; af[a][2][d] = p2;
 #endif
       }
@@ -369,6 +407,19 @@
       if (bits_at && row_ok) *bits_at = mbits;
     }
   }
+}
+
+template <int NT, int EPI, int WM, int WN>
+__global__ __launch_bounds__(WM * WN * 64, WN == 1 ? 2 : 1) void gemm_bf16x3_kernel(
+    int64_t M, int N, int K, const float* __restrict__ A, int64_t lda, const char* __restrict__ Bimg_all,
+    float* __restrict__ C, int64_t ldc, EpiArgs epi, int ncb) {
+  x3_gemm_body<NT, EPI, WM, WN, false>(M, N, K, A, lda, Bimg_all, C, ldc, epi, ncb);
+}
+template <int NT, int EPI, int WM, int WN>
+__global__ __launch_bounds__(WM * WN * 64, WN == 1 ? 2 : 1) void gemm_bf16x3_gen_kernel(
+    int64_t M, int N, int K, const float* __restrict__ A, int64_t lda, const char* __restrict__ Bimg_all,
+    float* __restrict__ C, int64_t ldc, EpiArgs epi, int ncb) {
+  x3_gemm_body<NT, EPI, WM, WN, true>(M, N, K, A, lda, Bimg_all, C, ldc, epi, ncb);
 }
 
 constexpr int kX3DwCols = 208;
@@ -418,10 +469,12 @@
   int slices, steps_per_slice;
   float* P; int64_t ldp;
   float* cpart;
+  const float* gen_dz;
+  const float* gen_w;
 };
 
-template <int PW, bool PIPE>
-__global__ __launch_bounds__(256) void gemm_bf16x3_dw_kernel(X3DwArgs w) {
+template <int PW, bool PIPE, bool GEN>
+__device__ __forceinline__ void x3_dw_body(const X3DwArgs& w) {
   extern __shared__ __attribute__((aligned(1024))) char x3_smem[];
   const int tid = threadIdx.x;
   const int lane = tid % kWave;
@@ -450,6 +503,13 @@
   const float* xp = w.X + (row0 + mg * 8) * w.ldx + (x_ok ? xc : 0);
   const float* gp = w.G + (row0 + mg * 8) * w.ldg + (g_ok ? gc : 0);
   float4 xr[8], gr[8];
+  float4 gen_dzr[2];
+  float4 gen_wc = make_float4(0.f, 0.f, 0.f, 0.f);
+  const float* gen_dzp = nullptr;
+  if constexpr (GEN) {
+    gen_dzp = w.gen_dz + row0 + mg * 8;
+    if (g_ok) gen_wc = *reinterpret_cast<const float4*>(w.gen_w + gc);
+  }
   auto load_patches = [&](int kt) {
 #ifdef REC_X3_DW_NO_LOADS
     if (kt > 0) return;
@@ -458,6 +518,10 @@
     for (int r = 0; r < 8; ++r) {
       xr[r] = *reinterpret_cast<const float4*>(xp + ((int64_t)kt * 32 + r) * w.ldx);
       gr[r] = *reinterpret_cast<const float4*>(gp + ((int64_t)kt * 32 + r) * w.ldg);
+    }
+    if constexpr (GEN) {
+      gen_dzr[0] = *reinterpret_cast<const float4*>(gen_dzp + (int64_t)kt * 32);
+      gen_dzr[1] = *reinterpret_cast<const float4*>(gen_dzp + (int64_t)kt * 32 + 4);
     }
   };
   unsigned wr_off[4];
@@ -480,6 +544,13 @@
     }
     asm volatile("" : "+v"(xv[0]), "+v"(xv[1]), "+v"(xv[2]), "+v"(xv[3]), "+v"(xv[4]), "+v"(xv[5]), "+v"(xv[6]), "+v"(xv[7]),
                       "+v"(gv[0]), "+v"(gv[1]), "+v"(gv[2]), "+v"(gv[3]), "+v"(gv[4]), "+v"(gv[5]), "+v"(gv[6]), "+v"(gv[7]));
+    if constexpr (GEN) {
+      const float we = e == 0 ? gen_wc.x : e == 1 ? gen_wc.y : e == 2 ? gen_wc.z : gen_wc.w;
+      const float dz[8] = {gen_dzr[0].x, gen_dzr[0].y, gen_dzr[0].z, gen_dzr[0].w,
+                           gen_dzr[1].x, gen_dzr[1].y, gen_dzr[1].z, gen_dzr[1].w};
+#pragma unroll
+      for (int r = 0; r < 8; ++r) gv[r] = x3_gen(gv[r], dz[r], we);
+    }
 #pragma unroll
     for (int d = 0; d < 4; ++d) {
       unsigned a, b, c;
@@ -614,7 +685,7 @@
           if (cv) __builtin_amdgcn_sched_group_barrier(0x002, REC_X3_DW_VALU_PER_MFMA, 0);
           if (wr && i % PW == PW / 2) __builtin_amdgcn_sched_group_barrier(0x200, 1, 0);
         }
-        if (cv) __builtin_amdgcn_sched_group_barrier(0x002, 32, 0);
+        if (cv) __builtin_amdgcn_sched_group_barrier(0x002, GEN ? 64 : 32, 0);
       }
       } else if (MORE && t >= kX3DwWT - 4) {
         convert_part(stage ^ 1, t - (kX3DwWT - 4));
@@ -623,7 +694,7 @@
           __builtin_amdgcn_sched_group_barrier(0x008, 1, 0);
           __builtin_amdgcn_sched_group_barrier(0x002, REC_X3_DW_VALU_PER_MFMA, 0);
         }
-        __builtin_amdgcn_sched_group_barrier(0x002, 32, 0);
+        __builtin_amdgcn_sched_group_barrier(0x002, GEN ? 64 : 32, 0);
         __builtin_amdgcn_sched_group_barrier(0x200, 6, 0);
       }
 #endif
@@ -664,6 +735,11 @@
   }
 }
 
+template <int PW, bool PIPE>
+__global__ __launch_bounds__(256) void gemm_bf16x3_dw_kernel(X3DwArgs w) { x3_dw_body<PW, PIPE, false>(w); }
+template <int PW, bool PIPE>
+__global__ __launch_bounds__(256) void gemm_bf16x3_dw_gen_kernel(X3DwArgs w) { x3_dw_body<PW, PIPE, true>(w); }
+
 template <int PW>
 struct X3Dw8Acc { f32x4_t v[PW][kX3DwWT]; };
 
@@ -674,19 +750,34 @@
   float4 raw[8];
   float4 csum;
   float* P; int64_t ldp; int kin, nout, k_tile0, n_tile0, my_k0, my_n0, my_p, my_q, li, g;
+  const float* gen_dzp; float4 gen_dzr[2]; float4 gen_wc; float gen_thr; unsigned gen_keep;
+  template <bool GEN>
   __device__ __forceinline__ void load_patch(int kt) {
 #pragma unroll
     for (int r = 0; r < 8; ++r) raw[r] = *reinterpret_cast<const float4*>(src + ((int64_t)kt * 32 + r) * ld);
-  }
+    if constexpr (GEN) {
+      gen_dzr[0] = *reinterpret_cast<const float4*>(gen_dzp + (int64_t)kt * 32);
+      gen_dzr[1] = *reinterpret_cast<const float4*>(gen_dzp + (int64_t)kt * 32 + 4);
+    }
+  }
+  template <bool GEN>
   __device__ __forceinline__ void convert(int e, u32x4_t (&ch)[3]) {
     float v[8];
 #pragma unroll
     for (int r = 0; r < 8; ++r) v[r] = e == 0 ? raw[r].x : e == 1 ? raw[r].y : e == 2 ? raw[r].z : raw[r].w;
     asm volatile("" : "+v"(v[0]), "+v"(v[1]), "+v"(v[2]), "+v"(v[3]), "+v"(v[4]), "+v"(v[5]), "+v"(v[6]), "+v"(v[7]));
+    if constexpr (GEN) {
+      const float we = e == 0 ? gen_wc.x : e == 1 ? gen_wc.y : e == 2 ? gen_wc.z : gen_wc.w;
+      const float dz[8] = {gen_dzr[0].x, gen_dzr[0].y, gen_dzr[0].z, gen_dzr[0].w,
+                           gen_dzr[1].x, gen_dzr[1].y, gen_dzr[1].z, gen_dzr[1].w};
+#pragma unroll
+      for (int r = 0; r < 8; ++r)
+        v[r] = v[r] > gen_thr ? __fmul_rn(dz[r], we) : __uint_as_float(__float_as_uint(v[r]) & gen_keep);
+    }
     float cs = 0.f;
 #pragma unroll
     for (int d = 0; d < 4; ++d) {
-      const float u0 = ok ? v[2 * d] : 0.f, u1 = ok ? v[2 * d + 1] : 0.f;
+      const float u0 = GEN || ok ? v[2 * d] : 0.f, u1 = GEN || ok ? v[2 * d + 1] : 0.f;
       cs += u0 + u1;
       unsigned a, b, cc;
       x3_split_pair(u0, u1, a, b, cc);
@@ -716,7 +807,7 @@
   }
 };
 
-template <int PW>
+template <int PW, bool GEN>
 __device__ __forceinline__ void x3_dw8_run(X3Dw8Ctx& c, int nsteps) {
   X3Dw8Acc<PW> acc;
 #pragma unroll
@@ -726,7 +817,7 @@
   auto step = [&](int kt, auto more_c) {
     constexpr bool MORE = decltype(more_c)::value;
     const int stage = kt & 1;
-    if (MORE) c.load_patch(kt + 1);
+    if (MORE) c.template load_patch<GEN>(kt + 1);
     __builtin_amdgcn_sched_barrier(0);
     const unsigned so = stage * kX3Stage;
     u32x4_t af[PW][3];
@@ -777,14 +868,14 @@
       if (MORE && t >= kX3DwWT - 5) {
         const bool wr = t >= kX3DwWT - 4, cv = t <= kX3DwWT - 2;
         if (wr) c.write(stage ^ 1, t - (kX3DwWT - 4), pend);
-        if (cv) c.convert(t - (kX3DwWT - 5), pend);
+        if (cv) c.template convert<GEN>(t - (kX3DwWT - 5), pend);
 #pragma unroll
         for (int i = 0; i < 6 * PW; ++i) {
           __builtin_amdgcn_sched_group_barrier(0x008, 1, 0);
           if (cv) __builtin_amdgcn_sched_group_barrier(0x002, REC_X3_DW_VALU_PER_MFMA, 0);
           if (wr && i % (2 * PW) == PW) __builtin_amdgcn_sched_group_barrier(0x200, 1, 0);
         }
-        if (cv) __builtin_amdgcn_sched_group_barrier(0x002, 32, 0);
+        if (cv) __builtin_amdgcn_sched_group_barrier(0x002, GEN ? 64 : 32, 0);
       }
       __builtin_amdgcn_sched_barrier(0);
     }
@@ -795,8 +886,8 @@
   c.store(acc.v);
 }
 
-template <int PW>
-__global__ __launch_bounds__(512) void gemm_bf16x3_dw_kernel_w8(X3DwArgs w) {
+template <int PW, bool GEN>
+__device__ __forceinline__ void x3_dw8_body(const X3DwArgs& w) {
   static_assert(PW >= 2 && PW <= 4, "four X tiles at most fit the 256-register budget");
   extern __shared__ __attribute__((aligned(1024))) char x3_smem[];
   const int tid = threadIdx.x;
@@ -819,7 +910,9 @@
   int nsteps = (int)min((int64_t)w.steps_per_slice, (w.rows - row0) / 32);
   if (nsteps < 0) nsteps = 0;
 
-  const int op = wave >> 2, s = tid & 255;
+  constexpr bool REMAP = GEN && PW == 4;
+  const int op = REMAP ? (wave >= 3 && wave <= 6 ? 1 : 0) : wave >> 2;
+  const int s = REMAP ? (op ? wave - 3 : (wave == 7 ? 3 : wave)) * 64 + lane : tid & 255;
   const bool stager = s < 4 * (kX3DwCols / 4);
   const int sp = stager ? s : s - 4 * (kX3DwCols / 4);
   const int mg = sp / (kX3DwCols / 4), cg = sp % (kX3DwCols / 4);
@@ -830,6 +923,12 @@
 
   X3Dw8Ctx c;
   c.src = src; c.ld = ld; c.ok = ok;
+  if constexpr (GEN) {
+    c.gen_dzp = w.gen_dz + row0 + mg * 8;
+    c.gen_wc = op && ok ? *reinterpret_cast<const float4*>(w.gen_w + col) : make_float4(0.f, 0.f, 0.f, 0.f);
+    c.gen_thr = op && ok ? 0.f : __builtin_inff();
+    c.gen_keep = !op && ok ? 0xffffffffu : 0u;
+  }
   c.base = x3_smem + op * kX3DwOperand;
 #pragma unroll
   for (int e = 0; e < 4; ++e) {
@@ -848,17 +947,17 @@
   c.my_p = my_p; c.my_q = my_q; c.li = li; c.g = g;
 
   if (nsteps > 0) {
-    c.load_patch(0);
+    c.template load_patch<GEN>(0);
 #pragma unroll
     for (int e = 0; e < 4; ++e) {
       u32x4_t ch[3];
-      c.convert(e, ch);
+      c.template convert<GEN>(e, ch);
       c.write(0, e, ch);
     }
   }
   __syncthreads();
-  if (my_p == PW) x3_dw8_run<PW>(c, nsteps);
-  else x3_dw8_run<PW - 1>(c, nsteps);
+  if (my_p == PW) x3_dw8_run<PW, GEN && !REMAP>(c, nsteps);
+  else x3_dw8_run<PW - 1, GEN>(c, nsteps);
 
   if (w.cpart && kb == 0) {
     float4* red = reinterpret_cast<float4*>(x3_smem);
@@ -875,6 +974,11 @@
   }
 }
 
+template <int PW>
+__global__ __launch_bounds__(512) void gemm_bf16x3_dw_kernel_w8(X3DwArgs w) { x3_dw8_body<PW, false>(w); }
+template <int PW>
+__global__ __launch_bounds__(512) void gemm_bf16x3_dw_gen_kernel_w8(X3DwArgs w) { x3_dw8_body<PW, true>(w); }
+
 inline int x3_launch_split(const float* W, int64_t ldw, int K, int N, int trans, char* img, hipStream_t st) {
   const X3Cols c = x3_cols(N);
   const int nkt = (K + 31) / 32, np = c.nt * 16, ncb = 2 * c.ncb;
@@ -891,13 +995,17 @@
          ((uintptr_t)A % 16) == 0 && ((uintptr_t)C % 16) == 0;
 }
 
-template <int NT, int EPI, int WM, int WN>
+template <int NT, int EPI, int WM, int WN, bool GEN = false>
 inline int x3_launch_gemm_wm(int64_t M, int N, int K, const float* A, int64_t lda, const char* img, float* C, int64_t ldc,
                              const EpiArgs& e, int ncb, hipStream_t st) {
   static std::atomic<bool> attr_set{false};
   constexpr int lds = 2 * WN * X3Geo<NT>::Stage;
+  const auto kernel = [] {
+    if constexpr (GEN) return &gemm_bf16x3_gen_kernel<NT, EPI, WM, WN>;
+    else return &gemm_bf16x3_kernel<NT, EPI, WM, WN>;
+  }();
   if (!attr_set.load(std::memory_order_acquire)) {
-    if (hipFuncSetAttribute(reinterpret_cast<const void*>(&gemm_bf16x3_kernel<NT, EPI, WM, WN>),
+    if (hipFuncSetAttribute(reinterpret_cast<const void*>(kernel),
                             hipFuncAttributeMaxDynamicSharedMemorySize, lds) != hipSuccess) {
       (void)hipGetLastError();
       set_error("gemm_bf16x3: %d B of dynamic LDS refused", lds);
@@ -909,10 +1017,10 @@
   if constexpr (WN == 1) {
     const int64_t grid = (row_tiles + 7) / 8 * 8 * ncb;
     if (grid >= (1ll << 31)) { set_error("gemm_bf16x3: too many workgroups"); return REC_ESHAPE; }
-    hipLaunchKernelGGL((gemm_bf16x3_kernel<NT, EPI, WM, WN>), dim3((unsigned)grid), dim3(WM * WN * 64), lds, st, M, N, K, A,
+    hipLaunchKernelGGL(kernel, dim3((unsigned)grid), dim3(WM * WN * 64), lds, st, M, N, K, A,
                        lda, img, C, ldc, e, ncb);
   } else {
-    hipLaunchKernelGGL((gemm_bf16x3_kernel<NT, EPI, WM, WN>), dim3((unsigned)row_tiles, (unsigned)(ncb / WN)),
+    hipLaunchKernelGGL(kernel, dim3((unsigned)row_tiles, (unsigned)(ncb / WN)),
                        dim3(WM * WN * 64), lds, st, M, N, K, A, lda, img, C, ldc, e, ncb);
   }
   return check_launch("gemm_bf16x3_kernel");
@@ -925,34 +1033,43 @@
   static const int v = [] { const char* e = getenv("REC_X3_WN"); return e && *e == '2' ? 2 : 1; }();
   return v;
 }
-template <int NT, int EPI>
+template <int NT, int EPI, bool GEN>
 inline int x3_launch_gemm_cfg(int64_t M, int N, int K, const float* A, int64_t lda, const char* img, float* C, int64_t ldc,
                               const EpiArgs& e, int ncb, hipStream_t st) {
   if constexpr (EpiUses<EPI>::aux1) {
     return x3_launch_gemm_wm<NT, EPI, 2, 2>(M, N, K, A, lda, img, C, ldc, e, ncb, st);
   } else {
     if (REC_X3_WM == 4 && x3_wn_default() == 1)
-      return x3_launch_gemm_wm<NT, EPI, 4, 1>(M, N, K, A, lda, img, C, ldc, e, ncb, st);
-    return x3_launch_gemm_wm<NT, EPI, REC_X3_WM, 2>(M, N, K, A, lda, img, C, ldc, e, ncb, st);
-  }
-}
-
-template <int EPI>
+      return x3_launch_gemm_wm<NT, EPI, 4, 1, GEN>(M, N, K, A, lda, img, C, ldc, e, ncb, st);
+    return x3_launch_gemm_wm<NT, EPI, REC_X3_WM, 2, GEN>(M, N, K, A, lda, img, C, ldc, e, ncb, st);
+  }
+}
+
+template <int EPI, bool GEN = false>
 inline int x3_launch_gemm_epi(int64_t M, int N, int K, const float* A, int64_t lda, const char* img, float* C, int64_t ldc,
                               const EpiArgs& e, hipStream_t st) {
   const X3Cols c = x3_cols(N);
   switch (c.nt) {
-    case 13: return x3_launch_gemm_cfg<13, EPI>(M, N, K, A, lda, img, C, ldc, e, 2 * c.ncb, st);
-    case 8: return x3_launch_gemm_cfg<8, EPI>(M, N, K, A, lda, img, C, ldc, e, 2 * c.ncb, st);
-    case 7: return x3_launch_gemm_cfg<7, EPI>(M, N, K, A, lda, img, C, ldc, e, 2 * c.ncb, st);
+    case 13: return x3_launch_gemm_cfg<13, EPI, GEN>(M, N, K, A, lda, img, C, ldc, e, 2 * c.ncb, st);
+    case 8: return x3_launch_gemm_cfg<8, EPI, GEN>(M, N, K, A, lda, img, C, ldc, e, 2 * c.ncb, st);
+    case 7: return x3_launch_gemm_cfg<7, EPI, GEN>(M, N, K, A, lda, img, C, ldc, e, 2 * c.ncb, st);
     default: set_error("gemm_bf16x3: no column blocking for N = %d", N); return REC_ESHAPE;
   }
 }
 
 inline bool x3_epilogue_ok(int epi) { return epi >= REC_EPI_NONE && epi <= REC_EPI_DTANH; }
+
+inline bool x3_gen_epilogue_ok(int epi) { return epi == REC_EPI_NONE || epi == REC_EPI_RELU_MASK; }
 
 inline int x3_launch_gemm(int epi, int64_t M, int N, int K, const float* A, int64_t lda, const char* img, float* C,
                           int64_t ldc, const EpiArgs& e, hipStream_t st) {
+  if (e.gen_dz) {
+    switch (epi) {
+      case REC_EPI_NONE: return x3_launch_gemm_epi<REC_EPI_NONE, true>(M, N, K, A, lda, img, C, ldc, e, st);
+      case REC_EPI_RELU_MASK: return x3_launch_gemm_epi<REC_EPI_RELU_MASK, true>(M, N, K, A, lda, img, C, ldc, e, st);
+      default: set_error("gemm_bf16x3: no generated operand under epilogue %d", epi); return REC_EINVAL;
+    }
+  }
   switch (epi) {
     case REC_EPI_NONE: return x3_launch_gemm_epi<REC_EPI_NONE>(M, N, K, A, lda, img, C, ldc, e, st);
     case REC_EPI_BIAS: return x3_launch_gemm_epi<REC_EPI_BIAS>(M, N, K, A, lda, img, C, ldc, e, st);
@@ -994,13 +1111,17 @@
   return hipFuncSetAttribute(reinterpret_cast<const void*>(kernel), hipFuncAttributeMaxDynamicSharedMemorySize, lds) == hipSuccess;
 }
 inline int x3_launch_dw(const X3DwPlan& pl, int kin, int nout, int64_t rows, const float* X, int64_t ldx, const float* G,
-                        int64_t ldg, float* P, int64_t ldp, float* cpart, hipStream_t st, int form = -1) {
+                        int64_t ldg, float* P, int64_t ldp, float* cpart, hipStream_t st, int form = -1,
+                        const float* gen_dz = nullptr, const float* gen_w = nullptr) {
   static std::atomic<bool> attr_set{false};
   constexpr int lds = 2 * kX3Stage + 4096;
   if (!attr_set.load(std::memory_order_acquire)) {
     if (!x3_dw_lds_attr(&gemm_bf16x3_dw_kernel<7, true>, lds) || !x3_dw_lds_attr(&gemm_bf16x3_dw_kernel<5, true>, lds) ||
         !x3_dw_lds_attr(&gemm_bf16x3_dw_kernel<7, false>, lds) || !x3_dw_lds_attr(&gemm_bf16x3_dw_kernel<5, false>, lds) ||
-        !x3_dw_lds_attr(&gemm_bf16x3_dw_kernel_w8<4>, lds) || !x3_dw_lds_attr(&gemm_bf16x3_dw_kernel_w8<3>, lds)) {
+        !x3_dw_lds_attr(&gemm_bf16x3_dw_kernel_w8<4>, lds) || !x3_dw_lds_attr(&gemm_bf16x3_dw_kernel_w8<3>, lds) ||
+        !x3_dw_lds_attr(&gemm_bf16x3_dw_gen_kernel<7, true>, lds) || !x3_dw_lds_attr(&gemm_bf16x3_dw_gen_kernel<5, true>, lds) ||
+        !x3_dw_lds_attr(&gemm_bf16x3_dw_gen_kernel<7, false>, lds) || !x3_dw_lds_attr(&gemm_bf16x3_dw_gen_kernel<5, false>, lds) ||
+        !x3_dw_lds_attr(&gemm_bf16x3_dw_gen_kernel_w8<4>, lds) || !x3_dw_lds_attr(&gemm_bf16x3_dw_gen_kernel_w8<3>, lds)) {
       (void)hipGetLastError();
       set_error("gemm_bf16x3_dw: %d B of dynamic LDS refused", lds);
       return REC_EHIP;
@@ -1008,19 +1129,30 @@
     attr_set.store(true, std::memory_order_release);
   }
   X3DwArgs w{X, ldx, G, ldg, rows, kin, nout, pl.kb_tiles, pl.nb_tiles, pl.kblocks, pl.nblocks, pl.slices,
-             pl.steps_per_slice, P, ldp, cpart};
+             pl.steps_per_slice, P, ldp, cpart, gen_dz, gen_w};
+  const bool gen = gen_dz != nullptr;
   const unsigned grid = (unsigned)(pl.slices * pl.kblocks * pl.nblocks);
   static const int env_form = [] {
     const char* v = getenv("REC_X3_DW_FORM");
     return v && *v ? (*v != '0' ? 1 : 0) : REC_X3_DW_FORM_DEFAULT;
   }();
   if ((form < 0 ? env_form : form) != 0) {
-    if ((pl.kb_tiles + 3) / 4 >= 4) hipLaunchKernelGGL((gemm_bf16x3_dw_kernel_w8<4>), dim3(grid), dim3(512), lds, st, w);
+    const bool p4 = (pl.kb_tiles + 3) / 4 >= 4;
+    if (p4 && gen) hipLaunchKernelGGL((gemm_bf16x3_dw_gen_kernel_w8<4>), dim3(grid), dim3(512), lds, st, w);
+    else if (gen) hipLaunchKernelGGL((gemm_bf16x3_dw_gen_kernel_w8<3>), dim3(grid), dim3(512), lds, st, w);
+    else if (p4) hipLaunchKernelGGL((gemm_bf16x3_dw_kernel_w8<4>), dim3(grid), dim3(512), lds, st, w);
     else hipLaunchKernelGGL((gemm_bf16x3_dw_kernel_w8<3>), dim3(grid), dim3(512), lds, st, w);
     return check_launch("gemm_bf16x3_dw_kernel_w8");
   }
   static const bool pipe = [] { const char* v = getenv("REC_X3_DW_PIPE"); return v && *v ? *v != '0' : REC_X3_DW_PIPE_STORES != 0; }();
   const bool p5 = (pl.kb_tiles + 1) / 2 <= 5;
+  if (gen) {
+    if (p5 && pipe) hipLaunchKernelGGL((gemm_bf16x3_dw_gen_kernel<5, true>), dim3(grid), dim3(256), lds, st, w);
+    else if (p5) hipLaunchKernelGGL((gemm_bf16x3_dw_gen_kernel<5, false>), dim3(grid), dim3(256), lds, st, w);
+    else if (pipe) hipLaunchKernelGGL((gemm_bf16x3_dw_gen_kernel<7, true>), dim3(grid), dim3(256), lds, st, w);
+    else hipLaunchKernelGGL((gemm_bf16x3_dw_gen_kernel<7, false>), dim3(grid), dim3(256), lds, st, w);
+    return check_launch("gemm_bf16x3_dw_kernel");
+  }
   if (p5 && pipe) hipLaunchKernelGGL((gemm_bf16x3_dw_kernel<5, true>), dim3(grid), dim3(256), lds, st, w);
   else if (p5) hipLaunchKernelGGL((gemm_bf16x3_dw_kernel<5, false>), dim3(grid), dim3(256), lds, st, w);
   else if (pipe) hipLaunchKernelGGL((gemm_bf16x3_dw_kernel<7, true>), dim3(grid), dim3(256), lds, st, w);
diff --git a/paddlerec_amd/csrc/gemm_epi.h b/paddlerec_amd/csrc/gemm_epi.h
--- a/paddlerec_amd/csrc/gemm_epi.h
+++ b/paddlerec_amd/csrc/gemm_epi.h
@@ -85,6 +85,8 @@
   int ld0, ld1, rs_stride, ld2;
   int nt_store;
   unsigned long long* relu_bits;
+  const float* gen_dz;
+  const float* gen_w;
 };
 
 template <int EPI>
diff --git a/paddlerec_amd/csrc/gemm_f32.hip b/paddlerec_amd/csrc/gemm_f32.hip
--- a/paddlerec_amd/csrc/gemm_f32.hip
+++ b/paddlerec_amd/csrc/gemm_f32.hip
@@ -776,12 +776,13 @@
   if (!workspace || ((uintptr_t)workspace) % 16 || workspace_bytes < x3_dw_bytes(d, pl)) return false;
   float* partial = (float*)workspace;
   float* cpart = (float*)((char*)workspace + align_up((size_t)pl.slices * d->m * d->ldc * sizeof(float), 256));
-  if (x3_launch_dw(pl, (int)d->m, d->n, d->k, A, d->lda, B, d->ldb, partial, d->ldc, b_colsum ? cpart : nullptr, st) != REC_OK)
+  if (x3_launch_dw(pl, (int)d->m, d->n, d->k, A, d->lda, B, d->ldb, partial, d->ldc, b_colsum ? cpart : nullptr, st, -1,
+                   e.gen_dz, e.gen_w) != REC_OK)
     return false;
   GemmPlan sp{};
   sp.splits = pl.slices;
   launch_reduce<REC_EPI_NONE>(d, sp, partial, C, e, st, b_colsum ? cpart : nullptr, b_colsum);
-  set_route(REC_GEMM_ROUTE_X3_DW, -1, pl.slices);
+  set_route(REC_GEMM_ROUTE_X3_DW, -1, pl.slices, e.gen_dz ? REC_GEMM_ROUTE_GEN : 0);
   return true;
 }
 
@@ -809,6 +810,34 @@
   const bool ok = relu_bits_ok(desc);
   if (eligible) *eligible = ok ? 1 : 0;
   *bytes = ok ? align_up(x3_relu_bits_bytes(desc->m, desc->n), 256) : 0;
+  return REC_OK;
+}
+
+static bool gen_operand_ok(const rec_gemm_desc* d, const float* A, const float* B, const float* C,
+                           const rec_gemm_epilogue_args* x, const void* workspace, size_t workspace_bytes) {
+  if (!A || !B || !C || !x || !x->gen_dz || !x->gen_w) return false;
+  if (((uintptr_t)x->gen_dz) % 16 || ((uintptr_t)x->gen_w) % 16) return false;
+  if (skinny_rows(d) || skinny_dw(d)) return false;
+  if (d->trans_a) {
+    X3DwPlan pl;
+    if (!x3_dw_eligible(d, &pl)) return false;
+    if (((uintptr_t)A) % 16 || ((uintptr_t)B) % 16 || ((uintptr_t)C) % 16) return false;
+    return workspace && ((uintptr_t)workspace) % 16 == 0 && workspace_bytes >= x3_dw_bytes(d, pl);
+  }
+  if (!x3_gen_epilogue_ok(d->epilogue) || x->b_colsum) return false;
+  EpiArgs e{};
+  e.aux0 = x->aux0; e.ld0 = x->ld_aux0; e.aux1 = x->aux1; e.ld1 = x->ld_aux1; e.out2 = x->out2; e.ld2 = x->ld_out2;
+  if (!x3_call_ok(d, A, C, e)) return false;
+  if (x->relu_bits && (!relu_bits_ok(d) || ((uintptr_t)x->relu_bits) % 8)) return false;
+  if (x->b_image && ((uintptr_t)x->b_image) % 16 == 0) return true;
+  return workspace && ((uintptr_t)workspace) % 16 == 0 && workspace_bytes >= x3_image_bytes(d->k, d->n);
+}
+extern "C" int rec_gemm_gen_operand_ok(const rec_gemm_desc* desc, const float* A, const float* B, const float* C,
+                                       const rec_gemm_epilogue_args* args, const void* workspace, size_t workspace_size,
+                                       int32_t* eligible) {
+  if (int rc = check_gemm(desc)) return rc;
+  REC_REQUIRE(eligible, REC_EINVAL, "eligible is NULL");
+  *eligible = gen_operand_ok(desc, A, B, C, args, workspace, workspace_size) ? 1 : 0;
   return REC_OK;
 }
 
@@ -901,7 +930,7 @@
                      (desc1->epilogue == REC_EPI_NONE ||
                       ((desc1->epilogue == REC_EPI_RELU_MASK || desc1->epilogue == REC_EPI_DSIGMOID) && y1->aux0 &&
                        y1->ld_aux0 >= desc1->n)) &&
-                     !y1->b_colsum;
+                     !y1->b_colsum && !y0->gen_dz && !y0->gen_w && !y1->gen_dz && !y1->gen_w;
   if (shape) {
     EpiArgs e0{}, e1{};
     e1.aux0 = y1->aux0;
@@ -947,7 +976,11 @@
   hipStream_t st = (hipStream_t)stream;
   static const int nt_env = [] { const char* v = getenv("REC_GEMM_NT_STORE"); return v && *v ? atoi(v) : 0; }();
   const int nt_store = nt_env == 2 || (nt_env == 1 && epi == REC_EPI_RELU_MASK) ? 1 : 0;
-  EpiArgs e{bias, aux0, aux1, x->row_scale, x->out2, ld_aux0, ld_aux1, x->row_scale_stride, x->ld_out2, nt_store, relu_bits};
+  REC_REQUIRE((!x->gen_dz && !x->gen_w) || gen_operand_ok(desc, A, B, C, x, workspace, workspace_bytes), REC_EINVAL,
+              "gen_dz / gen_w: only a call that takes a bf16 x 3 kernel with a generated operand "
+              "(rec_gemm_gen_operand_ok says which)");
+  EpiArgs e{bias, aux0, aux1, x->row_scale, x->out2, ld_aux0, ld_aux1, x->row_scale_stride, x->ld_out2, nt_store, relu_bits,
+            x->gen_dz, x->gen_w};
   REC_REQUIRE(!x->out2 || x->ld_out2 >= desc->n, REC_EINVAL, "bad ld_out2");
   if (skinny_rows(desc) && !b_colsum) {
     const bool vec_a = desc->lda % 4 == 0 && ((uintptr_t)A) % 16 == 0 && desc->k % 4 == 0;
@@ -999,10 +1032,11 @@
   }
   if (launch_x3_dw(desc, A, B, C, e, b_colsum, workspace, workspace_bytes, st)) return check_launch("rec_gemm_f32 (bf16x3 dW)");
   if (!b_colsum && launch_x3(desc, A, B, C, e, x->b_image, workspace, workspace_bytes, st)) {
-    set_route(REC_GEMM_ROUTE_X3);
+    set_route(REC_GEMM_ROUTE_X3, -1, 1, e.gen_dz ? REC_GEMM_ROUTE_GEN : 0);
     return check_launch("rec_gemm_f32 (bf16x3)");
   }
   REC_REQUIRE(!relu_bits, REC_EINVAL, "relu_bits: the call did not take the bf16 x 3 kernel (alignment / workspace)");
+  REC_REQUIRE(!e.gen_dz, REC_EINVAL, "gen_dz / gen_w: the call did not take a bf16 x 3 kernel");
   if (!b_colsum && launch_panel(desc, A, B, C, e, st, device_cus())) {
     set_route(REC_GEMM_ROUTE_PANEL);
     return check_launch("rec_gemm_f32 (panel)");
diff --git a/paddlerec_amd/csrc/head_ops.hip b/paddlerec_amd/csrc/head_ops.hip
--- a/paddlerec_amd/csrc/head_ops.hip
+++ b/paddlerec_amd/csrc/head_ops.hip
@@ -112,6 +112,7 @@
 }
 
 constexpr int kCtrHeadMaxBlocks = kNumCU * 4;
+template <bool STORE_DX>
 __global__ __launch_bounds__(kBlock) void ctr_head_kernel(
     int64_t B, int N, float invB, const float* __restrict__ act, int64_t ld_act, const float* __restrict__ w,
     const float* __restrict__ bias, const float* __restrict__ y1, const float* __restrict__ y2,
@@ -175,8 +176,10 @@
         o0[v] = (!relu || a0[u][v] > 0.f) ? dz * w0[v] : 0.f;
         o1[v] = (!relu || a1[u][v] > 0.f) ? dz * w1[v] : 0.f;
       }
-      if (ok0) vstore<4>(dx + i * ld_dx + c0, o0);
-      if (ok1) vstore<4>(dx + i * ld_dx + c1, o1);
+      if constexpr (STORE_DX) {
+        if (ok0) vstore<4>(dx + i * ld_dx + c0, o0);
+        if (ok1) vstore<4>(dx + i * ld_dx + c1, o1);
+      }
     }
   }
   float* mine = ctr_red + wave * (N + 2);
@@ -269,8 +272,9 @@
                          size_t workspace_bytes, void* stream, bool fold, int* nblk, float* invB) {
   REC_REQUIRE(batch > 0 && mean_over >= 0, REC_EINVAL, "bad batch");
   REC_REQUIRE(n > 0 && n % 4 == 0 && n <= 512, REC_ESHAPE, "rec_ctr_head_fwd_bwd: n must be a multiple of 4 and <= 512");
-  REC_REQUIRE(act && w && label && pred && dz && dx && (!fold || (loss_out && dw && db)), REC_EINVAL,
+  REC_REQUIRE(act && w && label && pred && dz && (!fold || (loss_out && dw && db)), REC_EINVAL,
               "null pointer argument");
+  if (!dx) ld_dx = ld_act;
   REC_REQUIRE(!y2 || y1, REC_EINVAL, "y2 without y1");
   REC_REQUIRE(ld_act >= n && ld_dx >= n && ld_act % 4 == 0 && ld_dx % 4 == 0 && ((uintptr_t)act) % 16 == 0 &&
                   ((uintptr_t)dx) % 16 == 0 && ((uintptr_t)w) % 16 == 0, REC_ESHAPE,
@@ -282,8 +286,12 @@
   const int64_t grid = ctr_head_grid(batch);
   hipStream_t st = (hipStream_t)stream;
   const size_t shmem = (size_t)(kBlock / kWave) * (n + 2) * sizeof(float);
-  hipLaunchKernelGGL(ctr_head_kernel, dim3((unsigned)grid), dim3(kBlock), shmem, st, batch, n, inv, act, ld_act, w, bias, y1,
-                     y2, label, eps, clip_lo, clip_hi, relu, y_dnn, pred, dz, dx, ld_dx, (float*)workspace);
+  if (dx)
+    hipLaunchKernelGGL(ctr_head_kernel<true>, dim3((unsigned)grid), dim3(kBlock), shmem, st, batch, n, inv, act, ld_act, w,
+                       bias, y1, y2, label, eps, clip_lo, clip_hi, relu, y_dnn, pred, dz, dx, ld_dx, (float*)workspace);
+  else
+    hipLaunchKernelGGL(ctr_head_kernel<false>, dim3((unsigned)grid), dim3(kBlock), shmem, st, batch, n, inv, act, ld_act, w,
+                       bias, y1, y2, label, eps, clip_lo, clip_hi, relu, y_dnn, pred, dz, dx, ld_dx, (float*)workspace);
   if (fold)
     hipLaunchKernelGGL(ctr_head_fold_kernel, dim3((unsigned)((n + 2 + 15) / 16)), dim3(kBlock), 0, st, (int)grid,
                        n + 2, (const float*)workspace, inv, dw, db, loss_out);
diff --git a/paddlerec_amd/deepfm.py b/paddlerec_amd/deepfm.py
--- a/paddlerec_amd/deepfm.py
+++ b/paddlerec_amd/deepfm.py
@@ -458,8 +458,22 @@
             if fused_head:
                 h, acts = self.k.mlp_forward(feat.view(B, -1), mlp_w[:-1], self.mlp_b[:-1], self.ws_mlp, relu_last=True,
                                              **ikw_f(nl - 1))
-                pred, dz, loss, g_head = self.k.ctr_head(h, mlp_w[-1], self.mlp_b[-1], y1, y2, label, self.ws,
-                                                         mlp_dw[-1], self.mlp_db[-1])
+                head_gen = None
+                if hasattr(self.k, "head_in_gemm") and not small and not self._recording:
+                    dz_buf = torch.empty(B, 1, dtype=torch.float32, device=self.device)
+                    hkw = dict(defer_all=os.environ.get("REC_DEEPFM_DEFER_ALL", "0") == "1",
+                               dw_stream=True if os.environ.get("REC_MLP_DW_STREAM", "0") == "1" else None)
+                    head_gen = self.k.head_in_gemm(acts, mlp_w[:-1], mlp_dw[:-1], self.mlp_db[:-1], self.ws_mlp,
+                                                   dz_buf, mlp_w[-1], **ikw_t(nl - 1), **hkw)
+                if head_gen is not None:
+                    hout = (torch.empty(B, 1, dtype=torch.float32, device=self.device), dz_buf,
+                            torch.empty(1, dtype=torch.float32, device=self.device), None)
+                    pred, dz, loss, _ = self.k.ctr_head(h, mlp_w[-1], self.mlp_b[-1], y1, y2, label, self.ws,
+                                                        mlp_dw[-1], self.mlp_db[-1], out=hout, want_dx=False)
+                    g_head = h
+                else:
+                    pred, dz, loss, g_head = self.k.ctr_head(h, mlp_w[-1], self.mlp_b[-1], y1, y2, label, self.ws,
+                                                             mlp_dw[-1], self.mlp_db[-1])
             else:
                 y_dnn, acts = self.k.mlp_forward(feat.view(B, -1), mlp_w, self.mlp_b, self.ws_mlp, **ikw_f(nl))
         if not fused_head:
@@ -480,7 +494,7 @@
         with self._timed("mlp_bwd"):
             if fused_head:
                 res = self.k.mlp_backward(g_head, acts, mlp_w[:-1], mlp_dw[:-1], self.mlp_db[:-1], self.ws_mlp, **kw,
-                                          **ikw_t(nl - 1))
+                                          **ikw_t(nl - 1), **(dict(head_gen=head_gen) if head_gen is not None else {}))
             else:
                 res = self.k.mlp_backward(dz, acts, mlp_w, mlp_dw, self.mlp_db, self.ws_mlp, **kw, **ikw_t(nl))
             d_flat, finish_dw0 = res if kw else (res, (lambda: None))
diff --git a/paddlerec_amd/ops.py b/paddlerec_amd/ops.py
--- a/paddlerec_amd/ops.py
+++ b/paddlerec_amd/ops.py
@@ -3034,9 +3034,13 @@
 
 
 def gemm(A, B, ws, trans_a=False, trans_b=False, epilogue="none", bias=None, aux0=None, aux1=None,
-         out=None, split_k=0, b_colsum=None, row_scale=None, out2=None, num_cus=0, b_image=None, relu_bits=None):
+         out=None, split_k=0, b_colsum=None, row_scale=None, out2=None, num_cus=0, b_image=None, relu_bits=None, gen=None):
     d, x, out, need = _gemm_prepare(A, B, trans_a, trans_b, epilogue, bias, aux0, aux1, out, split_k, b_colsum, row_scale,
                                     out2, num_cus, b_image)
+    if gen is not None:
+        x.gen_dz, x.gen_w = gen[0].data_ptr(), gen[1].data_ptr()
+        if _recorder is not None:
+            _recorder.keep.extend(gen)
     if relu_bits is not None:
         nb = _relu_bits_bytes(d)
         if epilogue == "bias_relu":
@@ -3055,7 +3059,8 @@
     return out
 
 
-def linear_backward(X, G, W, ws, dW, db, relu_src=None, b_image=None, epilogue=None, aux0=None, relu_bits=None, out=None):
+def linear_backward(X, G, W, ws, dW, db, relu_src=None, b_image=None, epilogue=None, aux0=None, relu_bits=None, out=None,
+                    gen=None, gen_query=False):
     if epilogue is None:
         epilogue, aux0 = ("relu_mask", relu_src) if relu_src is not None else ("none", None)
     d0, x0, _, need0 = _gemm_prepare(X, G, True, False, "none", None, None, None, dW, 0, db, None, None, 0, None)
@@ -3066,6 +3071,26 @@
             x1.relu_bits = relu_bits.data_ptr()
             if _recorder is not None:
                 _recorder.keep.append(relu_bits)
+    if gen is not None:
+        dz, wl = gen
+        _chk(dz, torch.float32, "gen dz")
+        _chk(wl, torch.float32, "gen w")
+        if dz.numel() != G.shape[0] or wl.numel() != G.shape[1] or not (dz.is_contiguous() and wl.is_contiguous()):
+            raise RecError("gen: dz must be contiguous with one entry per row of G, w with one per column")
+        x0.gen_dz = x1.gen_dz = dz.data_ptr()
+        x0.gen_w = x1.gen_w = wl.data_ptr()
+        if _recorder is not None:
+            _recorder.keep.extend((dz, wl))
+    if gen_query:
+        if gen is None or not hasattr(lib(), "rec_gemm_gen_operand_ok"):
+            return False
+        w = ws.get(max(need0, need1))
+        ok0, ok1 = C.c_int32(0), C.c_int32(0)
+        check(lib().rec_gemm_gen_operand_ok(C.byref(d0), _p(X), _p(G), _p(dW), C.byref(x0), _p(w), C.c_size_t(w.numel()),
+                                            C.byref(ok0)), "rec_gemm_gen_operand_ok")
+        check(lib().rec_gemm_gen_operand_ok(C.byref(d1), _p(G), _p(W), _p(dX), C.byref(x1), _p(w), C.c_size_t(w.numel()),
+                                            C.byref(ok1)), "rec_gemm_gen_operand_ok")
+        return bool(ok0.value and ok1.value)
     w = ws.get(max(need0, need1))
     check(lib().rec_gemm_f32_pair(C.byref(d0), _p(X), _p(G), _p(dW), C.byref(x0), C.byref(d1), _p(G), _p(W), _p(dX),
                                   C.byref(x1), _p(w), C.c_size_t(w.numel()), _stream()), "rec_gemm_f32_pair")
@@ -3206,7 +3231,7 @@
             dw.is_contiguous())
 
 
-def ctr_head(act, w, bias, y1, y2, label, ws, dw, db, eps=1e-4, clip=None, mean_over=0, relu=True, out=None):
+def ctr_head(act, w, bias, y1, y2, label, ws, dw, db, eps=1e-4, clip=None, mean_over=0, relu=True, out=None, want_dx=True):
     B, n = act.shape
     dev = act.device
     _chk(label, torch.int64, "label")
@@ -3220,16 +3245,18 @@
         pred = torch.empty(B, 1, dtype=torch.float32, device=dev)
         dz = torch.empty(B, 1, dtype=torch.float32, device=dev)
         loss = torch.empty(1, dtype=torch.float32, device=dev)
-        dx = torch.empty(B, n, dtype=torch.float32, device=dev)
+        dx = torch.empty(B, n, dtype=torch.float32, device=dev) if want_dx else None
     else:
         pred, dz, loss, dx = out
+        dx = dx if want_dx else None
     nbytes = C.c_size_t(0)
     check(lib().rec_ctr_head_workspace_bytes(B, n, C.byref(nbytes)))
     wk = ws.get(nbytes.value)
     lo, hi = (float(clip[0]), float(clip[1])) if clip is not None else (0.0, 0.0)
     check(lib().rec_ctr_head_fwd_bwd(B, n, int(mean_over), _p(act), act.stride(0), _p(w), _p(bias), _p(y1), _p(y2),
                                      _p(label), float(eps), lo, hi, 1 if relu else 0, None, _p(pred), _p(dz), _p(loss),
-                                     _p(dx), dx.stride(0), _p(dw), _p(db), _p(wk), C.c_size_t(wk.numel()), _stream()),
+                                     _p(dx), dx.stride(0) if dx is not None else 0, _p(dw), _p(db), _p(wk),
+                                     C.c_size_t(wk.numel()), _stream()),
           "rec_ctr_head_fwd_bwd")
     return pred, dz, loss, dx
 
@@ -3241,10 +3268,30 @@
             dw.is_contiguous() and dy.is_contiguous() and dy.shape[-1] == 1 and act.shape[0] >= 64)
 
 
+def head_in_gemm(acts, weights, dws, dbs, ws, dz, w_head, images_t=None, **kw):
+    i = len(weights) - 1
+    if (os.environ.get("REC_CTR_HEAD_IN_GEMM", "1") == "0" or i < 1 or kw.get("defer_all") or kw.get("dw_stream") is not None
+            or _recorder is not None or len(acts) != len(weights) + 1):
+        return None
+    h = acts[i + 1]
+    out = torch.empty(acts[i].shape, dtype=torch.float32, device=h.device)
+    rbl = getattr(acts, "relu_bits", None)
+    gen = (dz.reshape(-1), w_head.reshape(-1))
+    if not (h.dim() == 2 and w_head.is_contiguous() and dz.is_contiguous() and w_head.numel() == h.shape[1] and
+            dz.numel() == h.shape[0]):
+        return None
+    ok = linear_backward(acts[i], h, weights[i], ws, dws[i], dbs[i], relu_src=acts[i],
+                         b_image=images_t[i] if images_t is not None else None,
+                         relu_bits=rbl[i] if rbl is not None else None, out=out, gen=gen, gen_query=True)
+    return dict(gen=gen, out=out) if ok else None
+
+
 def mlp_backward(dy, acts, weights, dws, dbs, ws, defer_first=False, defer_all=False, dw_stream=None, dw_ws=None,
-                 defer_split=0, images_t=None, defer_cus=0):
+                 defer_split=0, images_t=None, defer_cus=0, head_gen=None):
     n = len(weights)
     g = dy
+    if head_gen is not None and (defer_all or dw_stream is not None or n < 2):
+        raise RecError("head_gen: this schedule does not issue the last layer as one linear_backward call")
     imt = (lambda i: images_t[i]) if images_t is not None else (lambda i: None)
     rbl = getattr(acts, "relu_bits", None)
     rb = (lambda i: rbl[i]) if rbl is not None else (lambda i: None)
@@ -3285,8 +3332,10 @@
             with torch.cuda.stream(dw_stream):
                 gemm(acts[i], g, dw_ws if dw_ws is not None else ws, trans_a=True, out=dws[i], b_colsum=dbs[i])
         else:
+            hg = head_gen if head_gen is not None and i == n_run - 1 else None
             g = linear_backward(acts[i], g, weights[i], ws, dws[i], dbs[i], relu_src=acts[i] if i > 0 else None,
-                                b_image=imt(i), relu_bits=rb(i) if i > 0 else None)
+                                b_image=imt(i), relu_bits=rb(i) if i > 0 else None,
+                                **(dict(gen=hg["gen"], out=hg["out"]) if hg is not None else {}))
             continue
         if i > 0:
             g = gemm(g, weights[i], ws, trans_b=True, epilogue="relu_mask", aux0=acts[i], b_image=imt(i), relu_bits=rb(i))
```

Result: no change. 45.22 million samples/s (median of 6 runs) (+0.4%).
